# fperezgamonal/flownet2-tf

Measured on AMD Instinct MI355X. Metric: forward pairs/sec at 512x384 (FlowNet2), higher is better.
Workload: dtype f16x2 (split fp16 hi+lo operands, 3 fp16 MFMAs per product, fp32 accumulate); 1 GPU; FlowNet2 forward, batch=4 synthetic 512x384 pairs per GPU, seeded synthetic weights; pairs_per_gpu=4, parallelism=dp1 (no collective)

## Files before the change

flownet2-tf_amd/csrc/conv.hip:

```cpp
#include "conv_common.h"
#include <cstdlib>

namespace fn2 {

template <typename T, typename OutT, int TC, int WC, int WP>
__global__ void __launch_bounds__(256) conv_igemm_kernel(const ConvArgs p) {
  constexpr int CH = 16 / (int)sizeof(T);
  constexpr int BC = WC * TC * 16;
  constexpr int BP = WP * 64;
  constexpr int NT = 256;
  static_assert(WC * WP == 4, "4 waves per block");
  constexpr int NPR = BP / 64;
  constexpr int NWR = (BC * 4 + NT - 1) / NT;
  constexpr int WSWZ_BIT = (TC == 4) ? 5 : (TC == 2) ? 4 : 3;
  __shared__ uint4 lds[2][(BC + BP) * 4];

  const int tid = threadIdx.x, lane = tid & 63, wave = tid >> 6;
  const int wc = wave / WP, wp = wave % WP;
  const int cid = tid & 3;

  int pad_y = p.pad, pad_x = p.pad, oy_off = 0, ox_off = 0, osc = 1;
  const T* wgt = reinterpret_cast<const T*>(p.wgt);
  const int phase = blockIdx.z / p.splitk, split = blockIdx.z - phase * p.splitk;
  if (p.deconv) {
// ... 40 lines not shown
        const T* src = in + (pbase[q] + (size_t)iy * p.W + ix) * p.in_cs + p.in_c0 + cc * CH;
        v = *reinterpret_cast<const uint4*>(src);
      }
      rp[q] = v;
    }
#pragma unroll
    for (int q = 0; q < NWR; ++q) {
      const int e = tid + NT * q;
      uint4 v = make_uint4(0, 0, 0, 0);
      if (e < BC * 4) {
        const T* src = wgt + (size_t)(c0 + (e >> 2)) * wrow_elems + ((size_t)kt * 4 + cid) * CH;
        v = *reinterpret_cast<const uint4*>(src);
      }
      rw[q] = v;
    }
  };
  auto advance = [&]() {
    cc += 4;
    while (cc >= p.cin_chunks) {
      cc -= p.cin_chunks;
      if (++kx == p.KW) { kx = 0; ++ky; }
    }
  };
  auto store_step = [&](int buf) {
#pragma unroll
    for (int q = 0; q < NWR; ++q) {
      const int e = tid + NT * q;
      if (e < BC * 4) {
        const int row = e >> 2;
        lds[buf][row * 4 + (cid ^ (((row >> WSWZ_BIT) & 1) * 3))] = rw[q];
      }
    }
#pragma unroll
    for (int q = 0; q < NPR; ++q) {
      const int row = (tid >> 2) + 64 * q;
      lds[buf][(BC + row) * 4 + (cid ^ (((row >> 3) & 1) * 3))] = rp[q];
    }
  };

  const int fi = lane & 15, fchunk = (lane >> 4) ^ (((fi >> 3) & 1) * 3);
  int a_off[TC], b_off[4];
#pragma unroll
  for (int t = 0; t < TC; ++t)
    a_off[t] = (wc * TC * 16 + (fi >> 2) * (TC * 4) + t * 4 + (fi & 3)) * 4 + fchunk;
#pragma unroll
  for (int pt = 0; pt < 4; ++pt) b_off[pt] = (BC + wp * 64 + pt * 16 + fi) * 4 + fchunk;

  f32x4 acc[TC][4];
#pragma unroll
  for (int t = 0; t < TC; ++t)
#pragma unroll
    for (int pt = 0; pt < 4; ++pt) acc[t][pt] = f32x4{0.f, 0.f, 0.f, 0.f};

  load_step(kt0);
  store_step(0);
  __syncthreads();

  for (int kt = kt0; kt < kt1; ++kt) {
    const int buf = (kt - kt0) & 1;
    const bool more = kt + 1 < kt1;
    if (more) {
      advance();
      load_step(kt + 1);
    }
    uint4 fa[TC], fb[4];
#pragma unroll
    for (int t = 0; t < TC; ++t) fa[t] = lds[buf][a_off[t]];
#pragma unroll
    for (int pt = 0; pt < 4; ++pt) fb[pt] = lds[buf][b_off[pt]];
    if constexpr (sizeof(T) == 2) {
#pragma unroll
      for (int t = 0; t < TC; ++t)
#pragma unroll
        for (int pt = 0; pt < 4; ++pt)
          acc[t][pt] = mfma_16x16x32<T>(fa[t], fb[pt], acc[t][pt]);
    } else {
#pragma unroll
      for (int j = 0; j < 4; ++j)
#pragma unroll
        for (int t = 0; t < TC; ++t)
#pragma unroll
          for (int pt = 0; pt < 4; ++pt)
            acc[t][pt] = __builtin_amdgcn_mfma_f32_16x16x4f32(__builtin_bit_cast(f32x4, fa[t])[j],
                                                             __builtin_bit_cast(f32x4, fb[pt])[j], acc[t][pt], 0, 0, 0);
    }
    if (more) store_step(buf ^ 1);
    __syncthreads();
  }

  OutT* out = reinterpret_cast<OutT*>(p.out);
  const int cout_base = c0 + wc * TC * 16 + (lane >> 4) * (TC * 4);
  if (p.splitk > 1) {
    float* slab = p.ws + (size_t)split * p.N * p.out_H * p.out_W * p.ws_cs;
#pragma unroll
    for (int pt = 0; pt < 4; ++pt) {
      const int m = m0 + wp * 64 + pt * 16 + fi;
      if (m >= p.M) continue;
      const int n = m / (p.OH * p.OW);
      const int rem = m - n * (p.OH * p.OW);
      const int oy = rem / p.OW, ox = rem - oy * p.OW;
      float* po = slab + (((size_t)n * p.out_H + (oy * osc + oy_off)) * p.out_W + (ox * osc + ox_off)) * p.ws_cs;
#pragma unroll
      for (int t = 0; t < TC; ++t) {
        const int co = cout_base + t * 4;
        if (co < p.ws_cs)
          *reinterpret_cast<float4*>(po + co) =
              make_float4(acc[t][pt][0], acc[t][pt][1], acc[t][pt][2], acc[t][pt][3]);
      }
    }
    return;
  }
  float bias[TC][4];
#pragma unroll
  for (int t = 0; t < TC; ++t)
#pragma unroll
    for (int r = 0; r < 4; ++r) {
      const int co = cout_base + t * 4 + r;
      bias[t][r] = (p.bias != nullptr && co < p.Cout) ? p.bias[co] : 0.f;
    }
#pragma unroll
  for (int pt = 0; pt < 4; ++pt) {
    const int m = m0 + wp * 64 + pt * 16 + fi;
    if (m >= p.M) continue;
    const int n = m / (p.OH * p.OW);
    const int rem = m - n * (p.OH * p.OW);
    const int oy = rem / p.OW, ox = rem - oy * p.OW;
    OutT* po = out + (((size_t)n * p.out_H + (oy * osc + oy_off)) * p.out_W + (ox * osc + ox_off)) * p.out_cs +
               p.out_c0;
#pragma unroll
    for (int t = 0; t < TC; ++t) {
      float v[4];
      const int co = cout_base + t * 4;
#pragma unroll
      for (int r = 0; r < 4; ++r) {
        float x = acc[t][pt][r] * p.out_scale + bias[t][r];
        if constexpr (sizeof(OutT) == 4) {
          if (p.accum && co + r < p.Cout) x += load_elem<OutT>(po + co + r);
          if (co + r < p.Cout) x = act_grad<OutT>(p, out, po + co + r, co + r, x);
        }
        if (p.act == FN2_ACT_LEAKY) x = leaky(x);
        v[r] = x;
      }
      if (p.vec_ok && co + 3 < p.Cout) {
        store4<OutT>(po + co, v[0], v[1], v[2], v[3]);
      } else {
#pragma unroll
        for (int r = 0; r < 4; ++r)
          if (co + r < p.Cout) store_elem<OutT>(po + co + r, v[r]);
      }
    }
  }
}

template <typename OutT>
__global__ void __launch_bounds__(256) splitk_finalize_kernel(const float* __restrict__ ws, const float* __restrict__ bias,
                                                              OutT* __restrict__ out, long npix, int ws_cs, int splitk,
                                                              int Cout, int out_cs, int out_c0, int act, int vec_ok,
                                                              float out_scale, int accum, const OutT* __restrict__ mask_y,
                                                              int mask_c0, int mask_c1, const float* __restrict__ up_src,
                                                              const float* __restrict__ up_w, const float* __restrict__ up_bias,
                                                              int up_c0, int out_H, int out_W) {
  const int groups = ws_cs / 4;
  const int groups_all = groups + (up_src != nullptr ? 1 : 0);
  const long total = npix * groups_all;
  const size_t slab = (size_t)npix * ws_cs;
  for (long i = (long)blockIdx.x * blockDim.x + threadIdx.x; i < total; i += (long)gridDim.x * blockDim.x) {
    const long pix = i / groups_all;
    const int co = (int)(i - pix * groups_all) * 4;
    if (co == groups * 4) {
      const int ox = (int)(pix % out_W), oy = (int)((pix / out_W) % out_H), n = (int)(pix / out_W / out_H);
      const int H = out_H >> 1, W = out_W >> 1;
      const int a = oy & 1, b = ox & 1, y = oy >> 1, x = ox >> 1;
      float r0 = up_bias ? up_bias[0] : 0.f, r1 = up_bias ? up_bias[1] : 0.f;
#pragma unroll
      for (int ty = 0; ty < 2; ++ty) {
        const int iy = y - 1 + a + ty, ky = 3 - a - 2 * ty;
        if (iy < 0 || iy >= H) continue;
#pragma unroll
        for (int tx = 0; tx < 2; ++tx) {
          const int ix = x - 1 + b + tx, kx = 3 - b - 2 * tx;
          if (ix < 0 || ix >= W) continue;
          const float2 v = *reinterpret_cast<const float2*>(up_src + (((long)n * H + iy) * W + ix) * 2);
          const float* ww = up_w + (ky * 4 + kx) * 4;
          r0 += v.x * ww[0] + v.y * ww[1];
          r1 += v.x * ww[2] + v.y * ww[3];
        }
      }
      OutT* pu = out + (size_t)pix * out_cs + up_c0;
      store_elem<OutT>(pu, r0);
      store_elem<OutT>(pu + 1, r1);
      continue;
    }
    float4 v = *reinterpret_cast<const float4*>(ws + pix * ws_cs + co);
    int s = 1;
    for (; s + 3 < splitk; s += 4) {
      float4 t[4];
#pragma unroll
      for (int u = 0; u < 4; ++u) t[u] = *reinterpret_cast<const float4*>(ws + (s + u) * slab + pix * ws_cs + co);
#pragma unroll
      for (int u = 0; u < 4; ++u) { v.x += t[u].x; v.y += t[u].y; v.z += t[u].z; v.w += t[u].w; }
    }
    for (; s < splitk; ++s) {
      const float4 t = *reinterpret_cast<const float4*>(ws + s * slab + pix * ws_cs + co);
      v.x += t.x; v.y += t.y; v.z += t.z; v.w += t.w;
    }
    float r[4] = {v.x, v.y, v.z, v.w};
    OutT* po = out + (size_t)pix * out_cs + out_c0 + co;
    const bool full = vec_ok && co + 3 < Cout;
    float old[4] = {0.f, 0.f, 0.f, 0.f}, yv[4] = {1.f, 1.f, 1.f, 1.f};
    const bool mask = mask_y != nullptr && co < mask_c1 && co + 4 > mask_c0;
    if constexpr (sizeof(OutT) == 4) {
      if (full) {
        if (accum) load4<OutT>(po, old);
        if (mask) load4<OutT>(mask_y + (size_t)pix * out_cs + out_c0 + co, yv);
      } else {
#pragma unroll
        for (int j = 0; j < 4; ++j)
          if (co + j < Cout) {
            if (accum) old[j] = load_elem<OutT>(po + j);
            if (mask) yv[j] = load_elem<OutT>(mask_y + (size_t)pix * out_cs + out_c0 + co + j);
          }
      }
    }
#pragma unroll
    for (int j = 0; j < 4; ++j) {
      r[j] *= out_scale;
      if (bias != nullptr && co + j < Cout) r[j] += bias[co + j];
      if constexpr (sizeof(OutT) == 4) {
        if (accum) r[j] += old[j];
        if (mask && co + j >= mask_c0 && co + j < mask_c1) r[j] *= yv[j] > 0.f ? 1.f : (yv[j] < 0.f ? 0.1f : 0.55f);
      }
      if (act == FN2_ACT_LEAKY) r[j] = leaky(r[j]);
    }
    if (vec_ok && co + 3 < Cout) {
      store4<OutT>(po, r[0], r[1], r[2], r[3]);
    } else {
#pragma unroll
      for (int j = 0; j < 4; ++j)
        if (co + j < Cout) store_elem<OutT>(po + j, r[j]);
    }
  }
}

template <typename T>
__device__ __forceinline__ void dot_chunk(const uint4& x, const uint4& w0, const uint4& w1, float& a0, float& a1);
template <>
__device__ __forceinline__ void dot_chunk<float>(const uint4& x, const uint4& w0, const uint4& w1, float& a0,
                                                 float& a1) {
  const float4 xv = __builtin_bit_cast(float4, x), u = __builtin_bit_cast(float4, w0), v = __builtin_bit_cast(float4, w1);
  a0 += xv.x * u.x + xv.y * u.y + xv.z * u.z + xv.w * u.w;
  a1 += xv.x * v.x + xv.y * v.y + xv.z * v.z + xv.w * v.w;
}
template <>
__device__ __forceinline__ void dot_chunk<bf16_t>(const uint4& x, const uint4& w0, const uint4& w1, float& a0,
                                                  float& a1) {
  const unsigned xs[4] = {x.x, x.y, x.z, x.w}, us[4] = {w0.x, w0.y, w0.z, w0.w}, vs[4] = {w1.x, w1.y, w1.z, w1.w};
#pragma unroll
  for (int j = 0; j < 4; ++j) {
    const float xl = __uint_as_float(xs[j] << 16), xh = __uint_as_float(xs[j] & 0xffff0000u);
    a0 += xl * __uint_as_float(us[j] << 16) + xh * __uint_as_float(us[j] & 0xffff0000u);
    a1 += xl * __uint_as_float(vs[j] << 16) + xh * __uint_as_float(vs[j] & 0xffff0000u);
  }
}

template <>
__device__ __forceinline__ void dot_chunk<x2_t>(const uint4&, const uint4&, const uint4&, float&, float&) {}
template <>
__device__ __forceinline__ void dot_chunk<f16_t>(const uint4& x, const uint4& w0, const uint4& w1, float& a0,
                                                 float& a1) {
  typedef __attribute__((ext_vector_type(8))) _Float16 h8;
  const h8 xv = __builtin_bit_cast(h8, x), u = __builtin_bit_cast(h8, w0), v = __builtin_bit_cast(h8, w1);
#pragma unroll
  for (int j = 0; j < 8; ++j) {
    a0 += (float)xv[j] * (float)u[j];
    a1 += (float)xv[j] * (float)v[j];
  }
}

template <typename T>
__global__ void __launch_bounds__(256) flow_head_kernel(const ConvArgs p) {
  constexpr int CH = 16 / (int)sizeof(T);
  const int lane = threadIdx.x & 63;
  const long wave = ((long)blockIdx.x * blockDim.x + threadIdx.x) >> 6;
  const long nwaves = ((long)gridDim.x * blockDim.x) >> 6;
  const T* in = reinterpret_cast<const T*>(p.in);
  const T* w0 = reinterpret_cast<const T*>(p.wgt);
  const T* w1 = w0 + (size_t)p.ksteps * 4 * CH;
  float* out = reinterpret_cast<float*>(p.out);
  if constexpr (is_x2<T>::value) {
    const float* wf0 = reinterpret_cast<const float*>(p.wgt);
    const float* wf1 = wf0 + (size_t)p.ksteps * 4 * CH;
    const int groups = p.cin_chunks >> 1;
    const int nitems = 9 * groups;
    if (p.dbg & 16384) {
      __shared__ float part[8];
      for (long m = blockIdx.x; m < p.M; m += gridDim.x)
        fh_pixel(in, p.H, p.W, p.in_cs, p.in_c0, groups, wf0, wf1, p.bias, p.out_scale, out + (size_t)m * p.out_cs + p.out_c0, m, part);
      return;
    }
    for (long m = wave; m < p.M; m += nwaves) {
      const int x = (int)(m % p.W), y = (int)((m / p.W) % p.H);
      const size_t nb = (size_t)(m / p.W / p.H) * p.H * p.W;
      float a0 = 0.f, a1 = 0.f;
      for (int q = lane; q < nitems; q += 64) {
        const int tap = q / groups, gi = q - tap * groups;
        const int ky = tap / 3, kx = tap - ky * 3;
        const int iy = y + ky - 1, ix = x + kx - 1;
        if (iy < 0 || iy >= p.H || ix < 0 || ix >= p.W) continue;
        const uint4* src = reinterpret_cast<const uint4*>(in + (nb + (size_t)iy * p.W + ix) * p.in_cs + p.in_c0 + gi * 8);
        float xv[8];
        join8(src[0], src[1], xv);
        const float* u = wf0 + (size_t)q * 8;
        const float* v = wf1 + (size_t)q * 8;
#pragma unroll
        for (int j = 0; j < 8; ++j) {
          a0 += xv[j] * u[j];
          a1 += xv[j] * v[j];
        }
      }
// ... 626 lines not shown
  }
  a.kg = 1;
  if (d->wgt_layout == 1 && tile == 128 && !(a.dbg & 32)) {
    const char* e_kg = getenv("FN2_KG");
    if (!e_kg || atoi(e_kg) != 0) {
      const char* e3 = getenv("FN2_KG3_MAX");
      const char* e2 = getenv("FN2_KG2_MAX");
      const long blocks = (long)cdiv(a.M, 64) * (a.cout_pad / 128) * phases;
      if (blocks <= (e3 ? atoi(e3) : 0)) { a.bp64 = 1; a.kg = 3; }
      else if (blocks <= (e2 ? atoi(e2) : 95)) { a.bp64 = 1; a.kg = 2; }
    }
  }
  if (d->wgt_layout == 1 && tile == 128 && !(a.dbg & 32) && d->in.dtype == FN2_F16X2) {
    const char* e_lo = getenv("FN2_DEEP_MIN");
    const char* e_hi = getenv("FN2_DEEP_MAX");
    const long blocks = (long)cdiv(a.M, 64) * (a.cout_pad / 128) * phases;
    const int lo = e_lo ? atoi(e_lo) : 0, hi = e_hi ? atoi(e_hi) : -1;
    if (blocks >= lo && blocks <= hi) { a.bp64 = 3; a.kg = 1; }
  }
  if (d->wgt_layout == 1 && tile == 128 && a.bp64 == 1 && a.kg == 1) {
    const char* e_ring = getenv("FN2_RING_MAX");
    const int ring_max = e_ring ? atoi(e_ring) : 512;
    const long blocks = (long)cdiv(a.M, 64) * (a.cout_pad / 128) * phases;
    if ((a.dbg & 256) || (blocks >= 384 && blocks <= ring_max)) a.bp64 = 2;
    const char* e_rs = getenv("FN2_RING_SPLIT");
    if (e_rs && blocks >= atoi(e_rs) && blocks < 384) a.bp64 = 2;
  }
  *tile_out = tile;
  *phases_out = phases;
  return FN2_OK;
}

static int preferred_split(const ConvArgs& a, int tile, int phases) {
  if (a.merged) return 1;
  const int bp = tile == 128 ? (a.bp64 ? 64 : 128) : (a.bp64 ? 128 : 256);
  const long blocks = (long)cdiv(a.M, bp) * (a.cout_pad / tile) * phases;
  const char* e_min = getenv("FN2_SPLIT_MINBLOCKS");
  if (blocks >= (e_min ? atoi(e_min) : 384)) return 1;
  if (a.bp64 == 3) {
    const char* e_sl = getenv("FN2_DEEP_SLOTS");
    int s = (int)((e_sl ? atoi(e_sl) : 256) / blocks);
    const int maxs = a.ksteps / 16;
    if (s > maxs) s = maxs;
    if (s > 16) s = 16;
    if (s < 2) return 1;
    const int kper = cdiv(a.ksteps, s);
    return cdiv(a.ksteps, kper);
  }
  if (a.kg > 1) {
    const char* e_nos = getenv("FN2_KG_NOSPLIT");
    if (blocks >= (e_nos ? atoi(e_nos) : 96)) return 1;
    const char* e_sl = getenv("FN2_KG_SLOTS");
    int s = (int)((e_sl ? atoi(e_sl) : 256) / blocks);
    const int maxs = a.ksteps / (12 * a.kg);
    if (s > maxs) s = maxs;
    if (s > 16) s = 16;
    if (s < 2) return 1;
    const int kper = cdiv(a.ksteps, s);
    return cdiv(a.ksteps, kper);
  }
  const char* e = getenv("FN2_SPLIT_SLOTS");
  const char* e_rsl = getenv("FN2_RING_SPLIT_SLOTS");
  const int slots = (tile == 128 && a.bp64 == 2) ? (e_rsl ? atoi(e_rsl) : 512) : e ? atoi(e) : 640;
  int s = (int)(slots / blocks);
  const int maxs = a.ksteps / 8;
  if (s > maxs) s = maxs;
  if (s > 16) s = 16;
  if (s < 2) return 1;
  const int kper = cdiv(a.ksteps, s);
  return cdiv(a.ksteps, kper);
}

static int64_t split_bytes(const ConvArgs& a, int s) {
  return (int64_t)s * a.N * a.out_H * a.out_W * a.ws_cs * (int64_t)sizeof(float);
}

}

extern "C" {

int64_t fn2_conv2d_workspace_bytes(const fn2_conv_desc* d) {
  ConvArgs a;
  int tile, phases;
  if (build_args(d, &a, &tile, &phases) != FN2_OK) return 0;
  if (is_flow_head(d)) return 0;
  const int s = preferred_split(a, tile, phases);
  return s > 1 ? split_bytes(a, s) : 0;
}

int fn2_conv2d_splits(const fn2_conv_desc* d) {
  ConvArgs a;
  int tile, phases;
  if (build_args(d, &a, &tile, &phases) != FN2_OK || is_flow_head(d)) return 1;
  int sk = preferred_split(a, tile, phases);
  while (sk > 1 && (d->workspace == nullptr || split_bytes(a, sk) > d->workspace_bytes)) --sk;
  if ((long)a.N * a.out_H * a.out_W * a.ws_cs >= (1L << 31)) sk = 1;
  if (sk > 1) {
    const int kper = cdiv(a.ksteps, sk);
    sk = cdiv(a.ksteps, kper);
    if (d->wgt_layout >= 1) sk = cdiv(a.ksteps / 2, cdiv(kper, 2));
  }
  return sk < 1 ? 1 : sk;
}

int fn2_conv2d_kernel_name(const fn2_conv_desc* d, char* name, int cap) {
  FN2_REQUIRE(name && cap > 0, "conv2d_kernel_name: no buffer");
  name[0] = 0;
  if (!d || d->wgt_layout < 1 || is_flow_head(d)) return FN2_OK;
  conv_name_sink() = ConvNameSink{name, cap};
  const int rc = fn2_conv2d(d, nullptr);
  conv_name_sink() = ConvNameSink{nullptr, 0};
  return rc;
}

int fn2_conv2d(const fn2_conv_desc* d, void* stream) {
  ConvArgs a;
  int tile, phases;
  int rc = build_args(d, &a, &tile, &phases);
  if (rc) return rc;
  hipStream_t s = (hipStream_t)stream;
  if (is_flow_head(d)) {
    int blocks = grid_for((long)a.M * 64, 256);
    if (d->in.dtype == FN2_F16X2 && a.M <= 4096 && !(a.dbg & 32768)) {
      a.dbg |= 16384;
      blocks = a.M;
    } else {
      a.dbg &= ~16384;
    }
    if (d->in.dtype == FN2_F32)
      hipLaunchKernelGGL(flow_head_kernel<float>, dim3(blocks), dim3(256), 0, s, a);
    else if (d->in.dtype == FN2_BF16)
      hipLaunchKernelGGL(flow_head_kernel<bf16_t>, dim3(blocks), dim3(256), 0, s, a);
    else if (d->in.dtype == FN2_F16)
      hipLaunchKernelGGL(flow_head_kernel<f16_t>, dim3(blocks), dim3(256), 0, s, a);
    else
      hipLaunchKernelGGL(flow_head_kernel<x2_t>, dim3(blocks), dim3(256), 0, s, a);
    FN2_CHECK_LAUNCH("flow_head");
    return FN2_OK;
  }
  int sk = preferred_split(a, tile, phases);
  while (sk > 1 && (d->workspace == nullptr || split_bytes(a, sk) > d->workspace_bytes)) --sk;
  if ((long)a.N * a.out_H * a.out_W * a.ws_cs >= (1L << 31)) sk = 1;
  if (sk > 1) {
    a.kper = cdiv(a.ksteps, sk);
    sk = cdiv(a.ksteps, a.kper);
  }
  if (sk > 1) {
    a.splitk = sk;
    a.ws = reinterpret_cast<float*>(d->workspace);
  }
  if (d->up_src != nullptr && d->kind == 5 && 2 * d->out.c == 32) {
    a.up_src = d->up_src; a.up_w = d->up_w; a.up_bias = d->up_bias; a.up_c0 = d->up_c0;
  }
  if (d->head != nullptr && !conv_name_sink().buf) {
    const fn2_conv_desc* h = reinterpret_cast<const fn2_conv_desc*>(d->head);
    FN2_REQUIRE(d->kind == 1 && is_flow_head(h) && h->head == nullptr && h->up_src == nullptr,
                "conv2d: head rides on a kind-1 transposed conv and is a 3x3 two-output fp32 flow head");
    FN2_REQUIRE(h->in.data == d->in.data && h->in.n == d->in.n && h->in.h == d->in.h && h->in.w == d->in.w &&
                    h->in.cs == d->in.cs && h->in.c0 == d->in.c0 && h->in.dtype == d->in.dtype,
                "conv2d: head and transposed conv must read the same view");
    ConvArgs ha;
    int htile, hphases;
    rc = build_args(h, &ha, &htile, &hphases);
    if (rc) return rc;
    const char* e = getenv("FN2_HEAD_RIDE");
    const bool ride = d->in.dtype == FN2_F16X2 && d->wgt_layout == 2 && tile == 128 && sk > 1 && !(e && atoi(e) == 0);
    if (ride) {
      a.fh_M = ha.M;
      a.fh_w = reinterpret_cast<const float*>(ha.wgt);
      a.fh_w1 = ha.ksteps * 4 * 4;
      a.fh_groups = ha.cin_chunks >> 1;
      a.fh_bias = ha.bias;
      a.fh_out = reinterpret_cast<float*>(ha.out);
      a.fh_out_cs = ha.out_cs; a.fh_out_c0 = ha.out_c0;
      a.fh_scale = ha.out_scale;
    } else {
      rc = fn2_conv2d(h, stream);
      if (rc) return rc;
    }
  }
  if (d->wgt_layout >= 1) {
    a.ksteps = a.ksteps / 2;
    a.kper = cdiv(a.kper, 2);
    a.splitk = cdiv(a.ksteps, a.kper);
    if (a.splitk == 1) a.ws = nullptr;
    rc = launch_conv_fast(a, d->in.dtype, d->out.dtype, tile, phases, s);
  } else if (d->in.dtype == FN2_F32 && d->out.dtype == FN2_F16X2) rc = launch_conv<float, x2_t>(a, tile, phases, s);
  else if (d->in.dtype == FN2_F32) rc = launch_conv<float, float>(a, tile, phases, s);
  else if (d->in.dtype == FN2_BF16 && d->out.dtype == FN2_BF16) rc = launch_conv<bf16_t, bf16_t>(a, tile, phases, s);
  else if (d->in.dtype == FN2_BF16) rc = launch_conv<bf16_t, float>(a, tile, phases, s);
  else if (d->out.dtype == FN2_F16) rc = launch_conv<f16_t, f16_t>(a, tile, phases, s);
  else rc = launch_conv<f16_t, float>(a, tile, phases, s);
  if (rc || conv_name_sink().buf) return rc;
  if (a.splitk == 1) {
    if (d->up_src == nullptr || a.up_src != nullptr) return rc;
    fn2_tensor uv = d->out;
    uv.c = 2; uv.c0 = d->up_c0;
    return fn2_upsample_flow(d->up_src, d->up_w, d->up_bias, &uv, d->out.n, d->out.h / 2, d->out.w / 2, stream);
  }
  if ((a.dbg & 524288) || d->raw_partials) return rc;
  const long npix = (long)a.N * a.out_H * a.out_W;
  const int fgrid = grid_for(npix * (a.ws_cs / 4 + (d->up_src != nullptr ? 1 : 0)), 256);
  if (d->out.dtype == FN2_F32)
    hipLaunchKernelGGL(splitk_finalize_kernel<float>, dim3(fgrid), dim3(256), 0, s, a.ws, a.bias, (float*)a.out, npix,
                       a.ws_cs, a.splitk, a.Cout, a.out_cs, a.out_c0, a.act, a.vec_ok, a.out_scale, a.accum, (const float*)a.mask_y, a.mask_c0, a.mask_c1, d->up_src, d->up_w, d->up_bias, d->up_c0, a.out_H, a.out_W);
  else if (d->out.dtype == FN2_F16X2)
    hipLaunchKernelGGL(splitk_finalize_kernel<x2_t>, dim3(fgrid), dim3(256), 0, s, a.ws, a.bias, (x2_t*)a.out,
                       npix, a.ws_cs, a.splitk, a.Cout, a.out_cs, a.out_c0, a.act, a.vec_ok, a.out_scale, a.accum, (const x2_t*)a.mask_y, a.mask_c0, a.mask_c1, d->up_src, d->up_w, d->up_bias, d->up_c0, a.out_H, a.out_W);
  else if (d->out.dtype == FN2_BF16)
    hipLaunchKernelGGL(splitk_finalize_kernel<bf16_t>, dim3(fgrid), dim3(256), 0, s, a.ws, a.bias, (bf16_t*)a.out,
                       npix, a.ws_cs, a.splitk, a.Cout, a.out_cs, a.out_c0, a.act, a.vec_ok, a.out_scale, a.accum, (const bf16_t*)a.mask_y, a.mask_c0, a.mask_c1, d->up_src, d->up_w, d->up_bias, d->up_c0, a.out_H, a.out_W);
  else
    hipLaunchKernelGGL(splitk_finalize_kernel<f16_t>, dim3(fgrid), dim3(256), 0, s, a.ws, a.bias, (f16_t*)a.out,
                       npix, a.ws_cs, a.splitk, a.Cout, a.out_cs, a.out_c0, a.act, a.vec_ok, a.out_scale, a.accum, (const f16_t*)a.mask_y, a.mask_c0, a.mask_c1, d->up_src, d->up_w, d->up_bias, d->up_c0, a.out_H, a.out_W);
  FN2_CHECK_LAUNCH("splitk_finalize");
  return FN2_OK;
}

int fn2_flow_head_gather(const float* t, int t_cs, const float* bias, float* out, int n, int h, int w, void* stream) {
  FN2_REQUIRE(t && out, "flow_head_gather: null pointer");
  FN2_REQUIRE(t_cs >= 18 && t_cs % 2 == 0 && n >= 1 && h >= 1 && w >= 1, "flow_head_gather: t must hold 18 partials per pixel");
  const long tiles = (long)n * ((h + GT_Y - 1) / GT_Y) * ((w + GT_X - 1) / GT_X);
  if (tiles >= 1024)
    hipLaunchKernelGGL(flow_head_gather_kernel, dim3((unsigned)std::min<long>(tiles, 1 << 16)), dim3(256), 0,
                       (hipStream_t)stream, t, t_cs, bias, out, n, h, w);
  else
    hipLaunchKernelGGL(flow_head_gather_small_kernel, dim3(grid_for((long)n * h * w, 256)), dim3(256), 0,
                       (hipStream_t)stream, t, t_cs, bias, out, n, h, w);
  FN2_CHECK_LAUNCH("flow_head_gather");
  return FN2_OK;
}

int fn2_flow_head_tail(const float* t, int t_cs, int taps, const float* bias, float* pf, int n, int h, int w, int ring,
                       const float* up_w, const float* up_bias, const fn2_tensor* up_out, void* stream) {
  return fn2_flow_head_tail_slabs(t, t_cs, 1, 0, 1.f, taps, bias, pf, n, h, w, ring, up_w, up_bias, up_out, stream);
}

int fn2_flow_head_tail_slabs(const float* t, int t_cs, int nslab, int64_t slab_stride, float scale, int taps, const float* bias,
                             float* pf, int n, int h, int w, int ring, const float* up_w, const float* up_bias,
                             const fn2_tensor* up_out, void* stream) {
  FN2_REQUIRE(t && pf, "flow_head_tail: null pointer");
  FN2_REQUIRE(nslab >= 1 && (nslab == 1 || slab_stride >= (int64_t)n * h * w * t_cs), "flow_head_tail: bad slab geometry");
  const TailSrc ts{t, t_cs, nslab, (long)slab_stride, scale};
  FN2_REQUIRE(taps == 3 || taps == 5, "flow_head_tail: taps must be 3 or 5");
  FN2_REQUIRE(t_cs >= 2 * taps * taps && t_cs % 2 == 0 && n >= 1 && h >= 1 && w >= 1,
              "flow_head_tail: t must hold 2 * taps^2 partials per pixel");
  FN2_REQUIRE(!ring || (h >= 3 && w >= 3), "flow_head_tail: a border ring needs h, w >= 3");
  const bool up = up_w != nullptr;
  hipStream_t s = (hipStream_t)stream;
  if (!up) {
    launch_head_tail_t<float>(taps, false, ts, bias, pf, n, h, w, ring, nullptr, nullptr, nullptr, 0, 0, s);
  } else {
    int rc = check_view(up_out, "flow_head_tail upsample output");
    if (rc) return rc;
    FN2_REQUIRE(up_out->c == 2 && up_out->n == n && up_out->h == 2 * h && up_out->w == 2 * w,
                "flow_head_tail: the upsample view must be [n, 2h, 2w, 2]");
    if (up_out->dtype == FN2_F16X2) FN2_REQUIRE(up_out->c0 % 2 == 0, "flow_head_tail: split-fp16 slice must start at an even channel");
    void* d = up_out->data;
    if (up_out->dtype == FN2_F32) launch_head_tail_t<float>(taps, true, ts, bias, pf, n, h, w, ring, up_w, up_bias, d, up_out->cs, up_out->c0, s);
    else if (up_out->dtype == FN2_F16X2) launch_head_tail_t<x2_t>(taps, true, ts, bias, pf, n, h, w, ring, up_w, up_bias, d, up_out->cs, up_out->c0, s);
    else if (up_out->dtype == FN2_BF16) launch_head_tail_t<bf16_t>(taps, true, ts, bias, pf, n, h, w, ring, up_w, up_bias, d, up_out->cs, up_out->c0, s);
    else launch_head_tail_t<f16_t>(taps, true, ts, bias, pf, n, h, w, ring, up_w, up_bias, d, up_out->cs, up_out->c0, s);
  }
  FN2_CHECK_LAUNCH("flow_head_tail");
  return FN2_OK;
}

int fn2_flow_head5(const fn2_tensor* x, const void* wgt, int cin_pad, int kpad, float out_scale, const float* bias, float* pf,
                   int ring, const float* ring_w, const float* ring_b, void* stream) {
  int rc = check_view(x, "flow_head5 input");
  if (rc) return rc;
  FN2_REQUIRE(wgt && pf, "flow_head5: null pointer");
  FN2_REQUIRE(x->dtype == FN2_F16X2 && x->cs % 8 == 0 && x->c0 % 8 == 0, "flow_head5: split-fp16 input, 8-aligned view");
  FN2_REQUIRE(cin_pad % 32 == 0 && cin_pad >= x->c && x->c0 + cin_pad <= x->cs && kpad == cin_pad,
              "flow_head5: the channel run must be whole 128-byte lines inside the buffer (kpad = cin_pad)");
  FN2_REQUIRE(!ring || (x->h >= 3 && x->w >= 3), "flow_head5: a border ring needs h, w >= 3");
  const long in_bytes = (long)x->n * x->h * x->w * x->cs * 4;
  FN2_REQUIRE(in_bytes < (1L << 31), "flow_head5: input buffer >= 2 GiB is not addressable by the LDS-DMA kernel");
  ConvArgs a = {};
  a.in = x->data; a.wgt = wgt; a.bias = bias; a.out = pf;
  a.N = x->n; a.H = x->h; a.W = x->w; a.in_cs = x->cs; a.in_c0 = x->c0;
  a.cin_chunks = cin_pad / 4;
  a.KH = a.KW = 1; a.stride = 1; a.pad = 0;
  a.OH = x->h; a.OW = x->w;
  a.h5_tx = cdiv(x->w, 28); a.h5_ty = cdiv(x->h, 4); a.h5_ring = ring ? 1 : 0;
  const long blocks = (long)x->n * a.h5_ty * a.h5_tx;
  FN2_REQUIRE(blocks * 256 < (1L << 31), "flow_head5: too many tiles");
  a.M = (int)(blocks * 256);
  a.out_H = x->h; a.out_W = x->w; a.out_cs = 2; a.out_c0 = 0; a.Cout = 2;
  a.ksteps = cin_pad / 32;
  a.cout_pad = 64;
  a.act = FN2_ACT_NONE;
  a.kh_ph[0] = a.kh_ph[1] = a.kw_ph[0] = a.kw_ph[1] = 1;
  a.kg = 1; a.splitk = 1; a.kper = a.ksteps; a.ws = nullptr; a.ws_cs = 4;
  a.out_scale = out_scale == 0.f ? 1.f : out_scale;
  a.in_bytes = (int)in_bytes;
  { const char* e = getenv("FN2_H5_DBG"); a.dbg = e ? atoi(e) : 0; }
  a.h5_tiles = (int)blocks;
  long total = blocks;
  if (ring && ring_w != nullptr) {
    FN2_REQUIRE(ring_b != nullptr, "flow_head5: ring_w without ring_b");
    a.h5_wc = ring_w; a.h5_bc = ring_b; a.h5_groups = (x->c + 7) / 8;
    FN2_REQUIRE(x->c0 + a.h5_groups * 8 <= x->cs, "flow_head5: the last 8-channel group reaches past the buffer");
    total += cdiv((long)x->n * (2 * x->w + 2 * (x->h - 2)), 16);
  }
  {
    const char* e = getenv("FN2_H5_STRIP");
    if ((a.ksteps == 3 || a.ksteps == 6) && !(e && atoi(e) == 0) && !(a.dbg & 10)) {
      const int nstrip = cdiv(x->w, 60);
      const char* eb = getenv("FN2_H5_BLOCKS");
      const int target = eb ? atoi(eb) : 256;
      const int segs = std::max(1, std::min(x->h, target / std::max(1, x->n * nstrip)));
      const int rows = cdiv(x->h, segs);
      a.h5_tx = nstrip; a.h5_ty = cdiv(x->h, rows); a.h5_rows = rows;
      return launch_head5_strip(a, x->n * a.h5_ty * a.h5_tx, (hipStream_t)stream);
    }
  }
  return launch_head5(a, (int)total, (hipStream_t)stream);
}

int fn2_flow_head_ring(const fn2_tensor* x, const float* wc, const float* bc, float* pf, void* stream) {
  int rc = check_view(x, "flow_head_ring input");
  if (rc) return rc;
  FN2_REQUIRE(wc && bc && pf, "flow_head_ring: null pointer");
  FN2_REQUIRE(x->dtype == FN2_F16X2 && x->cs % 8 == 0 && x->c0 % 8 == 0, "flow_head_ring: split-fp16 input, 8-aligned view");
  FN2_REQUIRE(x->h >= 3 && x->w >= 3, "flow_head_ring: h, w >= 3");
  const int groups = (x->c + 7) / 8;
  FN2_REQUIRE(x->c0 + groups * 8 <= x->cs, "flow_head_ring: the last 8-channel group reaches past the buffer");
  const long ring = (long)x->n * (2 * x->w + 2 * (x->h - 2));
  hipLaunchKernelGGL(head_ring_kernel, dim3(grid_for(ring * 64, 256)), dim3(256), 0, (hipStream_t)stream, (const x2_t*)x->data,
                     x->cs, x->c0, groups, wc, bc, pf, x->n, x->h, x->w);
  FN2_CHECK_LAUNCH("flow_head_ring");
  return FN2_OK;
}

int fn2_upsample_flow(const float* in, const float* w, const float* bias, const fn2_tensor* out, int n, int h, int wd,
                      void* stream) {
  FN2_REQUIRE(in && w, "upsample_flow: null pointer");
  int rc = check_view(out, "upsample_flow output");
  if (rc) return rc;
  FN2_REQUIRE(out->c == 2 && out->n == n && out->h == 2 * h && out->w == 2 * wd,
              "upsample_flow: output view must be [n, 2h, 2w, 2]");
  const long total = (long)n * 4 * h * wd;
  if (out->dtype == FN2_F32)
    hipLaunchKernelGGL(upsample_flow_kernel<float>, dim3(grid_for(total, 256)), dim3(256), 0, (hipStream_t)stream,
                       in, w, bias, (float*)out->data, n, h, wd, out->cs, out->c0);
  else if (out->dtype == FN2_F16X2)
    hipLaunchKernelGGL(upsample_flow_kernel<x2_t>, dim3(grid_for(total, 256)), dim3(256), 0, (hipStream_t)stream,
                       in, w, bias, (x2_t*)out->data, n, h, wd, out->cs, out->c0);
  else if (out->dtype == FN2_BF16)
    hipLaunchKernelGGL(upsample_flow_kernel<bf16_t>, dim3(grid_for(total, 256)), dim3(256), 0, (hipStream_t)stream,
                       in, w, bias, (bf16_t*)out->data, n, h, wd, out->cs, out->c0);
  else
    hipLaunchKernelGGL(upsample_flow_kernel<f16_t>, dim3(grid_for(total, 256)), dim3(256), 0, (hipStream_t)stream,
                       in, w, bias, (f16_t*)out->data, n, h, wd, out->cs, out->c0);
  FN2_CHECK_LAUNCH("upsample_flow");
  return FN2_OK;
}

int fn2_pack_pair(const float* a, const float* b, const fn2_tensor* out, int pad, void* stream) {
  FN2_REQUIRE(a && b, "pack_pair: null pointer");
  int rc = check_view(out, "pack_pair output");
  if (rc) return rc;
  FN2_REQUIRE(out->c == 6, "pack_pair: output view must have 6 channels");
  return pack_imgs<2>(a, b, out, out->n, 0, pad, stream);
}

int fn2_pack_image_s2d(const float* img, int n_img, int h, int w, const fn2_tensor* out, int n0, int pad, void* stream) {
  FN2_REQUIRE(img, "pack_image_s2d: null pointer");
// ... 32 lines not shown
```

flownet2-tf_amd/csrc/conv2.hip:

```cpp
#include "conv_common.h"

#include <type_traits>
#include <algorithm>
#include <utility>

#ifndef FN2_X2_ORDER
#define FN2_X2_ORDER 0
#endif
#ifndef FN2_CONV_ABLATE
#define FN2_CONV_ABLATE 0
#endif
#ifndef FN2_SETPRIO
#define FN2_SETPRIO 1
#endif

namespace fn2 {

typedef __attribute__((address_space(3))) void* lptr_t;

constexpr unsigned kOobOffset = 0x80000000u;

typedef int v4i_t __attribute__((ext_vector_type(4)));
typedef unsigned u32x4_t __attribute__((ext_vector_type(4)));

__device__ __forceinline__ v4i_t make_rsrc(const void* base, int bytes) {
  const unsigned long long a = (unsigned long long)base;
  return v4i_t{(int)(a & 0xffffffffu), (int)((a >> 32) & 0xffffu), bytes, 0x00020000};
}

__device__ __forceinline__ void dma16(const v4i_t rsrc, const void* lds, unsigned voff, int soff) {
  const unsigned la = (unsigned)(unsigned long long)(lptr_t)lds;
  asm volatile("s_mov_b32 m0, %0\n\ts_nop 0\n\tbuffer_load_dwordx4 %1, %2, %3 offen lds"
               :: "s"(la), "v"(voff), "s"(rsrc), "s"(soff) : "memory");
}

__device__ __forceinline__ void h5_ring_pixel(const ConvArgs& p, long m) {
  const int lane = threadIdx.x & 63;
  const int H = p.OH, W = p.OW, ring = 2 * W + 2 * (H - 2);
  const int nitems = 25 * p.h5_groups;
  const size_t case_stride = (size_t)nitems * 16;
  const x2_t* in = reinterpret_cast<const x2_t*>(p.in);
  float* pf = reinterpret_cast<float*>(p.out);
  const int n = (int)(m / ring), r = (int)(m - (long)n * ring);
  int y, x;
  if (r < W) { y = 0; x = r; }
  else if (r < 2 * W) { y = H - 1; x = r - W; }
  else { const int q = r - 2 * W; y = 1 + (q >> 1); x = (q & 1) ? W - 1 : 0; }
  const int cy = y == 0 ? 0 : (y == H - 1 ? 2 : 1), cx = x == 0 ? 0 : (x == W - 1 ? 2 : 1);
  const int cs = 3 * cy + cx;
  const float* w = p.h5_wc + (size_t)cs * case_stride;
  float a0 = 0.f, a1 = 0.f;
  constexpr int U = 5;
  for (int q0 = lane; q0 < nitems; q0 += 64 * U) {
    uint4 xs[U][2];
    float4 ws[U][4];
    bool ok[U];
#pragma unroll
    for (int k = 0; k < U; ++k) {
      const int q = min(q0 + 64 * k, nitems - 1);
      const int tap = q / p.h5_groups, gi = q - tap * p.h5_groups;
      const int ky = tap / 5, kx = tap - ky * 5;
      const int iy = y + ky - 2, ix = x + kx - 2;
      ok[k] = q0 + 64 * k < nitems && iy >= 0 && iy < H && ix >= 0 && ix < W;
      const int cy2 = min(max(iy, 0), H - 1), cx2 = min(max(ix, 0), W - 1);
      const uint4* src = reinterpret_cast<const uint4*>(in + (((size_t)n * H + cy2) * W + cx2) * p.in_cs + p.in_c0 + gi * 8);
      xs[k][0] = src[0];
      xs[k][1] = src[1];
      const float4* u = reinterpret_cast<const float4*>(w + (size_t)q * 16);
#pragma unroll
      for (int j = 0; j < 4; ++j) ws[k][j] = u[j];
    }
#pragma unroll
    for (int k = 0; k < U; ++k) {
      float xv[8];
      join8(xs[k][0], xs[k][1], xv);
      if (ok[k]) {
#pragma unroll
        for (int j = 0; j < 4; ++j) {
          a0 += xv[2 * j] * ws[k][j].x;
          a1 += xv[2 * j] * ws[k][j].y;
          a0 += xv[2 * j + 1] * ws[k][j].z;
          a1 += xv[2 * j + 1] * ws[k][j].w;
        }
      }
    }
  }
#pragma unroll
  for (int off = 32; off > 0; off >>= 1) {
    a0 += __shfl_xor(a0, off, 64);
    a1 += __shfl_xor(a1, off, 64);
  }
  if (lane == 0)
    *reinterpret_cast<float2*>(pf + (((size_t)n * H + y) * W + x) * 2) = make_float2(a0 + p.h5_bc[2 * cs], a1 + p.h5_bc[2 * cs + 1]);
}

__device__ __forceinline__ void h5_ring_block(const ConvArgs& p, int rb) {
  const int wave = threadIdx.x >> 6;
  const long total = (long)p.N * (2 * p.OW + 2 * (p.OH - 2));
  for (int k = 0; k < 4; ++k) {
    const long m = (long)rb * 16 + wave * 4 + k;
    if (m >= total) return;
    h5_ring_pixel(p, m);
  }
}

__device__ __forceinline__ float* h5_t(uint4* a, uint4* b, int half, int w) {
  const int byte = w * 4;
  return byte < half ? reinterpret_cast<float*>(reinterpret_cast<char*>(a) + byte)
                     : reinterpret_cast<float*>(reinterpret_cast<char*>(b) + (byte - half));
}

template <typename T, typename OutT, int WC, int WP, int TCN = 2, int TPN = 2, int STAGES = 2, int KG = 1, bool M16 = false,
          bool WREG = false, bool SLAB = false, bool HEAD5 = false, bool FEED = false>
__global__ void __launch_bounds__(256 * KG + (FEED ? 256 : 0)) conv_igemm2_kernel(const ConvArgs p) {
#if defined(__HIP_DEVICE_COMPILE__)
  constexpr int CH = 16 / (int)sizeof(T);
  constexpr int ESZ = (int)sizeof(T);
  constexpr int BC = WC * TCN * 32, BP = WP * TPN * 32;
  static_assert(WC * WP == 4, "4 waves per block");
  constexpr int NWI = BC / 32;
  constexpr int NPI = BP / 32;
  static_assert(!WREG || (is_x2<T>::value && TCN == 1 && KG == 1 && (STAGES == 2 || STAGES == 3) && !M16),
                "WREG: split fp16, one cout tile per wave, two-stage loop or 3-slot ring");
  constexpr int BOFF = WREG ? 0 : BC;
  constexpr int kWTileBytes = (32 * TPN * (TCN * 32 + 4) + 32 * TPN) * 4;
  constexpr int kPoolHalfRows = (STAGES * BP * 128 / 2 > 2 * kWTileBytes ? STAGES * BP * 128 / 2 : 2 * kWTileBytes) / 128 + 1;
  constexpr int ROWS = WREG ? kPoolHalfRows : BC + BP;
  static_assert(KG == 1 || STAGES == 2, "K groups run the two-stage loop");
  constexpr bool kDeep = STAGES > 3;
  __shared__ uint4 lds0_all[(kDeep ? STAGES : WREG ? 2 : KG) * ROWS * 8];
  __shared__ uint4 lds1_all[(kDeep || WREG) ? 1 : KG * ROWS * 8];
  __shared__ uint4 lds2_own[(STAGES == 3 && !WREG) ? ROWS * 8 : 1];

  if constexpr (HEAD5) {
    if ((int)blockIdx.x >= p.h5_tiles) {
      h5_ring_block(p, (int)blockIdx.x - p.h5_tiles);
      return;
    }
  }
  if constexpr (WREG && SLAB && is_x2<T>::value) {
    if (p.fh_M > 0 && (int)blockIdx.z >= p.fh_z0) {
      if (FEED && threadIdx.x >= 256) return;
      float* part = reinterpret_cast<float*>(lds0_all);
      const long e = (((long)blockIdx.z - p.fh_z0) * gridDim.y + blockIdx.y) * gridDim.x + blockIdx.x;
      const long total = (long)(gridDim.z - p.fh_z0) * gridDim.y * gridDim.x;
      for (long m = e; m < p.fh_M; m += total)
        fh_pixel(reinterpret_cast<const x2_t*>(p.in), p.H, p.W, p.in_cs, p.in_c0, p.fh_groups, p.fh_w, p.fh_w + p.fh_w1,
                 p.fh_bias, p.fh_scale, p.fh_out + (size_t)m * p.fh_out_cs + p.fh_out_c0, m, part);
      return;
    }
  }
  const int tid = threadIdx.x, lane = tid & 63;
  const int wave_all = __builtin_amdgcn_readfirstlane(tid >> 6);
  const int grp = KG > 1 ? wave_all >> 2 : 0;
  static_assert(!FEED || (WREG && STAGES == 3 && KG == 1), "FEED: the WREG ring");
  const bool feeder = FEED && wave_all >= 4;
  const int wave = (KG > 1 || FEED) ? wave_all & 3 : wave_all;
  uint4* const lds0 = lds0_all + grp * (ROWS * 8);
  uint4* const lds1 = WREG ? lds0_all + BP * 8 : kDeep ? lds0_all + ROWS * 8 : lds1_all + grp * (ROWS * 8);
  uint4* const lds2 = WREG ? lds0_all + 2 * BP * 8 : lds2_own;
  uint4* const ep1 = (kDeep || WREG) ? lds0_all + ROWS * 8 : lds1_all;
  const int wc = wave / WP, wp = wave % WP;

  int pad_y = p.pad, pad_x = p.pad, oy_off = 0, ox_off = 0, osc = 1;
  const T* wgt = reinterpret_cast<const T*>(p.wgt);
  const int phase = blockIdx.z / p.splitk, split = blockIdx.z - phase * p.splitk;
  const unsigned wrow_bytes = (unsigned)p.ksteps * 128u;
  if (p.deconv) {
    const int a = phase >> 1, b = phase & 1;
    pad_y = a ? p.ph_pad1 : p.ph_pad0; pad_x = b ? p.ph_pad1 : p.ph_pad0; oy_off = a; ox_off = b; osc = 2;
    wgt += (size_t)phase * p.cout_pad * (wrow_bytes / ESZ);
  }
  const int khi = p.deconv ? p.kh_ph[phase >> 1] : p.KH, kwi = p.deconv ? p.kw_ph[phase & 1] : p.KW;
  const int nst_all = (p.cin_chunks >> 3) * khi * kwi;
  const int kt0 = split * p.kper + grp;
  const int kt1 = (FN2_CONV_ABLATE && (p.dbg & 1048576)) ? kt0 : min(nst_all, split * p.kper + p.kper);
  int bx = blockIdx.x, by = blockIdx.y;
  if (!(p.dbg & 4)) {
    const int NT = HEAD5 ? p.h5_tiles : gridDim.x * gridDim.y, L = blockIdx.x + gridDim.x * blockIdx.y;
    const int xcd = L & 7, chunk = NT >> 3, rem = NT & 7;
    const int Lp = xcd * chunk + min(xcd, rem) + (L >> 3);
    if (p.wmajor) {
      by = Lp / (int)gridDim.x;
      bx = Lp - by * (int)gridDim.x;
    } else {
      bx = Lp / (int)gridDim.y;
      by = Lp - bx * (int)gridDim.y;
    }
  }
  const int m0 = bx * BP;
  const int c0 = by * BC;

  const v4i_t rsrc_w = make_rsrc(wgt, (int)(p.cout_pad * wrow_bytes));
  const v4i_t rsrc_x = make_rsrc(p.in, p.in_bytes);

  const int lrow = lane >> 3, lphys = lane & 7;
  unsigned woff[NWI];
#pragma unroll
  for (int j = 0; j < NWI; ++j) {
    const int row = wave * (BC / 4) + j * 8 + lrow;
    woff[j] = (unsigned)(c0 + row) * wrow_bytes + (unsigned)((lphys ^ ((row >> 1) & 7)) * 16);
  }
  int roff[NPI];
  unsigned vmask[NPI];
#pragma unroll
  for (int j = 0; j < NPI; ++j) {
    const int row = wave * (BP / 4) + j * 8 + lrow;
    const int m = m0 + row;
    bool v = m < p.M;
    const int mm = v ? m : 0;
    int n = mm / (p.OH * p.OW);
    const int rem = mm - n * (p.OH * p.OW);
    int oy = rem / p.OW, ox = rem - oy * p.OW;
    if constexpr (HEAD5) {
      static_assert(BP == 256, "HEAD5: 8 x 32 positions per block");
      const int tx = bx % p.h5_tx, tyn = bx / p.h5_tx;
      n = tyn / p.h5_ty;
      oy = (tyn - n * p.h5_ty) * 4 - 2 + (row >> 5);
      ox = tx * 28 - 2 + (row & 31);
      v = true;
    }
    const int iy0 = oy * p.stride - pad_y, ix0 = ox * p.stride - pad_x;
    roff[j] = (((n * p.H + iy0) * p.W + ix0) * p.in_cs + p.in_c0) * ESZ + (lphys ^ ((row >> 1) & 7)) * 16;
    unsigned mk = 0;
    if (v) {
      for (int k = 0; k < p.KH; ++k) mk |= (unsigned)(iy0 + k >= 0 && iy0 + k < p.H) << k;
      for (int k = 0; k < p.KW; ++k) mk |= (unsigned)(ix0 + k >= 0 && ix0 + k < p.W) << (8 + k);
    }
    vmask[j] = mk;
  }
  const int spt = p.cin_chunks >> 3;
  const int ntap = khi * kwi;
  const bool tap_outer = FN2_CONV_ABLATE && (p.dbg & 16);
  int sc = tap_outer ? kt0 % spt : kt0 / ntap;
  int tap = tap_outer ? kt0 / spt : kt0 - sc * ntap;
  int ky = tap / kwi, kx = tap - ky * kwi;
  int wstage = kt0;

  auto issue_piece = [&](auto piece_c, uint4* lds) {
    constexpr int i = decltype(piece_c)::value;
    if constexpr (i < NWI) {
      if constexpr (!WREG) {
        if (!(FN2_CONV_ABLATE && (p.dbg & 2)))
          dma16(rsrc_w, &lds[(wave * (BC / 4) + i * 8) * 8], woff[i], ((ky * p.KW + kx) * spt + sc) * 128);
      }
    } else {
      constexpr int j = i - NWI;
      const unsigned tbit = (1u << ky) | (1u << (8 + kx));
      const int toff = ((ky * p.W + kx) * p.in_cs + sc * 8 * CH) * ESZ;
      const unsigned voff = ((vmask[j] & tbit) == tbit && wstage < kt1) ? (unsigned)(roff[j] + toff) : kOobOffset;
      if (!(FN2_CONV_ABLATE && (p.dbg & 1)))
        dma16(rsrc_x, &lds[(BOFF + wave * (BP / 4) + j * 8) * 8], voff, 0);
    }
  };
  u32x4_t wfa[WREG ? 4 : 1], wfb[WREG ? 4 : 1], wfc[(WREG && STAGES == 3) ? 4 : 1];
  const unsigned wlane = (unsigned)lane * 16u;
  const int wtile_off = WREG ? ((c0 >> 5) + wc) * (p.ksteps * 4096) : 0;
  auto load_w = [&](u32x4_t (&wf)[WREG ? 4 : 1]) {
    if constexpr (WREG) {
      const int soff = wtile_off + ((ky * p.KW + kx) * spt + sc) * 4096;
      asm volatile("buffer_load_dwordx4 %0, %4, %5, %6 offen\n\t"
                   "buffer_load_dwordx4 %1, %4, %5, %6 offen offset:1024\n\t"
                   "buffer_load_dwordx4 %2, %4, %5, %6 offen offset:2048\n\t"
                   "buffer_load_dwordx4 %3, %4, %5, %6 offen offset:3072"
                   : "=&v"(wf[0]), "=&v"(wf[1]), "=&v"(wf[2]), "=&v"(wf[3])
                   : "v"(wlane), "s"(rsrc_w), "s"(soff) : "memory");
    }
  };
  auto advance1 = [&]() {
    ++wstage;
    if (tap_outer) {
      if (++sc == spt) {
        sc = 0;
        if (++kx == kwi) { kx = 0; ++ky; }
      }
      if (ky == khi) { ky = 0; sc = spt; }
    } else if (++kx == kwi) {
      kx = 0;
      if (++ky == khi) { ky = 0; ++sc; }
    }
  };
  auto advance = [&]() {
#pragma unroll
    for (int g = 0; g < KG; ++g) advance1();
  };
  auto issue_stage = [&](uint4* lds) {
    [&]<int... I>(std::integer_sequence<int, I...>) {
      (issue_piece(std::integral_constant<int, I>{}, lds), ...);
    }(std::make_integer_sequence<int, NWI + NPI>{});
    advance();
  };
  auto issue_stage_w = [&](uint4* lds, u32x4_t (&wf)[WREG ? 4 : 1]) {
    [&]<int... I>(std::integer_sequence<int, I...>) {
      (issue_piece(std::integral_constant<int, I>{}, lds), ...);
    }(std::make_integer_sequence<int, NWI + NPI>{});
    load_w(wf);
    advance();
  };
  auto wait_w = [&](u32x4_t (&wf)[WREG ? 4 : 1]) {
    if constexpr (WREG)
      asm volatile("s_waitcnt vmcnt(0)" : "+v"(wf[0]), "+v"(wf[1]), "+v"(wf[2]), "+v"(wf[3]) :: "memory");
  };

  const int fr = lane & 31, fh = lane >> 5, fsw = (fr >> 1) & 7;
  f32x16 acc[TCN][TPN];
#pragma unroll
  for (int tc = 0; tc < TCN; ++tc)
#pragma unroll
    for (int tp = 0; tp < TPN; ++tp)
#pragma unroll
      for (int q = 0; q < 16; ++q) acc[tc][tp][q] = 0.f;
  f32x4 acc16[M16 ? TCN * 2 : 1][M16 ? TPN * 2 : 1];
  if constexpr (M16) {
#pragma unroll
    for (int a = 0; a < TCN * 2; ++a)
#pragma unroll
      for (int b = 0; b < TPN * 2; ++b) acc16[a][b] = f32x4{0.f, 0.f, 0.f, 0.f};
  }

  auto compute = [&](const uint4* lds) {
    if (FN2_CONV_ABLATE && (p.dbg & 131072)) return;
#if FN2_SETPRIO
    __builtin_amdgcn_s_setprio(1);
#endif
    const uint4* A = &lds[(wc * TCN * 32 + fr) * 8];
    const uint4* B = &lds[(BC + wp * TPN * 32 + fr) * 8];
    if constexpr (is_x2<T>::value && M16) {
      const int r16 = lane & 15, g16 = lane >> 4;
      uint4 ah[TCN * 2], al[TCN * 2], bh[TPN * 2], bl[TPN * 2];
#pragma unroll
      for (int t = 0; t < TCN * 2; ++t) {
        const int row = wc * TCN * 32 + t * 16 + r16, sw = (row >> 1) & 7;
        ah[t] = lds[row * 8 + ((2 * g16) ^ sw)];
        al[t] = lds[row * 8 + ((2 * g16 + 1) ^ sw)];
      }
#pragma unroll
      for (int t = 0; t < TPN * 2; ++t) {
        const int row = BC + wp * TPN * 32 + t * 16 + r16, sw = (row >> 1) & 7;
        bh[t] = lds[row * 8 + ((2 * g16) ^ sw)];
        bl[t] = lds[row * 8 + ((2 * g16 + 1) ^ sw)];
      }
#pragma unroll
      for (int a = 0; a < TCN * 2; ++a)
#pragma unroll
        for (int b = 0; b < TPN * 2; ++b) {
          acc16[a][b] = mfma_16x16x32<f16_t>(al[a], bh[b], acc16[a][b]);
          acc16[a][b] = mfma_16x16x32<f16_t>(ah[a], bl[b], acc16[a][b]);
// ... 176 lines not shown
      asm volatile("s_waitcnt vmcnt(%0)\n\ts_barrier" :: "n"(ND * (D - 1)) : "memory");
      issue_stage(slot_ptr(wr));
      compute(slot_ptr(rd));
      rd = rd + 1 == STAGES ? 0 : rd + 1;
      wr = wr + 1 == STAGES ? 0 : wr + 1;
    }
    asm volatile("s_waitcnt vmcnt(0)" ::: "memory");
  } else {
    constexpr int ND = NWI + NPI;
    static_assert(ND == 5 || ND == 6 || ND == 8, "vmcnt literal below");
    auto ring_sync = [] {
      if constexpr (ND == 5) asm volatile("s_waitcnt vmcnt(5)\n\ts_barrier" ::: "memory");
      else if constexpr (ND == 6) asm volatile("s_waitcnt vmcnt(6)\n\ts_barrier" ::: "memory");
      else asm volatile("s_waitcnt vmcnt(8)\n\ts_barrier" ::: "memory");
    };
    issue_stage(lds0);
    issue_stage(lds1);
    const int nst3 = (kt1 - kt0 + 2) / 3 * 3;
    for (int s = 0; s < nst3; s += 3) {
      ring_sync(); issue_stage(lds2); compute(lds0);
      ring_sync(); issue_stage(lds0); compute(lds1);
      ring_sync(); issue_stage(lds1); compute(lds2);
    }
    asm volatile("s_waitcnt vmcnt(0)" ::: "memory");
  }

  if constexpr (KG > 1) {
    constexpr int NA4 = TCN * TPN * 4;
    static_assert((KG - 1) * 4 * NA4 * 64 <= KG * ROWS * 8, "reduction scratch must fit the stage buffers");
    float4* red = reinterpret_cast<float4*>(lds0_all);
    auto acc4 = [&](int idx) -> float4 {
      if constexpr (M16) {
        const f32x4 v = acc16[idx / (TPN * 2)][idx % (TPN * 2)];
        return make_float4(v[0], v[1], v[2], v[3]);
      } else {
        const int t = idx >> 2, q = idx & 3;
        return make_float4(acc[t / TPN][t % TPN][4 * q], acc[t / TPN][t % TPN][4 * q + 1], acc[t / TPN][t % TPN][4 * q + 2],
                           acc[t / TPN][t % TPN][4 * q + 3]);
      }
    };
    if (grp > 0) {
#pragma unroll
      for (int idx = 0; idx < NA4; ++idx) red[(((grp - 1) * 4 + wave) * NA4 + idx) * 64 + lane] = acc4(idx);
    }
    __syncthreads();
    if (grp > 0) return;
#pragma unroll
    for (int g = 0; g < KG - 1; ++g)
#pragma unroll
      for (int idx = 0; idx < NA4; ++idx) {
        const float4 v = red[((g * 4 + wave) * NA4 + idx) * 64 + lane];
        if constexpr (M16) {
          f32x4& d = acc16[idx / (TPN * 2)][idx % (TPN * 2)];
          d[0] += v.x; d[1] += v.y; d[2] += v.z; d[3] += v.w;
        } else {
          const int t = idx >> 2, q = idx & 3;
          acc[t / TPN][t % TPN][4 * q] += v.x; acc[t / TPN][t % TPN][4 * q + 1] += v.y;
          acc[t / TPN][t % TPN][4 * q + 2] += v.z; acc[t / TPN][t % TPN][4 * q + 3] += v.w;
        }
      }
  }

  if constexpr (HEAD5) {
    if (p.dbg & 2) return;
    constexpr int TS = 52;
    static_assert(256 * TS * 4 <= 2 * ROWS * 128, "T fits the stage buffers");
#pragma unroll
    for (int tc = 0; tc < TCN; ++tc)
#pragma unroll
      for (int tp = 0; tp < TPN; ++tp) {
        const int pos = wp * TPN * 32 + tp * 32 + fr;
        const int cb = tc * 32 + fh * 16;
#pragma unroll
        for (int q = 0; q < 4; ++q)
          if (cb + 4 * q < TS)
            *reinterpret_cast<float4*>(h5_t(lds0_all, lds1_all, ROWS * 128, pos * TS + cb + 4 * q)) =
                make_float4(acc[tc][tp][4 * q] * p.out_scale, acc[tc][tp][4 * q + 1] * p.out_scale,
                            acc[tc][tp][4 * q + 2] * p.out_scale, acc[tc][tp][4 * q + 3] * p.out_scale);
      }
    __syncthreads();
    if (p.dbg & 8) return;
    const int tx = bx % p.h5_tx, tyn = bx / p.h5_tx;
    const int n = tyn / p.h5_ty, ty = tyn - n * p.h5_ty;
    float* pf = reinterpret_cast<float*>(p.out);
    if (tid < 224) {
      const int o = tid & 1, px = tid >> 1;
      const int py = px / 28, pxx = px - py * 28;
      const int oy = ty * 4 + py, ox = tx * 28 + pxx;
      if (oy < p.OH && ox < p.OW && !(p.h5_ring && (oy == 0 || oy == p.OH - 1 || ox == 0 || ox == p.OW - 1))) {
        float a = p.bias ? p.bias[o] : 0.f;
#pragma unroll
        for (int uy = 0; uy < 5; ++uy)
#pragma unroll
          for (int ux = 0; ux < 5; ++ux)
            a += *h5_t(lds0_all, lds1_all, ROWS * 128, ((py + uy) * 32 + pxx + ux) * TS + (uy * 5 + ux) * 2 + o);
        pf[(((size_t)n * p.OH + oy) * p.OW + ox) * 2 + o] = a;
      }
    }
    return;
  }
  if (FN2_CONV_ABLATE && (p.dbg & 262144)) return;
  if constexpr (M16) {
    OutT* out16 = reinterpret_cast<OutT*>(p.out);
    const int r16 = lane & 15, g16 = lane >> 4;
    float* slab = p.splitk > 1 ? p.ws + (size_t)split * p.N * p.out_H * p.out_W * p.ws_cs : nullptr;
#pragma unroll
    for (int b = 0; b < TPN * 2; ++b) {
      const int m = m0 + wp * TPN * 32 + b * 16 + r16;
      if (m >= p.M) continue;
      const int n = m / (p.OH * p.OW);
      const int rem = m - n * (p.OH * p.OW);
      const int oy = rem / p.OW, ox = rem - oy * p.OW;
      const size_t opix = ((size_t)n * p.out_H + (oy * osc + oy_off)) * p.out_W + (ox * osc + ox_off);
      OutT* po = out16 + opix * p.out_cs + p.out_c0;
#pragma unroll
      for (int a = 0; a < TCN * 2; ++a) {
        const int co = c0 + wc * TCN * 32 + (a >> 1) * 32 + 16 * (g16 & 1) + 8 * (a & 1) + 4 * (g16 >> 1);
        if (slab != nullptr) {
          if (co < p.ws_cs)
            *reinterpret_cast<float4*>(slab + opix * p.ws_cs + co) =
                make_float4(acc16[a][b][0], acc16[a][b][1], acc16[a][b][2], acc16[a][b][3]);
          continue;
        }
        float v[4];
#pragma unroll
        for (int j = 0; j < 4; ++j) {
          float x = acc16[a][b][j] * p.out_scale + ((p.bias != nullptr && co + j < p.Cout) ? p.bias[co + j] : 0.f);
          if constexpr (sizeof(OutT) == 4) {
            if (p.accum && co + j < p.Cout) x += load_elem<OutT>(po + co + j);
            if (co + j < p.Cout) x = act_grad<OutT>(p, out16, po + co + j, co + j, x);
          }
          if (p.act == FN2_ACT_LEAKY) x = leaky(x);
          v[j] = x;
        }
        if (p.vec_ok && co + 3 < p.Cout) store_vec<OutT, 4>(po + co, v);
        else
#pragma unroll
          for (int j = 0; j < 4; ++j)
            if (co + j < p.Cout) store_elem<OutT>(po + co + j, v[j]);
      }
    }
    return;
  }

  OutT* out = reinterpret_cast<OutT*>(p.out);
  constexpr int WCOLS = TCN * 32, RS = WCOLS + 4, WROWS = 32 * TPN;
  constexpr int WTW = WROWS * RS + WROWS;
  constexpr bool kLdsT = (KG > 1 ? 4 : 2) * WTW * 4 <= KG * ROWS * 128;
  if constexpr (FEED && !kLdsT) { if (feeder) return; }
  float* const tl = reinterpret_cast<float*>(KG > 1 ? ep1 : (wave < 2 ? lds0_all : ep1)) + (KG > 1 ? wave : (wave & 1)) * WTW;
  constexpr int CPR = WCOLS / 4, RPI = 64 / CPR;
  static_assert(!SLAB || WREG, "SLAB is a specialisation of the WREG instantiations");
  if ((SLAB || !WREG) && p.splitk > 1) {
    float* slab = p.ws + (size_t)split * p.N * p.out_H * p.out_W * p.ws_cs;
    if constexpr (kLdsT) {
      if constexpr (STAGES >= 3) __syncthreads();
      if constexpr (FEED) { if (feeder) return; }
      int* rowoff = reinterpret_cast<int*>(tl + WROWS * RS);
#pragma unroll
      for (int tp = 0; tp < TPN; ++tp) {
        const int m = m0 + wp * TPN * 32 + tp * 32 + fr;
        const int mm = m < p.M ? m : 0;
        const int n = mm / (p.OH * p.OW);
        const int rem = mm - n * (p.OH * p.OW);
        const int oy = rem / p.OW, ox = rem - oy * p.OW;
        if (fh == 0) rowoff[tp * 32 + fr] = m < p.M ? (int)((((size_t)n * p.out_H + (oy * osc + oy_off)) * p.out_W + (ox * osc + ox_off)) * p.ws_cs) : -1;
#pragma unroll
        for (int tc = 0; tc < TCN; ++tc)
#pragma unroll
          for (int q = 0; q < 4; ++q)
            *reinterpret_cast<float4*>(tl + (tp * 32 + fr) * RS + tc * 32 + fh * 16 + q * 4) =
                make_float4(acc[tc][tp][4 * q], acc[tc][tp][4 * q + 1], acc[tc][tp][4 * q + 2], acc[tc][tp][4 * q + 3]);
      }
      const int rr = lane / CPR, ch = lane - rr * CPR;
      const int co = c0 + wc * WCOLS + ch * 4;
#pragma unroll
      for (int i = 0; i < WROWS / RPI; ++i) {
        const int row = i * RPI + rr;
        const float4 v = *reinterpret_cast<const float4*>(tl + row * RS + ch * 4);
        const int off = rowoff[row];
        if (off >= 0 && co < p.ws_cs) *reinterpret_cast<float4*>(slab + (size_t)off + co) = v;
      }
      return;
    }
#pragma unroll
    for (int tp = 0; tp < TPN; ++tp) {
      const int m = m0 + wp * TPN * 32 + tp * 32 + fr;
      if (m >= p.M) continue;
      const int n = m / (p.OH * p.OW);
      const int rem = m - n * (p.OH * p.OW);
      const int oy = rem / p.OW, ox = rem - oy * p.OW;
      float* po = slab + (((size_t)n * p.out_H + (oy * osc + oy_off)) * p.out_W + (ox * osc + ox_off)) * p.ws_cs;
#pragma unroll
      for (int tc = 0; tc < TCN; ++tc)
#pragma unroll
        for (int q = 0; q < 4; ++q) {
          const int co = c0 + wc * TCN * 32 + tc * 32 + fh * 16 + q * 4;
          if (co < p.ws_cs)
            *reinterpret_cast<float4*>(po + co) = make_float4(acc[tc][tp][4 * q], acc[tc][tp][4 * q + 1],
                                                              acc[tc][tp][4 * q + 2], acc[tc][tp][4 * q + 3]);
        }
    }
    return;
  }
  if constexpr (SLAB) return;
  const bool vec16 = (p.out_cs % 8 == 0) && (p.out_c0 % 8 == 0);
  const bool wide = kLdsT && sizeof(OutT) == 4 && vec16 && c0 + wc * WCOLS + WCOLS <= p.Cout && !(p.dbg & 4194304);
  int* const rowoff = reinterpret_cast<int*>(tl + WROWS * RS);
  if constexpr (STAGES >= 3 && kLdsT) __syncthreads();
  if constexpr (FEED) { if (feeder) return; }
#pragma unroll
  for (int tc = 0; tc < TCN; ++tc) {
    const int cout_base = c0 + wc * TCN * 32 + tc * 32 + fh * 16;
    float bias[16];
#pragma unroll
    for (int q = 0; q < 16; ++q) bias[q] = (p.bias != nullptr && cout_base + q < p.Cout) ? p.bias[cout_base + q] : 0.f;
#pragma unroll
    for (int tp = 0; tp < TPN; ++tp) {
      const int m = m0 + wp * TPN * 32 + tp * 32 + fr;
      if (wide && tc == 0 && fh == 0) rowoff[tp * 32 + fr] = m < p.M ? 0 : -1;
      if (m >= p.M) continue;
      const int n = m / (p.OH * p.OW);
      const int rem = m - n * (p.OH * p.OW);
      const int oy = rem / p.OW, ox = rem - oy * p.OW;
      const size_t opix = (((size_t)n * p.out_H + (oy * osc + oy_off)) * p.out_W + (ox * osc + ox_off));
      OutT* po = out + opix * p.out_cs + p.out_c0 + cout_base;
      float v[16];
#pragma unroll
      for (int q = 0; q < 16; ++q) v[q] = acc[tc][tp][q] * p.out_scale + bias[q];
      accum_act_grad16<OutT>(p, out, po, cout_base, vec16 && cout_base + 15 < p.Cout, v);
      if (p.act == FN2_ACT_LEAKY) {
#pragma unroll
        for (int q = 0; q < 16; ++q) v[q] = leaky(v[q]);
      }
      if (wide) {
        if (tc == 0 && fh == 0) rowoff[tp * 32 + fr] = (int)opix;
        store16<OutT>(reinterpret_cast<OutT*>(tl + (tp * 32 + fr) * RS + tc * 32 + fh * 16), v);
      } else if (vec16 && cout_base + 15 < p.Cout) {
        store16<OutT>(po, v);
      } else {
#pragma unroll
        for (int q = 0; q < 16; ++q)
          if (cout_base + q < p.Cout) store_elem<OutT>(po + q, v[q]);
      }
    }
  }
  if (wide) {
    const int rr = lane / CPR, ch = lane - rr * CPR;
    OutT* ob = out + p.out_c0 + c0 + wc * WCOLS + ch * 4;
#pragma unroll
    for (int i = 0; i < WROWS / RPI; ++i) {
      const int row = i * RPI + rr;
      const uint4 v = *reinterpret_cast<const uint4*>(tl + row * RS + ch * 4);
      const int opix = rowoff[row];
      if (opix >= 0) *reinterpret_cast<uint4*>(ob + (size_t)opix * p.out_cs) = v;
    }
  }
#endif
}

template <typename OutT, int WC, int WP, int TCN, int TPN, int KW>
__global__ void __launch_bounds__(256) conv_halo_kernel(const ConvArgs p) {
#if defined(__HIP_DEVICE_COMPILE__)
  using T = x2_t;
  constexpr int ESZ = 4;
  constexpr int BC = WC * TCN * 32, BP = WP * TPN * 32;
  static_assert(WC * WP == 4, "4 waves per block");
  constexpr int NWI = BC / 32;
  constexpr int BROWS = BP + 8;
  constexpr int NBP = BROWS / 8;
  constexpr int NBW = (NBP + 3) / 4;
  __shared__ uint4 ldsA[2][BC * 8];
  __shared__ uint4 ldsB[2][BROWS * 8];

  const int tid = threadIdx.x, lane = tid & 63;
  const int wave = __builtin_amdgcn_readfirstlane(tid >> 6);
  const int wc = wave / WP, wp = wave % WP;

  int pad_y = p.pad, pad_x = p.pad, oy_off = 0, ox_off = 0, osc = 1;
  const T* wgt = reinterpret_cast<const T*>(p.wgt);
  const int phase = blockIdx.z;
  const unsigned wrow_bytes = (unsigned)p.ksteps * 128u;
  if (p.merged) {
    pad_y = phase ? p.ph_pad1 : p.ph_pad0; pad_x = 1; oy_off = phase; ox_off = 0; osc = 2;
    wgt += (size_t)phase * p.cout_pad * (wrow_bytes / ESZ);
  } else if (p.deconv) {
    const int a = phase >> 1, b = phase & 1;
    pad_y = a ? p.ph_pad1 : p.ph_pad0; pad_x = b ? p.ph_pad1 : p.ph_pad0; oy_off = a; ox_off = b; osc = 2;
    wgt += (size_t)phase * p.cout_pad * (wrow_bytes / ESZ);
  }
  int bx = blockIdx.x, by = blockIdx.y;
  {
    const int NT = gridDim.x * gridDim.y, L = blockIdx.x + gridDim.x * blockIdx.y;
    const int xcd = L & 7, chunk = NT >> 3, rem = NT & 7;
    const int Lp = xcd * chunk + min(xcd, rem) + (L >> 3);
    bx = Lp / (int)gridDim.y;
    by = Lp - bx * (int)gridDim.y;
  }
  const int m0 = bx * BP, c0 = by * BC;
  const int tn = m0 / (p.OH * p.OW);
  const int trem = m0 - tn * (p.OH * p.OW);
  const int toy = trem / p.OW, tox = trem - toy * p.OW;
  const int iy_base = toy - pad_y, ix_base = tox - pad_x;

  const v4i_t rsrc_w = make_rsrc(wgt, (int)(p.cout_pad * wrow_bytes));
  const v4i_t rsrc_x = make_rsrc(p.in, p.in_bytes);
  const int lrow = lane >> 3, lphys = lane & 7;
// ... 788 lines not shown
```

flownet2-tf_amd/csrc/conv_common.h:

```cpp
#pragma once
#include "fn2_common.h"

namespace fn2 {

struct ConvArgs {
  const void* in;
  const void* wgt;
  const float* bias;
  void* out;
  int N, H, W, in_cs, in_c0;
  int cin_chunks;
  int KH, KW, stride, pad;
  int OH, OW;
  int M;
  int out_H, out_W, out_cs, out_c0, Cout;
  int ksteps;
  int cout_pad;
  int act;
  int deconv;
  int ph_pad0, ph_pad1;
  int kh_ph[2], kw_ph[2];
  int merged;
  int wmajor;
  int bp64;
  int KH_KW_hint;
  int kg;
  int h5_tx, h5_ty, h5_ring;
  int h5_tiles, h5_groups;
  const float* h5_wc;
  const float* h5_bc;
  int h5_rows;
  int fh_M, fh_z0;
  const float* fh_w;
  int fh_w1, fh_groups;
  const float* fh_bias;
  float* fh_out;
  int fh_out_cs, fh_out_c0;
  float fh_scale;
  const float* up_src; const float* up_w; const float* up_bias; int up_c0;
  int wfrag;
  int accum;
  int vec_ok;
  int splitk;
  int kper;
  float* ws;
  int ws_cs;
  float out_scale;
  int in_bytes;
  const void* mask_y;
  int mask_c0, mask_c1;
  int dbg;
};

__device__ __forceinline__ void fh_pixel(const x2_t* __restrict__ in, int H, int W, int in_cs, int in_c0, int groups,
                                         const float* __restrict__ wf0, const float* __restrict__ wf1,
                                         const float* __restrict__ bias, float out_scale, float* __restrict__ po, long m,
                                         float* part) {
  const int lane = threadIdx.x & 63, wv = threadIdx.x >> 6;
  const int nitems = 9 * groups;
  const int x = (int)(m % W), y = (int)((m / W) % H);
  const size_t nb = (size_t)(m / W / H) * H * W;
  float a0 = 0.f, a1 = 0.f;
  for (int q = threadIdx.x; q < nitems; q += 256) {
    const int tap = q / groups, gi = q - tap * groups;
    const int ky = tap / 3, kx = tap - ky * 3;
    const int iy = y + ky - 1, ix = x + kx - 1;
    if (iy < 0 || iy >= H || ix < 0 || ix >= W) continue;
    const uint4* src = reinterpret_cast<const uint4*>(in + (nb + (size_t)iy * W + ix) * in_cs + in_c0 + gi * 8);
    float xv[8];
    join8(src[0], src[1], xv);
    const float* u = wf0 + (size_t)q * 8;
    const float* v = wf1 + (size_t)q * 8;
#pragma unroll
    for (int j = 0; j < 8; ++j) {
      a0 += xv[j] * u[j];
      a1 += xv[j] * v[j];
    }
  }
#pragma unroll
  for (int off = 32; off > 0; off >>= 1) {
    a0 += __shfl_xor(a0, off, 64);
    a1 += __shfl_xor(a1, off, 64);
  }
  if (lane == 0) { part[wv * 2] = a0; part[wv * 2 + 1] = a1; }
  __syncthreads();
  if (threadIdx.x == 0) {
    po[0] = (part[0] + part[2] + part[4] + part[6]) * out_scale + (bias ? bias[0] : 0.f);
    po[1] = (part[1] + part[3] + part[5] + part[7]) * out_scale + (bias ? bias[1] : 0.f);
  }
  __syncthreads();
}

template <typename OutT>
__device__ __forceinline__ float act_grad(const ConvArgs& p, const OutT* out_base, const OutT* elem, int co, float x) {
  if (p.mask_y != nullptr && co >= p.mask_c0 && co < p.mask_c1) {
    const float y = load_elem<OutT>(reinterpret_cast<const OutT*>(p.mask_y) + (elem - out_base));
    x *= y > 0.f ? 1.f : (y < 0.f ? 0.1f : 0.55f);
  }
  return x;
}

template <typename OutT>
__device__ __forceinline__ void accum_act_grad16(const ConvArgs& p, const OutT* out_base, const OutT* po, int cout_base,
                                                 bool full, float (&v)[16]) {
  if constexpr (sizeof(OutT) == 4) {
    const bool mask = p.mask_y != nullptr && cout_base < p.mask_c1 && cout_base + 16 > p.mask_c0;
    if (!p.accum && !mask) return;
    if (full) {
      if (p.accum) {
        float o[16];
        load16<OutT>(po, o);
#pragma unroll
        for (int q = 0; q < 16; ++q) v[q] += o[q];
      }
      if (mask) {
        float y[16];
        load16<OutT>(reinterpret_cast<const OutT*>(p.mask_y) + (po - out_base), y);
#pragma unroll
        for (int q = 0; q < 16; ++q)
          if (cout_base + q >= p.mask_c0 && cout_base + q < p.mask_c1) v[q] *= y[q] > 0.f ? 1.f : (y[q] < 0.f ? 0.1f : 0.55f);
      }
    } else {
#pragma unroll
      for (int q = 0; q < 16; ++q)
        if (cout_base + q < p.Cout) {
          if (p.accum) v[q] += load_elem<OutT>(po + q);
          v[q] = act_grad<OutT>(p, out_base, po + q, cout_base + q, v[q]);
        }
    }
  }
}

template <typename OutT>
__device__ __forceinline__ void store4(OutT* p, float a, float b, float c, float d) {
  const float v[4] = {a, b, c, d};
  store_vec<OutT, 4>(p, v);
}

struct ConvNameSink { char* buf; int cap; };
ConvNameSink& conv_name_sink();

int launch_conv_fast(const ConvArgs& a, int in_dtype, int out_dtype, int tile, int phases, hipStream_t s);
int launch_head5(const ConvArgs& a, int blocks, hipStream_t s);
int launch_head5_strip(const ConvArgs& a, int blocks, hipStream_t s);
bool conv_fast_ok(int in_dtype, int cin_pad, int cout);

}
```

flownet2-tf_amd/src/_hip.py:

```python
import ctypes as C
import os

import numpy as np
import torch

_HERE = os.path.dirname(os.path.abspath(__file__))
LIB_PATH = os.path.join(os.path.dirname(_HERE), "lib", "libflownet2_hip.so")

FN2_F32, FN2_BF16, FN2_F16, FN2_F16X2 = 0, 1, 2, 3
ACT_NONE, ACT_LEAKY = 0, 1
OK = 0
ERR_INVALID_ARGUMENT, ERR_UNSUPPORTED, ERR_HIP = -1, -2, -3


class Fn2Tensor(C.Structure):
    _fields_ = [("data", C.c_void_p), ("dtype", C.c_int32), ("n", C.c_int32), ("h", C.c_int32),
                ("w", C.c_int32), ("c", C.c_int32), ("cs", C.c_int32), ("c0", C.c_int32)]


class Fn2ConvPlan(C.Structure):
    _fields_ = [("layout", C.c_int32), ("cout_tile", C.c_int32), ("kstep_elems", C.c_int32),
                ("wgt_dtype", C.c_int32)]


class Fn2ConvDesc(C.Structure):
    _fields_ = [("inp", Fn2Tensor), ("out", Fn2Tensor), ("wgt", C.c_void_p), ("bias", C.c_void_p),
                ("kind", C.c_int32), ("kh", C.c_int32), ("kw", C.c_int32), ("stride", C.c_int32),
                ("pad", C.c_int32), ("act", C.c_int32), ("cin_pad", C.c_int32), ("cout_pad", C.c_int32),
                ("kpad", C.c_int32), ("wgt_layout", C.c_int32), ("accumulate", C.c_int32), ("out_scale", C.c_float), ("workspace", C.c_void_p), ("workspace_bytes", C.c_int64),
                ("act_grad_y", C.c_void_p), ("act_grad_c0", C.c_int32), ("act_grad_c1", C.c_int32),
                ("up_src", C.c_void_p), ("up_w", C.c_void_p), ("up_bias", C.c_void_p), ("up_c0", C.c_int32),
                ("head", C.c_void_p), ("raw_partials", C.c_int32)]


class Fn2BwdwDesc(C.Structure):
    _fields_ = [("x", Fn2Tensor), ("dy", Fn2Tensor), ("dw", C.c_void_p), ("kind", C.c_int32), ("kh", C.c_int32),
                ("kw", C.c_int32), ("stride", C.c_int32), ("pad", C.c_int32), ("cin_pad", C.c_int32),
                ("cout_pad", C.c_int32), ("kpad", C.c_int32), ("wgt_layout", C.c_int32), ("db", C.c_void_p)]


_i, _p, _f = C.c_int, C.c_void_p, C.c_float
_ip = C.POINTER(C.c_int)
_tp = C.POINTER(Fn2Tensor)

PROTOTYPES = {
    "fn2_last_error": (C.c_char_p, []),
    "fn2_version": (_i, []),
    "fn2_crc32c": (C.c_uint32, [_p, C.c_int64, C.c_uint32]),
    "fn2_device_info": (_i, [C.c_char_p, _i, _ip]),
    "fn2_correlation_out_shape": (_i, [_i] * 7 + [_ip] * 3),
    "fn2_correlation_f32": (_i, [_p, _p, _p] + [_i] * 9 + [_p]),
    "fn2_correlation_workspace_bytes": (C.c_int64, [_i] * 9),
    "fn2_correlation_f32_ws": (_i, [_p, _p, _p] + [_i] * 9 + [_p, C.c_int64, _p]),
    "fn2_correlation_grad_f32": (_i, [_p] * 5 + [_i] * 9 + [_p]),
    "fn2_flow_warp_f32": (_i, [_p, _p, _p, _i, _i, _i, _i, _p]),
    "fn2_flow_warp_grad_f32": (_i, [_p] * 5 + [_i] * 4 + [_p]),
    "fn2_downsample_f32": (_i, [_p, _p] + [_i] * 6 + [_p]),
    "fn2_downsample_scaled_f32": (_i, [_p, _f, _p] + [_i] * 6 + [_p]),
    "fn2_fill_zero": (_i, [_p, C.c_int64, _p]),
    "fn2_add_f32": (_i, [_p, _p, C.c_int64, _p]),
    "fn2_slice_copy_f32": (_i, [_tp, _p, _p]),
    "fn2_resize_bilinear_f32": (_i, [_p, _p] + [_i] * 6 + [_f, _p]),
    "fn2_conv2d_plan": (_i, [_i, _i, _i, C.POINTER(Fn2ConvPlan)]),
    "fn2_conv2d_workspace_bytes": (C.c_int64, [C.POINTER(Fn2ConvDesc)]),
    "fn2_conv2d": (_i, [C.POINTER(Fn2ConvDesc), _p]),
    "fn2_conv2d_kernel_name": (_i, [C.POINTER(Fn2ConvDesc), C.c_char_p, _i]),
    "fn2_conv2d_splits": (_i, [C.POINTER(Fn2ConvDesc)]),
    "fn2_augment_f32": (_i, [_p, _p, _p, _p, _i, _i, _i, _i, _i, _i, _p]),
    "fn2_flow_augmentation_f32": (_i, [_p, _p, _p, _p, _i, _i, _i, _i, _i, _p]),
    "fn2_flow_head_gather": (_i, [_p, _i, _p, _p, _i, _i, _i, _p]),
    "fn2_upsample_flow": (_i, [_p, _p, _p, _tp, _i, _i, _i, _p]),
    "fn2_flow_head_tail": (_i, [_p, _i, _i, _p, _p, _i, _i, _i, _i, _p, _p, _tp, _p]),
    "fn2_flow_head_tail_slabs": (_i, [_p, _i, _i, C.c_int64, _f, _i, _p, _p, _i, _i, _i, _i, _p, _p, _tp, _p]),
    "fn2_flow_head_ring": (_i, [_tp, _p, _p, _p, _p]),
    "fn2_flow_head5": (_i, [_tp, _p, _i, _i, _f, _p, _p, _i, _p, _p, _p]),
    "fn2_u8_to_f32_lut": (_i, [_p, _p, _p, C.c_int64, _p]),
    "fn2_pack_pair": (_i, [_p, _p, _tp, _i, _p]),
    "fn2_pack_interp_u8": (_i, [_p, _p, _p, _p, _p, _tp, _i, _p]),
    "fn2_pack_image": (_i, [_p, _i, _tp, _i, _i, _p]),
    "fn2_pack_image_s2d": (_i, [_p, _i, _i, _i, _tp, _i, _i, _p]),
    "fn2_correlation_fused": (_i, [_tp, _tp, _tp, _i, _i, _i, _p]),
    "fn2_stack_input": (_i, [_p, _p, _p, _tp, _i, _p]),
    "fn2_fusion_input": (_i, [_p, _p, _p, _p, _tp, _i, _p]),
    "fn2_stack_input_pf": (_i, [_p, _p, _p, _i, _i, _f, _p, _tp, _i, _p]),
    "fn2_fusion_input_pf": (_i, [_p, _p, _p, _f, _p, _p, _f, _p, _i, _i, _tp, _i, _p]),
    "fn2_epe_loss_grad": (_i, [_p, _p, _p, _p, _i, _i, _i, _f, _f, _p]),
    "fn2_epe_loss_grad_weighted": (_i, [_p, _p, _p, _p, _p, _i, _i, _i, _f, _f, _p]),
    "fn2_leaky_bwd": (_i, [_tp, _tp, _p, _p]),
    "fn2_bias_grad": (_i, [_tp, _p, _p]),
    "fn2_gather_f32": (_i, [_p, _p, _p, C.c_int64, _p]),
    "fn2_to_f16x2": (_i, [_p, _p, _p, C.c_int64, _f, _p]),
    "fn2_to_f16x2_frag": (_i, [_p, _p, _p, C.c_int64, _f, _i, _p]),
    "fn2_adam_step": (_i, [_p, _p, _p, _p, C.c_int64, _f, _f, _f, _f, _i, _f, _f, _p]),
    "fn2_adam_step_multi": (_i, [_p, _p, _p, _i, _f, _f, _f, _f, _i, _f, _p]),
    "fn2_adam_step_multi_dev": (_i, [_p, _p, _p, _i, _p, _p]),
    "fn2_upsample_flow_bwd": (_i, [_tp, _p, _p, _p, _p, _i, _p]),
    "fn2_head_bwd_filter": (_i, [_tp, _p, _p, _i, _i, _p]),
    "fn2_head_g18": (_i, [_p, _tp, _p]),
    "fn2_head_bwd_data": (_i, [_p, _p, _tp, _i, _i, _p]),
    "fn2_conv2d_bwd_filter": (_i, [C.POINTER(Fn2BwdwDesc), _p]),
    "fn2_variational_workspace_bytes": (C.c_int64, [_i, _i, _i]),
    "fn2_variational_refine": (_i, [_p, _p, C.c_int64, C.c_int64, _p, C.c_int64, C.c_int64, _i, _i, _i, _f, _f, _f, _f,
                                    _i, _i, _i, _f, _p, C.c_int64, _p]),
    "fn2_capture_begin": (_i, [_p]),
    "fn2_capture_end": (_i, [_p, C.POINTER(C.c_void_p)]),
    "fn2_graph_launch": (_i, [_p, _p]),
    "fn2_graph_destroy": (_i, [_p]),
}

_lib = None


class HipLibraryMissing(RuntimeError):
    pass


def lib():
    global _lib
    if _lib is None:
        if not os.path.exists(LIB_PATH):
            raise HipLibraryMissing(
                "libflownet2_hip.so not found at %s -- build it with `make -C flownet2-tf_amd/csrc` "
                "(or __graft_entry__.build()); this package has no CPU fallback" % LIB_PATH)
        l = C.CDLL(LIB_PATH)
        for name, (res, args) in PROTOTYPES.items():
            fn = getattr(l, name)
            fn.restype = res
            fn.argtypes = args
        _lib = l
    return _lib


def check(rc):
    if rc == OK:
        return
    msg = lib().fn2_last_error().decode("utf-8", "replace")
    if rc == ERR_INVALID_ARGUMENT:
        raise ValueError(msg)
    if rc == ERR_UNSUPPORTED:
        raise NotImplementedError(msg)
    raise RuntimeError("HIP error: " + msg)


def require_device():
    if not torch.cuda.is_available():
        raise RuntimeError("no ROCm device visible: the FlowNet2 ops run on MI355X only (no CPU fallback)")
    return torch.device("cuda", torch.cuda.current_device())


def stream_ptr():
    return C.c_void_p(torch.cuda.current_stream().cuda_stream)


def ptr(t):
    return C.c_void_p(t.data_ptr())


def dtype_code(t):
    if t.dtype == torch.float32:
        return FN2_F32
    if t.dtype == torch.bfloat16:
        return FN2_BF16
    if t.dtype == torch.float16:
        return FN2_F16
    raise ValueError("unsupported dtype %s" % t.dtype)


def view(buf, c=None, c0=0, code=None):
    n, h, w, cs = buf.shape
    assert buf.is_contiguous()
    return Fn2Tensor(buf.data_ptr(), dtype_code(buf) if code is None else code, n, h, w,
                     cs - c0 if c is None else c, cs, c0)


def conv_plan(in_code, cin_pad, cout):
    p = Fn2ConvPlan()
    check(lib().fn2_conv2d_plan(in_code, cin_pad, cout, C.byref(p)))
    return p


def to_device_f32(x):
    dev = require_device()
    if isinstance(x, np.ndarray):
        return torch.from_numpy(np.ascontiguousarray(x, dtype=np.float32)).to(dev), "numpy"
    if isinstance(x, torch.Tensor):
        kind = "cuda" if x.is_cuda else "cpu"
        return x.detach().to(device=dev, dtype=torch.float32).contiguous(), kind
    raise TypeError("expected torch.Tensor or numpy.ndarray, got %r" % type(x))


def from_device(t, kind):
    if kind == "numpy":
        return t.cpu().numpy()
    if kind == "cpu":
        return t.cpu()
    return t
```

flownet2-tf_amd/src/engine.py:

```python
import ctypes as C
import math
import os

import numpy as np
import torch

from . import _hip, netdefs, weights as W

_DT = {"f32": torch.float32, "bf16": torch.bfloat16, "f16": torch.float16, "f16x2": torch.float32}
_CODE = {"f32": _hip.FN2_F32, "bf16": _hip.FN2_BF16, "f16": _hip.FN2_F16, "f16x2": _hip.FN2_F16X2}
_TILE_ARGS = {128: "2, 2, 2, 2", 64: "1, 4, 2, 2", 32: "1, 4, 1, 2"}


def conv2_kernel_args(tile, m, cout_pad, phases, x2=True):
    dbg = int(os.environ.get("FN2_CONV_DBG", "0"))
    blocks64 = -(-m // 64) * (cout_pad // 128) * phases if tile == 128 else 0
    big = "FN2_M16_MIN" in os.environ and blocks64 >= max(int(os.environ["FN2_M16_MIN"]), 513)
    m16 = "true" if (x2 and not dbg & 512 and (dbg & 1024 or big)) else "false"
    full = dbg & 32
    if tile < 128:
        base = {64: "1, 4, 2, 2, 2, 1", 32: "1, 4, 1, 2, 2, 1"}[tile] if full else {64: "1, 4, 2, 1, 2, 1", 32: "1, 4, 1, 1, 2, 1"}[tile]
        return f"{base}, {m16}"
    blocks = -(-m // 64) * (cout_pad // 128) * phases
    if not full and int(os.environ.get("FN2_KG", "1")):
        if blocks <= int(os.environ.get("FN2_KG3_MAX", "0")):
            return f"2, 2, 2, 1, 2, 3, {m16}"
        if blocks <= int(os.environ.get("FN2_KG2_MAX", "95")):
            return f"2, 2, 2, 1, 2, 2, {m16}"
    if not full and blocks >= int(os.environ.get("FN2_BP64_MIN", "96")):
        ring = 384 <= blocks <= int(os.environ.get("FN2_RING_MAX", "512"))
        return f"2, 2, 2, 1, 3, 1, {m16}" if ring else f"2, 2, 2, 1, 2, 1, {m16}"
    return f"2, 2, 2, 2, 2, 1, {m16}"


_TNAME = {"f32": "float", "bf16": "__bf16", "f16": "_Float16", "f16x2": "fn2::x2_t"}


def _round_up(x, m):
    return (x + m - 1) // m * m


class BatchTooLarge(ValueError):

    def __init__(self, name, batch, nbytes, limit):
        self.fit = max(1, int(batch * (limit - 1) // nbytes))
        super().__init__("activation tensor %s of a batch of %d pairs is %d bytes (limit %d): at most %d pairs per engine"
                         % (name, batch, nbytes, limit, self.fit))


class Engine:
    MAX_TENSOR_BYTES = 1 << 31

    def __init__(self, model, weights, batch, height, width, dtype="f32", device=None, heads_as_gemm=True,
                 no_deconv_biases=None, strict=True, uint8_inputs=False, plain_stems=False, fragment_weights=None,
                 interp_u8_inputs=False):
        if model not in netdefs.MODELS:
            raise ValueError("unknown model %r" % model)
        if dtype not in _DT:
            raise ValueError("dtype must be 'f32', 'bf16', 'f16' or 'f16x2'")
        if height % 64 or width % 64:
            raise ValueError("height and width must be multiples of 64 (pad with Net.adapt_x, net.py:373-388)")
        self.lib = _hip.lib()
        self.device = device if device is not None else _hip.require_device()
        self.model, self.N, self.H, self.W = model, int(batch), int(height), int(width)
        self.dtype_name, self.tdtype = dtype, _DT[dtype]
        self.act_code = _CODE[dtype]
        self.code_of = {}
        self.weights = weights
        if no_deconv_biases is None:
            no_deconv_biases = "FlowNetS/predict_flow6/biases" not in weights
        self.no_deconv_biases = bool(no_deconv_biases)
        self.consumed = set()
        self.ignored_variables = []
        self.ops = []
        self.kernel_of = []
        self.branch_of = []
        self._branch = 0
        self.desc_branch = []
        self.syncs = []
        self._lanes_on = bool(int(os.environ.get("FN2_BRANCHES", "1")))
        default_mask = 0b10011 if model == "FlowNet2" else (0b10101 if model == "FlowNetSD" else 0b10001)
        self._lane_mask = int(os.environ.get("FN2_LANE_MASK", str(default_mask)))
        self.keep = []
        self.bufs = {}
        self.layer_flops = []
        self.layer_bytes = []
        self.layer_io_bytes = []
        self.in_a = torch.zeros((self.N, self.H, self.W, 3), dtype=torch.float32, device=self.device)
        self.in_b = torch.zeros_like(self.in_a)
        self.uint8_inputs = bool(uint8_inputs)
        if self.uint8_inputs:
            self.in_a_u8 = torch.zeros((self.N, self.H, self.W, 3), dtype=torch.uint8, device=self.device)
            self.in_b_u8 = torch.zeros_like(self.in_a_u8)
            self._lut_div = torch.from_numpy((np.arange(256, dtype=np.float64) / 255.0).astype(np.float32)).to(self.device)
            self._lut_raw = torch.arange(256, dtype=torch.float32, device=self.device)
            self._lut = [self._lut_div.clone(), self._lut_div.clone()]
            self._lut_mode = [True, True]
            cnt = self.in_a_u8.numel()
            for src, lut, dst, nm in ((self.in_a_u8, self._lut[0], self.in_a, "a"), (self.in_b_u8, self._lut[1], self.in_b, "b")):
                self.kernel_of.append("u8_to_f32_lut_kernel")
                self.ops.append((f"input_{nm}/u8_to_f32", self.lib.fn2_u8_to_f32_lut,
                                 (_hip.ptr(src), _hip.ptr(lut), _hip.ptr(dst), cnt)))
                self.branch_of.append(0)
        self.interp_u8_inputs = bool(interp_u8_inputs)
        if self.interp_u8_inputs:
            if model != "FlowNetS_interp":
                raise ValueError("interp_u8_inputs belongs to FlowNetS_interp, not %s" % model)
            self.in_img_u8 = torch.zeros((self.N, self.H, self.W, 3), dtype=torch.uint8, device=self.device)
            self.in_mask_u8 = torch.zeros((self.N, self.H, self.W), dtype=torch.uint8, device=self.device)
            self.in_sparse = torch.zeros((self.N, self.H, self.W, 2), dtype=torch.float32, device=self.device)
            self.in_flags = torch.ones((self.N, 2), dtype=torch.uint8, device=self.device)
            self._lut_255 = torch.from_numpy((np.arange(256, dtype=np.float64) / 255.0).astype(np.float32)).to(self.device)
        self.graph = None
        self.conv_descs = []
        self.layers = []
        self.heads_as_gemm = heads_as_gemm
        self.plain_stems = bool(plain_stems)
        self.fragment_weights = bool(int(os.environ.get("FN2_WREG", "1"))) if fragment_weights is None else bool(fragment_weights)
        self.compose_heads = bool(heads_as_gemm) and dtype == "f16x2" and bool(int(os.environ.get("FN2_COMPOSE", "1")))
        self._head_t = None
        self._defer_flow = False
        self._own_ws = set()
        self._pending_head = None
        self.outputs = self._build()
        assert self._pending_head is None
        self._check_variables(strict)
        self._alloc_workspace()
        self._resolve_kernel_names()

    def _buf(self, name, n, h, w, c, dtype=None, stem=False):
        line = 64 if self.act_code in (_hip.FN2_BF16, _hip.FN2_F16) else 32
        cs = (_round_up(c, line) if c > 32 else _round_up(c, 8)) if dtype is None else c
        if dtype is None and not stem and line == 32 and 8 < c <= 32:
            cs = 32

        td = self.tdtype if dtype is None else dtype
        nbytes = n * h * w * cs * torch.empty((), dtype=td).element_size()
        if nbytes >= self.MAX_TENSOR_BYTES:
            if self.N <= 1:
                raise ValueError("one %d x %d pair needs a %d-byte tensor (%s): above the %d-byte limit of the kernels"
                                 % (self.H, self.W, nbytes, name, self.MAX_TENSOR_BYTES))
            raise BatchTooLarge(name, self.N, nbytes, self.MAX_TENSOR_BYTES)
        t = torch.zeros((n, h, w, cs), dtype=td, device=self.device)
        assert name not in self.bufs, name
        self.bufs[name] = t
        self.code_of[t.data_ptr()] = self.act_code if dtype is None else _hip.FN2_F32
        return t

    def _code(self, buf):
        base = buf.untyped_storage().data_ptr()
        return self.code_of.get(buf.data_ptr(), self.code_of.get(base, _hip.dtype_code(buf)))

    def _v(self, buf, c=None, c0=0):
        return _hip.view(buf, c, c0, self._code(buf))

    def _w(self, key):
        if key not in self.weights:
            raise KeyError("the weights lack %r, a variable of the reference's %s graph" % (key, self.model))
        self.consumed.add(key)
        return self.weights[key]

    def _bias(self, scope, name, kind, cout):
        key = f"{scope}/{name}/biases"
        if not netdefs.has_bias(self.model, name, kind, self.no_deconv_biases):
            if key in self.weights:
                self.ignored_variables.append(key)
            return None
        b = np.asarray(self._w(key), np.float32).reshape(-1)
        if b.shape[0] != cout:
            raise ValueError("%s has %d entries, the layer has %d outputs" % (key, b.shape[0], cout))
        return W.to_device(b, torch.float32, self.device)

    _SLOT_SUFFIXES = ("/Adam", "/Adam_1", "/Momentum", "/ExponentialMovingAverage")

    def _check_variables(self, strict):
        roots = tuple(sorted({scope.split("/")[0] + "/" for scope, _ in netdefs.model_scopes(self.model)}))
        stray = [k for k in self.weights
                 if k.startswith(roots) and k not in self.consumed and k not in self.ignored_variables
                 and not k.endswith(self._SLOT_SUFFIXES)]
        if self.ignored_variables:
            import warnings
            warnings.warn("%s: %d bias tensors of the checkpoint belong to layers the reference graph builds without "
                          "biases and are ignored, as the reference ignores them (first: %s)"
                          % (self.model, len(self.ignored_variables), self.ignored_variables[0]))
        if stray and strict:
            raise ValueError("%s: %d checkpoint variables are read by no layer (first: %s); pass strict=False to "
                             "ignore them" % (self.model, len(stray), ", ".join(sorted(stray)[:4])))
        self.stray_variables = stray

    def _sync(self, waiter, waited):
        if waiter != waited:
            self.syncs.append((len(self.ops), waiter, waited))

    def _lane(self, lane):
        eng = self

        class _L:
            def __enter__(self_):
                self_.prev = eng._branch
                eng._branch = lane if (eng._lanes_on and (eng._lane_mask >> lane) & 1) else self_.prev

            def __exit__(self_, *exc):
                eng._branch = self_.prev
        return _L()

    def _head_lane(self):
        hd = self._branch + 2
        return hd if (self._lanes_on and self._branch in (0, 1) and (self._lane_mask >> hd) & 1) else self._branch

    def _op(self, name, fn, *args, kernel=None):
        self.kernel_of.append(kernel if kernel is not None else fn.__name__.replace("fn2_", ""))
        self.ops.append((name, fn, args))
        self.branch_of.append(self._branch)

    def _conv(self, scope, spec, src, dst, up=None, up_after=None, defer_head=False):
        name, kind, k, stride, pad, cin, cout, act = spec
        sbuf, sc0, sc = src
        dbuf, dc0, dc = dst
        assert sc == cin and dc == cout, (scope, name, sc, cin, dc, cout)
        head_px = dbuf.shape[0] * dbuf.shape[1] * dbuf.shape[2]
        if (self.heads_as_gemm and kind == "conv" and cout == 2 and k == 3 and stride == 1 and pad == 1 and not act
                and dbuf.dtype == torch.float32 and head_px >= int(os.environ.get("FN2_HEAD_GEMM_MIN", "8192"))
                and self._head_gemm(scope, spec, src, dst, up)):
            return up is not None and bool(int(os.environ.get("FN2_FUSE_UPFLOW", "1")))
        wname = f"{scope}/{name}/weights"
        in_code = self._code(sbuf)
        esz = 2 if in_code in (_hip.FN2_BF16, _hip.FN2_F16) else 4
        cin_pad = _round_up(cin, 8)
        cin_line = _round_up(cin, 128 // esz)
        if sc0 + cin_line <= sbuf.shape[3] and _hip.conv_plan(in_code, cin_line, cout).layout == 1:
            cin_pad = cin_line
        plan = _hip.conv_plan(in_code, cin_pad, cout)
        tile, layout = plan.cout_tile, plan.layout
        merged = (kind != "conv" and self.compose_heads and cout == 16 and in_code == _hip.FN2_F16X2 and layout == 1
                  and tile == 32 and sbuf.shape[2] % 128 == 0 and bool(int(os.environ.get("FN2_DECONV_MERGED", "1"))))
        if kind == "conv":
            packed, cin_pad, cout_pad, kpad = W.pack_conv(self._w(wname), tile, plan.kstep_elems, cin_pad, layout)
        elif merged:
            packed, cin_pad, cout_pad, kpad = W.pack_deconv_merged(self._w(wname), tile, plan.kstep_elems, cin_pad, layout)
        else:
            packed, cin_pad, cout_pad, kpad = W.pack_deconv(self._w(wname), tile, plan.kstep_elems, cin_pad, layout)
        bias = self._bias(scope, name, kind, cout)
        out_scale = 1.0
        if plan.wgt_dtype == _hip.FN2_F16X2:
            wmax = float(abs(packed).max())
            if wmax > 0:
                k2 = int(math.floor(math.log2(1024.0 / wmax)))
                packed = packed * (2.0 ** k2)
                out_scale = 2.0 ** (-k2)
        wdev = W.packed_to_device(packed, plan.wgt_dtype, self.device)
        d = _hip.Fn2ConvDesc()
        d.inp = self._v(sbuf, sc, sc0)
        d.out = self._v(dbuf, dc, dc0)
        d.wgt = wdev.data_ptr()
        d.bias = bias.data_ptr() if bias is not None else None
        d.kind = 0 if kind == "conv" else (5 if merged else 1)
        d.kh = d.kw = k
        d.stride, d.pad = stride, pad
        d.act = _hip.ACT_LEAKY if act else _hip.ACT_NONE
        d.cin_pad, d.cout_pad, d.kpad = cin_pad, cout_pad, kpad
        d.wgt_layout = layout
        d.out_scale = out_scale
        frag = False
        if (self.fragment_weights and layout == 1 and tile >= int(os.environ.get("FN2_WREG_TILE_MIN", "128"))
                and plan.wgt_dtype == _hip.FN2_F16X2 and self._wants_fragments(d)):
            wdev = W.to_fragment_order(wdev)
            d.wgt, d.wgt_layout, frag = wdev.data_ptr(), 2, True
        self.keep += [d, wdev, bias]
        self.conv_descs.append(d)
        self.desc_branch.append(self._branch)
        up_rec = None
        if self._pending_head is not None and kind != "conv":
            hd = self._pending_head
            assert up_after is not None and hd.inp.data == d.inp.data and hd.inp.c0 == d.inp.c0, (scope, name)
            d.head = C.addressof(hd)
            self._pending_head = None
        if up_after is not None:
            assert kind != "conv" and (not merged or cout == 16)
            up_name, up_src, (ubuf, uc0, uc) = up_after
            assert ubuf is dbuf and uc == 2
            uw = W.to_device(self._w(f"{scope}/{up_name}/weights"), torch.float32, self.device)
            ub = self._bias(scope, up_name, "deconv", 2)
            d.up_src, d.up_w, d.up_bias, d.up_c0 = up_src.data_ptr(), uw.data_ptr(), (ub.data_ptr() if ub is not None else None), uc0
            uv = self._v(ubuf, uc, uc0)
            self.keep += [uw, ub, uv]
            up_rec = dict(scope=scope, name=up_name, kind="upflow", src=up_src, dst=up_after[2], w=uw, b=ub, view=uv)
        self.layers.append(dict(scope=scope, name=name, kind=d.kind, k=k, stride=stride, pad=pad, cin=cin, cout=cout,
                                act=bool(act), src=src, dst=dst, desc=d, w=wdev, b=bias, cin_pad=cin_pad,
                                cout_pad=cout_pad, kpad=kpad, layout=layout, tile=tile, kstep=plan.kstep_elems, frag=frag))
        if up_rec is not None:
            self.layers.append(up_rec)
        tn = _TNAME[self.dtype_name] if in_code == self.act_code else "float"
        if kind == "conv" and cout == 2 and k == 3 and stride == 1 and pad == 1:
            kern = f"flow_head_kernel<{tn}>"
        elif layout == 1:
            on = _TNAME[self.dtype_name] if self._code(dbuf) == self.act_code else "float"
            m_px = dbuf.shape[0] * dbuf.shape[1] * dbuf.shape[2] // (4 if kind != "conv" else 1)
            kern = f"conv_igemm2_kernel<{tn}, {on}, {conv2_kernel_args(tile, m_px, cout_pad, 4 if kind != 'conv' else 1, tn == 'fn2::x2_t')}>"
        else:
            shape = {128: "4, 2, 2", 64: "4, 1, 4", 32: "2, 1, 4", 16: "1, 1, 4"}[tile]
            on = _TNAME[self.dtype_name] if self._code(dbuf) == self.act_code else "float"
            kern = f"conv_igemm_kernel<{tn}, {on}, {shape}>"
        if defer_head and kern.startswith("flow_head_kernel"):
            assert self._pending_head is None
            self._pending_head = d
        else:
            self._op(f"{scope}/{name}", self.lib.fn2_conv2d, C.byref(d), kernel=kern)
        n, oh, ow = dbuf.shape[0], dbuf.shape[1], dbuf.shape[2]
        taps = k * k if kind == "conv" else 4
        self.layer_flops.append((f"{scope}/{name}", 2.0 * n * oh * ow * taps * cin * cout))
        osz = 4 if dbuf.dtype == torch.float32 else 2
        self.layer_io_bytes.append((f"{scope}/{name}", float(sbuf.shape[0] * sbuf.shape[1] * sbuf.shape[2] * cin * esz
                                                            + n * oh * ow * cout * osz + k * k * cin * cout * esz)))

    def _head_slabs(self, d, head_t, t_cs):
        need = int(self.lib.fn2_conv2d_workspace_bytes(C.byref(d)))
        if need <= 0 or not int(os.environ.get("FN2_HEAD_SLABS", "1")):
            return _hip.ptr(head_t), t_cs, 1, 0, 1.0
        ws = torch.empty((need + 3) // 4, dtype=torch.float32, device=self.device)
        d.workspace, d.workspace_bytes, d.raw_partials = ws.data_ptr(), need, 1
        self.keep.append(ws)
        self._own_ws.add(C.addressof(d))
        splits = int(self.lib.fn2_conv2d_splits(C.byref(d)))
        if splits <= 1:
            d.raw_partials = 0
            return _hip.ptr(head_t), t_cs, 1, 0, 1.0
        ws_cs = (d.out.c + 3) // 4 * 4
        return ws.data_ptr(), ws_cs, splits, d.out.n * d.out.h * d.out.w * ws_cs, float(d.out_scale) or 1.0

    def _wants_fragments(self, d):
        need = int(self.lib.fn2_conv2d_workspace_bytes(C.byref(d)))
        d.workspace, d.workspace_bytes = (1, need) if need else (None, 0)
        buf = C.create_string_buffer(256)
        rc = self.lib.fn2_conv2d_kernel_name(C.byref(d), buf, 256)
        d.workspace, d.workspace_bytes = None, 0
        which = os.environ.get("FN2_WREG_KERNELS", "false>")
        return rc == 0 and buf.value.decode().startswith("conv_igemm2_kernel") and buf.value.decode().endswith(which)

    def _head_gemm(self, scope, spec, src, dst, up=None):
        name, kind, k, stride, pad, cin, cout, act = spec
        sbuf, sc0, sc = src
        pf = dst[0]
        in_code = self._code(sbuf)
        esz = 2 if in_code in (_hip.FN2_BF16, _hip.FN2_F16) else 4
        cin_line = _round_up(cin, 128 // esz)
        if sc0 + cin_line > sbuf.shape[3]:
            return False
        plan = _hip.conv_plan(in_code, cin_line, 18)
        if plan.layout != 1:
            return False
        w = np.asarray(self._w(f"{scope}/{name}/weights"), np.float32)
        w1 = np.ascontiguousarray(w.transpose(2, 0, 1, 3)).reshape(1, 1, cin, 18)
        packed, cin_pad, cout_pad, kpad = W.pack_conv(w1, plan.cout_tile, plan.kstep_elems, cin_line, plan.layout)
        out_scale = 1.0
        if plan.wgt_dtype == _hip.FN2_F16X2:
            wmax = float(abs(packed).max())
            if wmax > 0:
                k2 = int(math.floor(math.log2(1024.0 / wmax)))
                packed, out_scale = packed * (2.0 ** k2), 2.0 ** (-k2)
        wdev = W.packed_to_device(packed, plan.wgt_dtype, self.device)
        bias = self._bias(scope, name, kind, cout)
        if self._head_t is None:
            self._head_t = {}
        if self._branch not in self._head_t:
            self._head_t[self._branch] = torch.zeros((self.N * self.H * self.W, 32), dtype=torch.float32, device=self.device)
        head_t = self._head_t[self._branch]
        n, h, wd = pf.shape[0], pf.shape[1], pf.shape[2]
        d = _hip.Fn2ConvDesc()
        d.inp = self._v(sbuf, sc, sc0)
        d.out = _hip.Fn2Tensor(head_t.data_ptr(), _hip.FN2_F32, n, h, wd, 18, 32, 0)
        d.wgt, d.bias = wdev.data_ptr(), None
        d.kind, d.kh, d.kw, d.stride, d.pad = 0, 1, 1, 1, 0
        d.act = _hip.ACT_NONE
        d.cin_pad, d.cout_pad, d.kpad, d.wgt_layout = cin_pad, cout_pad, kpad, plan.layout
        d.out_scale = out_scale
        self.keep += [d, wdev, bias]
        self.conv_descs.append(d)
        self.desc_branch.append(self._branch)
        tn = _TNAME[self.dtype_name] if in_code == self.act_code else "float"
        self._op(f"{scope}/{name}", self.lib.fn2_conv2d, C.byref(d),
                 kernel=f"conv_igemm2_kernel<{tn}, float, {conv2_kernel_args(plan.cout_tile, 0, cout_pad, 1, tn == 'fn2::x2_t')}>")
        t_ptr, t_cs, nslab, slab, tscale = self._head_slabs(d, head_t, 32)
        if up is not None and int(os.environ.get("FN2_FUSE_UPFLOW", "1")):
            up_name, (ubuf, uc0, uc) = up
            uw = W.to_device(self._w(f"{scope}/{up_name}/weights"), torch.float32, self.device)
            ub = self._bias(scope, up_name, "deconv", 2)
            uv = self._v(ubuf, uc, uc0)
            self.keep += [uw, ub, uv]
            self.layers.append(dict(scope=scope, name=up_name, kind="upflow", src=pf, dst=up[1], w=uw, b=ub, view=uv))
            self._op(f"{scope}/{name}/tail+{up_name}", self.lib.fn2_flow_head_tail_slabs, t_ptr, t_cs, nslab, slab,
                     C.c_float(tscale), 3, _hip.ptr(bias) if bias is not None else None, _hip.ptr(pf), n, h, wd, 0, _hip.ptr(uw),
                     _hip.ptr(ub) if ub is not None else None, C.byref(uv), kernel="flow_head_tail")
        else:
            self._op(f"{scope}/{name}/tail", self.lib.fn2_flow_head_tail_slabs, t_ptr, t_cs, nslab, slab, C.c_float(tscale), 3,
                     _hip.ptr(bias) if bias is not None else None, _hip.ptr(pf), n, h, wd, 0, None, None, None,
                     kernel="flow_head_tail")
        self.layer_flops.append((f"{scope}/{name}", 2.0 * n * h * wd * 9 * cin * 2))
        self.layer_io_bytes.append((f"{scope}/{name}", float(n * h * wd * (cin * esz + 2 * 4) + 18 * cin * esz)))
        return True

    def _composed_head(self, scope, ic_spec, pf_spec, src, pf, up=None):
        sbuf, sc0, sc = src
        in_code = self._code(sbuf)
        if in_code != _hip.FN2_F16X2 or sc0 % 8 or sbuf.shape[1] < 3 or sbuf.shape[2] < 3:
            return False
        cin_line = _round_up(sc, 32)
        if sc0 + cin_line > sbuf.shape[3]:
            return False
        plan = _hip.conv_plan(in_code, cin_line, 50)
        if plan.layout != 1:
            return False
        ic_name, pf_name = ic_spec[0], pf_spec[0]
        w1, w2 = self._w(f"{scope}/{ic_name}/weights"), self._w(f"{scope}/{pf_name}/weights")
        b1 = self._w(f"{scope}/{ic_name}/biases") if netdefs.has_bias(self.model, ic_name, "conv", self.no_deconv_biases) else None
        b2 = self._w(f"{scope}/{pf_name}/biases") if netdefs.has_bias(self.model, pf_name, "conv", self.no_deconv_biases) else None
        w5, bias5 = W.compose_interconv_head(w1, b1, w2, b2)
        n, h, wd = pf.shape[0], pf.shape[1], pf.shape[2]
        groups = (sc + 7) // 8
        wc = np.zeros((9, 25, groups * 8, 2), np.float32)
        wc[:, :, :sc, :] = w5.reshape(9, 25, sc, 2)
        wcd = W.to_device(wc, torch.float32, self.device)
        bcd = W.to_device(bias5.astype(np.float32), torch.float32, self.device)
        vin = self._v(sbuf, sc, sc0)
        self.keep += [wcd, bcd, vin]
        w1x1 = np.ascontiguousarray(w5[4].transpose(2, 0, 1, 3)).reshape(1, 1, sc, 50).astype(np.float32)
        packed, cin_pad, cout_pad, kpad = W.pack_conv(w1x1, plan.cout_tile, plan.kstep_elems, cin_line, plan.layout)
        out_scale = 1.0
        wmax = float(abs(packed).max())
        if wmax > 0:
            k2 = int(math.floor(math.log2(1024.0 / wmax)))
            packed, out_scale = packed * (2.0 ** k2), 2.0 ** (-k2)
        wdev = W.packed_to_device(packed, plan.wgt_dtype, self.device)
        cm = ic_spec[6]
        if n * h * wd >= int(os.environ.get("FN2_HEAD5_MIN", "65536")) and plan.cout_tile == 64 and kpad == cin_pad:
            b5 = W.to_device(bias5[4].astype(np.float32), torch.float32, self.device)
            vx = self._v(sbuf, sc, sc0)
            self.keep += [wdev, b5, vx]
            strip = cin_pad in (96, 192) and int(os.environ.get("FN2_H5_STRIP", "1"))
            self._op(f"{scope}/{ic_name}+{pf_name}", self.lib.fn2_flow_head5, C.byref(vx), _hip.ptr(wdev), cin_pad, kpad,
                     C.c_float(out_scale), _hip.ptr(b5), _hip.ptr(pf), 1, _hip.ptr(wcd), _hip.ptr(bcd),
                     kernel=("head5_strip_kernel<%d>" % (cin_pad // 96)) if strip else
                     "conv_igemm2_kernel<fn2::x2_t, float, 1, 4, 2, 2, 2, 1, false, false, false, true>")
            self.layer_flops.append((f"{scope}/{ic_name}+{pf_name}", 2.0 * n * h * wd * 9 * (sc * cm + cm * 2)))
            self.layer_io_bytes.append((f"{scope}/{ic_name}+{pf_name}", float(n * h * wd * (sc * 4 + 2 * 4) + 9 * (sc * cm + 2 * cm) * 4)))
            return 1
        self._op(f"{scope}/{pf_name}/ring", self.lib.fn2_flow_head_ring, C.byref(vin), _hip.ptr(wcd), _hip.ptr(bcd), _hip.ptr(pf),
                 kernel="flow_head_ring")
        if self._head_t is None:
            self._head_t = {}
        key = (self._branch, 64)
        if key not in self._head_t:
            self._head_t[key] = torch.zeros((self.N * self.H * self.W, 64), dtype=torch.float32, device=self.device)
        head_t = self._head_t[key]
        d = _hip.Fn2ConvDesc()
        d.inp = self._v(sbuf, sc, sc0)
        d.out = _hip.Fn2Tensor(head_t.data_ptr(), _hip.FN2_F32, n, h, wd, 50, 64, 0)
        d.wgt, d.bias = wdev.data_ptr(), None
        d.kind, d.kh, d.kw, d.stride, d.pad = 0, 1, 1, 1, 0
        d.act = _hip.ACT_NONE
        d.cin_pad, d.cout_pad, d.kpad, d.wgt_layout = cin_pad, cout_pad, kpad, plan.layout
        d.out_scale = out_scale
        b5 = W.to_device(bias5[4].astype(np.float32), torch.float32, self.device)
        self.keep += [d, wdev, b5]
        self.conv_descs.append(d)
        self.desc_branch.append(self._branch)
        self._op(f"{scope}/{ic_name}+{pf_name}", self.lib.fn2_conv2d, C.byref(d), kernel="conv_igemm2_kernel (composed head)")
        t_ptr, t_cs, nslab, slab, tscale = self._head_slabs(d, head_t, 64)
        if up is not None:
            up_name, (ubuf, uc0, uc) = up
            uw = W.to_device(self._w(f"{scope}/{up_name}/weights"), torch.float32, self.device)
            ub = self._bias(scope, up_name, "deconv", 2)
            uv = self._v(ubuf, uc, uc0)
            self.keep += [uw, ub, uv]
            self.layers.append(dict(scope=scope, name=up_name, kind="upflow", src=pf, dst=up[1], w=uw, b=ub, view=uv))
            self._op(f"{scope}/{pf_name}/tail+{up_name}", self.lib.fn2_flow_head_tail_slabs, t_ptr, t_cs, nslab, slab,
                     C.c_float(tscale), 5, _hip.ptr(b5), _hip.ptr(pf), n, h, wd, 1, _hip.ptr(uw),
                     _hip.ptr(ub) if ub is not None else None, C.byref(uv), kernel="flow_head_tail")
        else:
            self._op(f"{scope}/{pf_name}/tail", self.lib.fn2_flow_head_tail_slabs, t_ptr, t_cs, nslab, slab, C.c_float(tscale), 5,
                     _hip.ptr(b5), _hip.ptr(pf), n, h, wd, 1, None, None, None, kernel="flow_head_tail")
        self.layer_flops.append((f"{scope}/{ic_name}+{pf_name}", 2.0 * n * h * wd * 9 * (sc * cm + cm * 2)))
        self.layer_io_bytes.append((f"{scope}/{ic_name}+{pf_name}", float(n * h * wd * (sc * 4 + 2 * 4) + 9 * (sc * cm + 2 * cm) * 4)))
        return 2 if up is not None else 1

    def _conv_stem(self, scope, spec, sbuf, dst, s2d=False):
        name, kind, k, stride, pad, cin, cout, act = spec
        dbuf, dc0, dc = dst
        assert kind == "conv" and dc == cout
        k_alg, cin_alg = k, cin
        w_hwio = self._w(f"{scope}/{name}/weights")
        if s2d:
            assert stride == 2 and cin == 3 and sbuf.shape[3] == 16
            k2 = (k + 1) // 2
            w = np.zeros((k2, k2, 16, cout), np.float32)
            for ky in range(k):
                for kx in range(k):
                    w[ky // 2, kx // 2, ((ky & 1) * 2 + (kx & 1)) * 4:((ky & 1) * 2 + (kx & 1)) * 4 + 3] = w_hwio[ky, kx]
            w_hwio, k, stride, cin = w, k2, 1, 16
        cs = sbuf.shape[3]
        in_code = self._code(sbuf)
        esz = 2 if in_code in (_hip.FN2_BF16, _hip.FN2_F16) else 4
        run = _round_up(k * cs, 128 // esz)
        plan = _hip.conv_plan(in_code, run, cout)
        assert plan.layout == 1, (scope, name)
        packed, cin_pad, cout_pad, kpad = W.pack_stem(w_hwio, cs, run, plan.cout_tile, plan.layout)
        bias = self._bias(scope, name, kind, cout)
        out_scale = 1.0
        if plan.wgt_dtype == _hip.FN2_F16X2:
            k2 = int(math.floor(math.log2(1024.0 / float(abs(packed).max()))))
            packed, out_scale = packed * (2.0 ** k2), 2.0 ** (-k2)
        wdev = W.packed_to_device(packed, plan.wgt_dtype, self.device)
        d = _hip.Fn2ConvDesc()
        d.inp = self._v(sbuf, cs, 0)
        d.out = self._v(dbuf, dc, dc0)
        d.wgt = wdev.data_ptr()
        d.bias = bias.data_ptr() if bias is not None else None
        d.kind = 2
        d.kh = d.kw = k
        d.stride, d.pad = stride, 0
        d.act = _hip.ACT_LEAKY if act else _hip.ACT_NONE
        d.cin_pad, d.cout_pad, d.kpad = cin_pad, cout_pad, kpad
        d.wgt_layout = plan.layout
        d.out_scale = out_scale
        self.keep += [d, wdev, bias]
        self.conv_descs.append(d)
        self.desc_branch.append(self._branch)
        self.layers.append(dict(scope=scope, name=name, kind=2, k=k, stride=stride, pad=pad, cin=cin, cout=cout,
                                act=bool(act), src=(sbuf, 0, cs), dst=dst, desc=d, w=wdev, b=bias, cin_pad=cin_pad,
                                cout_pad=cout_pad, kpad=kpad, layout=plan.layout, tile=plan.cout_tile,
                                kstep=plan.kstep_elems, cs=cs))
        tn = _TNAME[self.dtype_name]
        self._op(f"{scope}/{name}", self.lib.fn2_conv2d, C.byref(d),
                 kernel=f"conv_igemm2_kernel<{tn}, {tn}, {conv2_kernel_args(plan.cout_tile, 0, cout_pad, 1, tn == 'fn2::x2_t')}>")
        n, oh, ow = dbuf.shape[0], dbuf.shape[1], dbuf.shape[2]
        self.layer_flops.append((f"{scope}/{name}", 2.0 * n * oh * ow * k_alg * k_alg * cin_alg * cout))
        self.layer_io_bytes.append((f"{scope}/{name}", float(sbuf.numel() * esz + n * oh * ow * cout * esz
                                                            + k_alg * k_alg * cin_alg * cout * esz)))

    def _upflow(self, scope, name, src_f32, dst):
        dbuf, dc0, dc = dst
        w = W.to_device(self._w(f"{scope}/{name}/weights"), torch.float32, self.device)
        b = self._bias(scope, name, "deconv", 2)
        v = self._v(dbuf, dc, dc0)
        self.keep += [w, v, b]
        n, h, wd, _ = src_f32.shape
        self.layers.append(dict(scope=scope, name=name, kind="upflow", src=src_f32, dst=dst, w=w, b=b, view=v))
        self._op(f"{scope}/{name}", self.lib.fn2_upsample_flow, _hip.ptr(src_f32), _hip.ptr(w),
                 _hip.ptr(b) if b is not None else None, C.byref(v), n, h, wd)

    def _resize(self, name, src_f32, scale):
        n, h, w, c = src_f32.shape
        dst = self._buf(name, n, self.H, self.W, 2, torch.float32)
        self._op(name, self.lib.fn2_resize_bilinear_f32, _hip.ptr(src_f32), _hip.ptr(dst), n, h, w, c, self.H,
                 self.W, C.c_float(scale))
        return dst

    def _resolve_kernel_names(self):
        buf = C.create_string_buffer(256)
        for i, (name, fn, args) in enumerate(self.ops):
            if fn is self.lib.fn2_conv2d:
                if self.lib.fn2_conv2d_kernel_name(args[0], buf, 256) == 0 and buf.value:
                    self.kernel_of[i] = buf.value.decode()

    def _alloc_workspace(self):
        branches = self.desc_branch + [0] * (len(self.conv_descs) - len(self.desc_branch))
        self.workspace = {}
        for br in sorted(set(branches)):
            descs = [d for d, b in zip(self.conv_descs, branches) if b == br and C.addressof(d) not in self._own_ws]
            need = max([int(self.lib.fn2_conv2d_workspace_bytes(C.byref(d))) for d in descs] + [0])
            if need > 0:
                self.workspace[br] = torch.empty((need + 3) // 4, dtype=torch.float32, device=self.device)
                for d in descs:
                    d.workspace = self.workspace[br].data_ptr()
                    d.workspace_bytes = need

    def _refine(self, scope, tag, L, c6_1, cats, interconv):
        N = c6_1.shape[0]
        preds = {}
        M, Hd = self._branch, self._head_lane()
        h, w = c6_1.shape[1], c6_1.shape[2]
        pf = self._buf(f"{tag}/predict_flow6", N, h, w, 2, torch.float32)
        self._sync(Hd, M)
        skips, decs = (512, 512, 256, 128), (512, 256, 128, 64)
        ride_heads = (Hd == M and self.heads_as_gemm and self.dtype_name == "f16x2"
                      and bool(int(os.environ.get("FN2_UP_IN_DECONV", "1"))) and bool(int(os.environ.get("FN2_HEAD_IN_DECONV", "1"))))
        with self._lane(Hd):
            fused = self._conv(scope, L["predict_flow6"], (c6_1, 0, 1024), (pf, 0, 2),
                               up=("upsample_flow6to5", (cats[5], skips[0] + decs[0], 2)), defer_head=ride_heads)
        preds["predict_flow6"] = pf
        cur, cur_c = c6_1, 1024
        for i, (lvl, skip_c, dec_c) in enumerate(zip((5, 4, 3, 2), skips, decs)):
            cat = cats[lvl]
            h, w = cat.shape[1], cat.shape[2]
            ride = (not fused and Hd == M and self._code(cat) == self.act_code
                    and bool(int(os.environ.get("FN2_UP_IN_DECONV", "1"))))
            self._conv(scope, L[f"deconv{lvl}"], (cur, 0, cur_c), (cat, skip_c, dec_c),
                       up_after=(f"upsample_flow{lvl + 1}to{lvl}", pf, (cat, skip_c + dec_c, 2)) if ride else None)
            if not fused and not ride:
                with self._lane(Hd):
                    self._upflow(scope, f"upsample_flow{lvl + 1}to{lvl}", pf, (cat, skip_c + dec_c, 2))
            self._sync(M, Hd)
            if not interconv:
                self._sync(Hd, M)
            cur, cur_c = cat, skip_c + dec_c + 2
            head_src = (cat, 0, cur_c)
            pf = self._buf(f"{tag}/predict_flow{lvl}", N, h, w, 2, torch.float32)
            up = None
            if lvl > 2:
                up = (f"upsample_flow{lvl}to{lvl - 1}", (cats[lvl - 1], skips[i + 1] + decs[i + 1], 2))
            if interconv and self.compose_heads:
                self._sync(Hd, M)
                with self._lane(Hd):
                    composed = self._composed_head(scope, L[f"interconv{lvl}"], L[f"predict_flow{lvl}"], head_src, pf, up=up)
                if composed:
                    fused = composed == 2
                    preds[f"predict_flow{lvl}"] = pf
                    continue
            if interconv:
                ic = self._buf(f"{tag}/interconv{lvl}", N, h, w, dec_c)
                self._conv(scope, L[f"interconv{lvl}"], (cat, 0, cur_c), (ic, 0, dec_c))
                self._sync(Hd, M)
                head_src = (ic, 0, dec_c)
            with self._lane(Hd):
                fused = self._conv(scope, L[f"predict_flow{lvl}"], head_src, (pf, 0, 2), up=up,
                                   defer_head=ride_heads and lvl > 2 and not interconv)
            preds[f"predict_flow{lvl}"] = pf
        return preds

    def _final_flow(self, tag, preds, scale):
        M, Hd = self._branch, self._head_lane()
        if self._defer_flow:
            preds["flow"] = self._buf(f"{tag}/flow", self.N, self.H, self.W, 2, torch.float32)
            preds["_flow_src"] = (preds["predict_flow2"], scale)
            self._sync(M, Hd)
            return preds
        with self._lane(Hd):
            preds["flow"] = self._resize(f"{tag}/flow", preds["predict_flow2"], scale)
        self._sync(M, Hd)
        return preds

    def _alloc_cats(self, tag, N):
        H, W_ = self.H, self.W
        return {5: self._buf(f"{tag}/concat5", N, H // 32, W_ // 32, 1026),
                4: self._buf(f"{tag}/concat4", N, H // 16, W_ // 16, 770),
                3: self._buf(f"{tag}/concat3", N, H // 8, W_ // 8, 386),
                2: self._buf(f"{tag}/concat2", N, H // 4, W_ // 4, 194)}

    def _encoder_tail(self, scope, tag, L, cats):
        N, H, W_ = self.N, self.H, self.W
        c4 = self._buf(f"{tag}/conv4", N, H // 16, W_ // 16, 512)
        self._conv(scope, L["conv4"], (cats[3], 0, 256), (c4, 0, 512))
        self._conv(scope, L["conv4_1"], (c4, 0, 512), (cats[4], 0, 512))
        c5 = self._buf(f"{tag}/conv5", N, H // 32, W_ // 32, 512)
        self._conv(scope, L["conv5"], (cats[4], 0, 512), (c5, 0, 512))
        self._conv(scope, L["conv5_1"], (c5, 0, 512), (cats[5], 0, 512))
        c6 = self._buf(f"{tag}/conv6", N, H // 64, W_ // 64, 1024)
        self._conv(scope, L["conv6"], (cats[5], 0, 512), (c6, 0, 1024))
        c6_1 = self._buf(f"{tag}/conv6_1", N, H // 64, W_ // 64, 1024)
        self._conv(scope, L["conv6_1"], (c6, 0, 1024), (c6_1, 0, 1024))
        return c6_1

    def _net_s(self, scope, tag, x, cin):
        N, H, W_ = self.N, self.H, self.W
        L = {s[0]: s for s in netdefs.flownet_s_layers(cin)}
        cats = self._alloc_cats(tag, N)
        c1 = self._buf(f"{tag}/conv1", N, H // 2, W_ // 2, 64)
        self._conv_stem(scope, L["conv1"], x, (c1, 0, 64))
        self._conv(scope, L["conv2"], (c1, 0, 64), (cats[2], 0, 128))
        c3 = self._buf(f"{tag}/conv3", N, H // 8, W_ // 8, 256)
        self._conv(scope, L["conv3"], (cats[2], 0, 128), (c3, 0, 256))
        self._conv(scope, L["conv3_1"], (c3, 0, 256), (cats[3], 0, 256))
        c6_1 = self._encoder_tail(scope, tag, L, cats)
        preds = self._refine(scope, tag, L, c6_1, cats, False)
        return self._final_flow(tag, preds, 20.0)

    def _net_c(self, scope, tag):
        N, H, W_ = self.N, self.H, self.W
        L = {s[0]: s for s in netdefs.flownet_c_layers()}
        cats = self._alloc_cats(tag, N)
        batch_towers = os.environ.get("FN2_C_TOWERS", "lane") == "batch"
        if batch_towers:
            del self.bufs[f"{tag}/concat2"]
            cat2_all = self._buf(f"{tag}/concat2", 2 * N, H // 4, W_ // 4, 194)
            cats[2] = cat2_all[:N]
        c1 = self._buf(f"{tag}/conv1", 2 * N, H // 2, W_ // 2, 64)
        if self.plain_stems:
            x2 = self._buf(f"{tag}/images", 2 * N, H + 6, W_ + 6, 3, stem=True)
            v = self._v(x2, 3, 0)
            self.keep.append(v)
            self._op(f"{tag}/pack_a", self.lib.fn2_pack_image, _hip.ptr(self.in_a), N, C.byref(v), 0, 3)
            self._op(f"{tag}/pack_b", self.lib.fn2_pack_image, _hip.ptr(self.in_b), N, C.byref(v), N, 3)
            self._conv_stem(scope, L["conv1"], x2, (c1, 0, 64))
        else:
            x2 = self._buf(f"{tag}/images", 2 * N, (H + 6) // 2, (W_ + 6) // 2, 16, stem=True)
            v = self._v(x2, 16, 0)
            self.keep.append(v)
            self._op(f"{tag}/pack_a", self.lib.fn2_pack_image_s2d, _hip.ptr(self.in_a), N, H, W_, C.byref(v), 0, 3)
            self._op(f"{tag}/pack_b", self.lib.fn2_pack_image_s2d, _hip.ptr(self.in_b), N, H, W_, C.byref(v), N, 3)
            self._conv_stem(scope, L["conv1"], x2, (c1, 0, 64), s2d=True)
        M, T = self._branch, (4 if (self._lanes_on and self._lane_mask & 16 and not batch_towers) else self._branch)
        if batch_towers:
            self._conv(scope, L["conv2"], (c1, 0, 64), (cat2_all, 0, 128))
            c3 = self._buf(f"{tag}/conv_ab_3", 2 * N, H // 8, W_ // 8, 256)
            self._conv(scope, L["conv3"], (cat2_all, 0, 128), (c3, 0, 256))
            c3a, c3b = c3[:N], c3[N:]
        else:
            c2b = self._buf(f"{tag}/conv_b_2", N, H // 4, W_ // 4, 128)
            self._sync(T, M)
            self._conv(scope, L["conv2"], (c1[:N], 0, 64), (cats[2], 0, 128))
            with self._lane(T):
                self._conv(scope, L["conv2"], (c1[N:], 0, 64), (c2b, 0, 128))
            c3a = self._buf(f"{tag}/conv_a_3", N, H // 8, W_ // 8, 256)
            c3b = self._buf(f"{tag}/conv_b_3", N, H // 8, W_ // 8, 256)
            self._conv(scope, L["conv3"], (cats[2], 0, 128), (c3a, 0, 256))
            with self._lane(T):
                self._conv(scope, L["conv3"], (c2b, 0, 128), (c3b, 0, 256))
            self._sync(M, T)
            self._sync(T, M)
        net = self._buf(f"{tag}/corr_concat", N, H // 8, W_ // 8, 473)
        va, vb, vo = self._v(c3a, 256, 0), self._v(c3b, 256, 0), self._v(net, 441, 32)
        self.keep += [va, vb, vo]
        tn = _TNAME[self.dtype_name]
        self._op(f"{tag}/correlation", self.lib.fn2_correlation_fused, C.byref(va), C.byref(vb), C.byref(vo), 20, 2,
                 _hip.ACT_LEAKY, kernel=self._corr_kernel_name(tn, H // 8))
        self.layers.append(dict(scope=scope, name="correlation", kind="corr", fa=c3a, fb=c3b, dst=(net, 32, 441)))
        self.layer_flops.append((f"{scope}/correlation", 2.0 * N * (H // 8) * (W_ // 8) * 441 * 256))
        self.layer_bytes.append((f"{tag}/correlation", 4.0 * N * (H // 8) * (W_ // 8) * (2 * 256 + 441)))
        with self._lane(T):
            self._conv(scope, L["conv_redir"], (c3a, 0, 256), (net, 0, 32))
        self._sync(M, T)
        self._conv(scope, L["conv3_1"], (net, 0, 473), (cats[3], 0, 256))
        c6_1 = self._encoder_tail(scope, tag, L, cats)
        preds = self._refine(scope, tag, L, c6_1, cats, False)
        return self._final_flow(tag, preds, 20.0)

    def _net_sd(self, scope, tag, x):
        N, H, W_ = self.N, self.H, self.W
        L = {s[0]: s for s in netdefs.flownet_sd_layers()}
        cats = self._alloc_cats(tag, N)
        c0 = self._buf(f"{tag}/conv0", N, H, W_, 64)
        self._conv_stem(scope, L["conv0"], x, (c0, 0, 64))
        c1 = self._buf(f"{tag}/conv1", N, H // 2, W_ // 2, 64)
        self._conv(scope, L["conv1"], (c0, 0, 64), (c1, 0, 64))
        c1_1 = self._buf(f"{tag}/conv1_1", N, H // 2, W_ // 2, 128)
        self._conv(scope, L["conv1_1"], (c1, 0, 64), (c1_1, 0, 128))
        self._conv(scope, L["conv2"], (c1_1, 0, 128), (cats[2], 0, 128))
        c2_1 = self._buf(f"{tag}/conv2_1", N, H // 4, W_ // 4, 128)
        self._conv(scope, L["conv2_1"], (cats[2], 0, 128), (c2_1, 0, 128))
        c3 = self._buf(f"{tag}/conv3", N, H // 8, W_ // 8, 256)
        self._conv(scope, L["conv3"], (c2_1, 0, 128), (c3, 0, 256))
        self._conv(scope, L["conv3_1"], (c3, 0, 256), (cats[3], 0, 256))
        c6_1 = self._encoder_tail(scope, tag, L, cats)
        preds = self._refine(scope, tag, L, c6_1, cats, True)
        return self._final_flow(tag, preds, 0.05)

    def _corr_kernel_name(self, tn, h):
        nl = 4 if self.dtype_name in ("bf16", "f16") else 8
        if self.dtype_name != "f32" and h % 4 == 0 and int(os.environ.get("FN2_CORR3", "1")):
            return f"corr3_kernel<{tn}, {tn}, {nl}>"
        return f"corr2_kernel<{tn}, {tn}, {nl}>"

    def _pair_input(self, tag, pad):
        x = self._buf(f"{tag}/pair", self.N, self.H + 2 * pad, self.W + 2 * pad, 6, stem=True)
        v = self._v(x, 6, 0)
        self.keep.append(v)
        if self.interp_u8_inputs:
            self._op(f"{tag}/pack_interp_u8", self.lib.fn2_pack_interp_u8, _hip.ptr(self.in_img_u8), _hip.ptr(self.in_mask_u8),
                     _hip.ptr(self.in_sparse), _hip.ptr(self._lut_255), _hip.ptr(self.in_flags), C.byref(v), pad)
            return x
        self._op(f"{tag}/pack_pair", self.lib.fn2_pack_pair, _hip.ptr(self.in_a), _hip.ptr(self.in_b), C.byref(v), pad)
        return x

    def _stacked_input(self, tag, preds):
        x = self._buf(f"{tag}/stack", self.N, self.H + 6, self.W + 6, 16, stem=True)
        v = self._v(x, 12, 0)
        self.keep.append(v)
        if "_flow_src" in preds:
            pf2, scale = preds["_flow_src"]
            self._op(f"{tag}/stack_input", self.lib.fn2_stack_input_pf, _hip.ptr(self.in_a), _hip.ptr(self.in_b), _hip.ptr(pf2),
                     pf2.shape[1], pf2.shape[2], C.c_float(scale), _hip.ptr(preds["flow"]), C.byref(v), 3, kernel="stack_input")
        else:
            self._op(f"{tag}/stack_input", self.lib.fn2_stack_input, _hip.ptr(self.in_a), _hip.ptr(self.in_b),
                     _hip.ptr(preds["flow"]), C.byref(v), 3)
        return x

    def _sub(self, build, *args):
        prev, self._defer_flow = self._defer_flow, bool(int(os.environ.get("FN2_FLOW_IN_CONSUMER", "1")))
        try:
            return build(*args)
        finally:
            self._defer_flow = prev

    def _net_cs(self, scope, tag):
        pc = self._sub(self._net_c, scope + "/FlowNetC", tag + "/C")
        return self._net_s(scope + "/FlowNetS", tag + "/S", self._stacked_input(tag + "/S", pc), 12)

    def _net_css(self, scope, tag):
        pcs = self._sub(self._net_cs, scope + "/FlowNetCS", tag + "/CS")
        return self._net_s(scope + "/FlowNetS", tag + "/S", self._stacked_input(tag + "/S", pcs), 12)

    def _net_2(self, scope, tag):
        N, H, W_ = self.N, self.H, self.W
        fork = len(self.ops)
        css = self._sub(self._net_css, scope + "/FlowNetCSS", tag + "/CSS")
        if self._lanes_on and self._lane_mask & 2:
            fork += min(int(os.environ.get("FN2_SD_FORK_OPS", "0")), len(self.ops) - fork)
            self.syncs.append((fork, 1, 0))
            if self._lane_mask & 8 and int(os.environ.get("FN2_FORK3", "1")):
                self.syncs.append((fork, 3, 0))
        with self._lane(1):
            sd = self._sub(self._net_sd, scope + "/FlowNetSD", tag + "/SD", self._pair_input(tag + "/SD", 1))
        if self._lanes_on and self._lane_mask & 2:
            self._sync(0, 1)
        L = {s[0]: s for s in netdefs.fusion_layers()}
        xf = self._buf(f"{tag}/fusion_in", N, H + 2, W_ + 2, 16, stem=True)
        v = self._v(xf, 11, 0)
        self.keep.append(v)
        if "_flow_src" in sd and "_flow_src" in css:
            (pf_sd, s_sd), (pf_css, s_css) = sd["_flow_src"], css["_flow_src"]
            self._op(f"{tag}/fusion_input", self.lib.fn2_fusion_input_pf, _hip.ptr(self.in_a), _hip.ptr(self.in_b),
                     _hip.ptr(pf_sd), C.c_float(s_sd), _hip.ptr(sd["flow"]), _hip.ptr(pf_css), C.c_float(s_css),
                     _hip.ptr(css["flow"]), pf_sd.shape[1], pf_sd.shape[2], C.byref(v), 1, kernel="fusion_input")
        else:
            self._op(f"{tag}/fusion_input", self.lib.fn2_fusion_input, _hip.ptr(self.in_a), _hip.ptr(self.in_b),
                     _hip.ptr(sd["flow"]), _hip.ptr(css["flow"]), C.byref(v), 1)
        cat0 = self._buf(f"{tag}/concat0", N, H, W_, 82)
        cat1 = self._buf(f"{tag}/concat1", N, H // 2, W_ // 2, 162)
        self._conv_stem(scope, L["fuse_conv0"], xf, (cat0, 0, 64))
        f1 = self._buf(f"{tag}/fuse_conv1", N, H // 2, W_ // 2, 64)
        self._conv(scope, L["fuse_conv1"], (cat0, 0, 64), (f1, 0, 64))
        self._conv(scope, L["fuse_conv1_1"], (f1, 0, 64), (cat1, 0, 128))
        f2 = self._buf(f"{tag}/fuse_conv2", N, H // 4, W_ // 4, 128)
        self._conv(scope, L["fuse_conv2"], (cat1, 0, 128), (f2, 0, 128))
        f2_1 = self._buf(f"{tag}/fuse_conv2_1", N, H // 4, W_ // 4, 128)
        self._conv(scope, L["fuse_conv2_1"], (f2, 0, 128), (f2_1, 0, 128))
        pf2 = self._buf(f"{tag}/predict_flow2", N, H // 4, W_ // 4, 2, torch.float32)
        M, Hd = self._branch, self._head_lane()
        self._sync(Hd, M)
        with self._lane(Hd):
            fused = self._conv(scope, L["predict_flow2"], (f2_1, 0, 128), (pf2, 0, 2),
                               up=("fuse_upsample_flow2to1", (cat1, 160, 2)))
        self._conv(scope, L["fuse_deconv1"], (f2_1, 0, 128), (cat1, 128, 32))
        if not fused:
            with self._lane(Hd):
                self._upflow(scope, "fuse_upsample_flow2to1", pf2, (cat1, 160, 2))
        self._sync(M, Hd)
        pf1 = self._buf(f"{tag}/predict_flow1", N, H // 2, W_ // 2, 2, torch.float32)
        fused, composed = None, 0
        if self.compose_heads:
            self._sync(Hd, M)
            with self._lane(Hd):
                composed = self._composed_head(scope, L["fuse_interconv1"], L["predict_flow1"], (cat1, 0, 162), pf1,
                                               up=("fuse_upsample_flow1to0", (cat0, 80, 2)))
            fused = composed == 2
        if not composed:
            ic1 = self._buf(f"{tag}/fuse_interconv1", N, H // 2, W_ // 2, 32)
            self._conv(scope, L["fuse_interconv1"], (cat1, 0, 162), (ic1, 0, 32))
            self._sync(Hd, M)
            with self._lane(Hd):
                fused = self._conv(scope, L["predict_flow1"], (ic1, 0, 32), (pf1, 0, 2),
                                   up=("fuse_upsample_flow1to0", (cat0, 80, 2)))
        ride0 = (not fused and Hd == M and self.dtype_name == "f16x2" and self.heads_as_gemm
                 and bool(int(os.environ.get("FN2_UP_IN_DECONV", "1"))))
        self._conv(scope, L["fuse_deconv0"], (cat1, 0, 162), (cat0, 64, 16),
                   up_after=("fuse_upsample_flow1to0", pf1, (cat0, 80, 2)) if ride0 else None)
        if not fused and not ride0:
            with self._lane(Hd):
                self._upflow(scope, "fuse_upsample_flow1to0", pf1, (cat0, 80, 2))
        self._sync(M, Hd)
        pf0 = self._buf(f"{tag}/predict_flow0", N, H, W_, 2, torch.float32)
        if not (self.compose_heads and self._composed_head(scope, L["fuse_interconv0"], L["predict_flow0"], (cat0, 0, 82), pf0)):
            ic0 = self._buf(f"{tag}/fuse_interconv0", N, H, W_, 16)
            self._conv(scope, L["fuse_interconv0"], (cat0, 0, 82), (ic0, 0, 16))
            self._conv(scope, L["predict_flow0"], (ic0, 0, 16), (pf0, 0, 2))
        return {"predict_flow0": pf0, "flow": pf0}

    def _build(self):
        m = self.model
        if m in ("FlowNetS", "FlowNetS_interp"):
            return self._net_s("FlowNetS", "S", self._pair_input("S", 3), 6)
        if m == "FlowNetC":
            return self._net_c("FlowNetC", "C")
        if m == "FlowNetSD":
            return self._net_sd("FlowNetSD", "SD", self._pair_input("SD", 1))
        if m == "FlowNetCS":
            return self._net_cs("FlowNetCS", "CS")
        if m == "FlowNetCSS":
            return self._net_css("FlowNetCSS", "CSS")
        return self._net_2("FlowNet2", "F2")

    def set_inputs(self, input_a, input_b):
        for dst, src in ((self.in_a, input_a), (self.in_b, input_b)):
            t = src if isinstance(src, torch.Tensor) else torch.as_tensor(src)
            if tuple(t.shape) != tuple(dst.shape):
                raise ValueError("input shape %s != engine shape %s" % (tuple(t.shape), tuple(dst.shape)))
            dst.copy_(t.to(dtype=torch.float32), non_blocking=True)

    def set_inputs_u8(self, input_a, input_b, scale=(True, True)):
        if not self.uint8_inputs:
            raise ValueError("engine was built without uint8_inputs=True")
        for i, (dst, src) in enumerate(((self.in_a_u8, input_a), (self.in_b_u8, input_b))):
            t = src if isinstance(src, torch.Tensor) else torch.as_tensor(src)
            if t.dtype != torch.uint8:
                raise ValueError("set_inputs_u8 takes uint8 images, got %s" % t.dtype)
            if tuple(t.shape) != tuple(dst.shape):
                raise ValueError("input shape %s != engine shape %s" % (tuple(t.shape), tuple(dst.shape)))
            dst.copy_(t, non_blocking=True)
            if bool(scale[i]) != self._lut_mode[i]:
                self._lut[i].copy_(self._lut_div if scale[i] else self._lut_raw)
                self._lut_mode[i] = bool(scale[i])

    def set_inputs_interp(self, input_a, matches_a, sparse_flow):
        dev = lambda x: (x if isinstance(x, torch.Tensor) else torch.as_tensor(np.asarray(x))).to(
            device=self.device, dtype=torch.float32)
        sf, m = dev(sparse_flow), dev(matches_a)
        if m.ndim == 3:
            m = m[..., None]
        self.set_inputs(dev(input_a), torch.cat([sf * 0.05, m], dim=3))

    def set_inputs_interp_u8(self, input_a, matches_a, sparse_flow, scale_flags):
        if not self.interp_u8_inputs:
            raise ValueError("engine was built without interp_u8_inputs=True")
        as_t = lambda x: x if isinstance(x, torch.Tensor) else torch.as_tensor(np.asarray(x))
        img, m, sf = as_t(input_a), as_t(matches_a), as_t(sparse_flow)
        if img.dtype != torch.uint8 or m.dtype != torch.uint8:
            raise ValueError("set_inputs_interp_u8 takes a uint8 image and mask, got %s and %s" % (img.dtype, m.dtype))
        if sf.dtype != torch.float32:
            raise ValueError("set_inputs_interp_u8 takes a float32 sparse flow, got %s" % sf.dtype)
        if m.ndim == 4 and m.shape[3] == 1:
            m = m[..., 0]
        fl = torch.as_tensor(np.asarray(scale_flags, dtype=bool).astype(np.uint8))
        if fl.ndim == 1:
            fl = fl.expand(self.N, 2)
        for dst, src in ((self.in_img_u8, img), (self.in_mask_u8, m), (self.in_sparse, sf), (self.in_flags, fl)):
            if tuple(src.shape) != tuple(dst.shape):
                raise ValueError("input shape %s != engine shape %s" % (tuple(src.shape), tuple(dst.shape)))
            dst.copy_(src, non_blocking=True)

    def launch(self):
        if self.graph is not None:
            _hip.check(self.lib.fn2_graph_launch(self.graph, _hip.stream_ptr()))
            return
        s = _hip.stream_ptr()
        for name, fn, args in self.ops:
            rc = fn(*args, s)
            if rc:
                try:
                    _hip.check(rc)
                except Exception as e:
                    raise type(e)("%s: %s" % (name, e)) from None

    def capture(self):
        if self.graph is not None:
            return
        side = torch.cuda.Stream(device=self.device)
        side.wait_stream(torch.cuda.current_stream())
        extra = {b: torch.cuda.Stream(device=self.device) for b in sorted(set(self.branch_of) - {0})}
        with torch.cuda.stream(side):
            self.launch()
            side.synchronize()
            _hip.check(self.lib.fn2_capture_begin(_hip.stream_ptr()))
            try:
                if not extra:
                    self.launch()
# ... 88 lines not shown
```

include/flownet2_hip.h:

```cpp
#ifndef FLOWNET2_HIP_H_
#define FLOWNET2_HIP_H_

#include <stddef.h>
#include <stdint.h>

#ifdef __cplusplus
extern "C" {
#endif

typedef enum {
  FN2_OK = 0,
  FN2_ERR_INVALID_ARGUMENT = -1,
  FN2_ERR_UNSUPPORTED = -2,
  FN2_ERR_HIP = -3
} fn2_status;

typedef enum { FN2_F32 = 0, FN2_BF16 = 1, FN2_F16 = 2, FN2_F16X2 = 3 } fn2_dtype;

typedef enum { FN2_ACT_NONE = 0, FN2_ACT_LEAKY = 1  } fn2_act;

typedef struct {
  void* data;
  int32_t dtype;
  int32_t n, h, w;
  int32_t c;
  int32_t cs;
  int32_t c0;
} fn2_tensor;

const char* fn2_last_error(void);
int fn2_version(void);
uint32_t fn2_crc32c(const void* data, int64_t n, uint32_t crc);
int fn2_device_info(char* name, int cap, int* cus);


int fn2_correlation_out_shape(int h, int w, int kernel_size, int max_displacement, int stride_1,
                              int stride_2, int pad, int* out_h, int* out_w, int* out_c);

int fn2_correlation_f32(const float* a, const float* b, float* out, int n, int h, int w, int c,
                        int kernel_size, int max_displacement, int stride_1, int stride_2, int pad,
                        void* stream);
int64_t fn2_correlation_workspace_bytes(int n, int h, int w, int c, int kernel_size, int max_displacement, int stride_1,
                                        int stride_2, int pad);
int fn2_correlation_f32_ws(const float* a, const float* b, float* out, int n, int h, int w, int c, int kernel_size,
                           int max_displacement, int stride_1, int stride_2, int pad, void* workspace,
                           int64_t workspace_bytes, void* stream);

int fn2_correlation_grad_f32(const float* grad_out, const float* a, const float* b, float* grad_a,
                             float* grad_b, int n, int h, int w, int c, int kernel_size,
                             int max_displacement, int stride_1, int stride_2, int pad, void* stream);

int fn2_flow_warp_f32(const float* image, const float* flow, float* out, int n, int h, int w, int c,
                      void* stream);

int fn2_flow_warp_grad_f32(const float* image, const float* flow, const float* grad_out,
                           float* image_grad, float* flow_grad, int n, int h, int w, int c,
                           void* stream);

int fn2_downsample_f32(const float* in, float* out, int n, int in_h, int in_w, int c, int out_h,
                       int out_w, void* stream);

int fn2_downsample_scaled_f32(const float* in, float in_scale, float* out, int n, int in_h, int in_w, int c, int out_h,
                              int out_w, void* stream);

int fn2_resize_bilinear_f32(const float* in, float* out, int n, int in_h, int in_w, int c, int out_h,
                            int out_w, float scale, void* stream);


typedef struct {
  fn2_tensor in;
  fn2_tensor out;
  const void* wgt;
  const float* bias;
  int32_t kind;
  int32_t kh, kw, stride, pad;
  int32_t act;
  int32_t cin_pad;
  int32_t cout_pad;
  int32_t kpad;
  int32_t wgt_layout;
  int32_t accumulate;
  float out_scale;
  void* workspace;
  int64_t workspace_bytes;
  const void* act_grad_y;
  int32_t act_grad_c0, act_grad_c1;
  const float* up_src;
  const float* up_w;
  const float* up_bias;
  int32_t up_c0;
  const void* head;
  int32_t raw_partials;
} fn2_conv_desc;

typedef struct {
  int32_t layout, cout_tile, kstep_elems, wgt_dtype;
} fn2_conv_plan;
int fn2_conv2d_plan(int in_dtype, int cin_pad, int cout, fn2_conv_plan* plan);
int64_t fn2_conv2d_workspace_bytes(const fn2_conv_desc* d);
int fn2_conv2d(const fn2_conv_desc* d, void* stream);
int fn2_conv2d_kernel_name(const fn2_conv_desc* desc, char* name, int cap);
int fn2_conv2d_splits(const fn2_conv_desc* desc);

int fn2_flow_head_gather(const float* t, int t_cs, const float* bias, float* out, int n, int h, int w, void* stream);
int fn2_flow_head_tail(const float* t, int t_cs, int taps, const float* bias, float* pf, int n, int h, int w, int ring,
                       const float* up_w, const float* up_bias, const fn2_tensor* up_out, void* stream);
int fn2_flow_head_tail_slabs(const float* t, int t_cs, int nslab, int64_t slab_stride, float scale, int taps, const float* bias,
                             float* pf, int n, int h, int w, int ring, const float* up_w, const float* up_bias,
                             const fn2_tensor* up_out, void* stream);
int fn2_flow_head5(const fn2_tensor* x, const void* wgt, int cin_pad, int kpad, float out_scale, const float* bias, float* pf,
                   int ring, const float* ring_w, const float* ring_b, void* stream);
int fn2_flow_head_ring(const fn2_tensor* x, const float* wc, const float* bc, float* pf, void* stream);
int fn2_upsample_flow(const float* in, const float* w, const float* bias, const fn2_tensor* out, int n, int h, int wd,
                      void* stream);

int fn2_u8_to_f32_lut(const unsigned char* src, const float* lut256, float* dst, long count, void* stream);

int fn2_pack_pair(const float* a, const float* b, const fn2_tensor* out, int pad, void* stream);
int fn2_pack_interp_u8(const unsigned char* img, const unsigned char* mask, const float* sparse, const float* lut256,
                       const unsigned char* flags, const fn2_tensor* out, int pad, void* stream);
int fn2_pack_image(const float* img, int n_img, const fn2_tensor* out, int n0, int pad, void* stream);
int fn2_pack_image_s2d(const float* img, int n_img, int h, int w, const fn2_tensor* out, int n0, int pad, void* stream);

int fn2_correlation_fused(const fn2_tensor* a, const fn2_tensor* b, const fn2_tensor* out,
                          int max_displacement, int stride_2, int act, void* stream);

int fn2_stack_input(const float* a, const float* b, const float* flow, const fn2_tensor* out, int pad,
                    void* stream);

int fn2_fusion_input(const float* a, const float* b, const float* flow_sd, const float* flow_css,
                     const fn2_tensor* out, int pad, void* stream);
int fn2_stack_input_pf(const float* a, const float* b, const float* pf, int pf_h, int pf_w, float scale, float* flow_out,
                       const fn2_tensor* out, int pad, void* stream);
int fn2_fusion_input_pf(const float* a, const float* b, const float* pf_sd, float scale_sd, float* flow_sd_out,
                        const float* pf_css, float scale_css, float* flow_css_out, int pf_h, int pf_w,
                        const fn2_tensor* out, int pad, void* stream);


int fn2_epe_loss_grad(const float* pred, const float* label, float* dpred, float* loss_accum, int n, int h, int w,
                      float weight, float grad_mult, void* stream);
int fn2_epe_loss_grad_weighted(const float* pred, const float* label, const float* pixel_weight, float* dpred,
                               float* loss_accum, int n, int h, int w, float weight, float grad_mult, void* stream);
int fn2_leaky_bwd(const fn2_tensor* y, const fn2_tensor* g, float* db, void* stream);
int fn2_bias_grad(const fn2_tensor* g, float* db, void* stream);
int fn2_to_f16x2(void* dst, const float* src, const int32_t* map, int64_t n, float scale, void* stream);
int fn2_to_f16x2_frag(void* dst, const float* src, const int32_t* map, int64_t n, float scale, int k, void* stream);
int fn2_fill_zero(void* dst, int64_t bytes, void* stream);
int fn2_add_f32(float* dst, const float* src, int64_t n, void* stream);
int fn2_slice_copy_f32(const fn2_tensor* src, float* dst, void* stream);
int fn2_gather_f32(float* dst, const float* src, const int32_t* map, int64_t n, void* stream);
int fn2_adam_step(float* w, float* m, float* v, const float* g, int64_t n, float lr, float beta1, float beta2,
                  float eps, int step, float l2, float grad_scale, void* stream);
int fn2_adam_step_multi(const void* table, const int64_t* counts, const float* l2, int n_tensors, float lr, float beta1,
                        float beta2, float eps, int step, float grad_scale, void* stream);
int fn2_adam_step_multi_dev(const void* table, const int64_t* counts, const float* l2, int n_tensors, const float* hyper,
                            void* stream);
int fn2_upsample_flow_bwd(const fn2_tensor* g, const float* pf, const float* w, float* dpf, float* dw,
                          int accumulate, void* stream);
int fn2_head_bwd_filter(const fn2_tensor* x, const float* g, float* dw, int cin_pad, int kpad, void* stream);
int fn2_head_bwd_data(const float* g, const float* w, const fn2_tensor* dx, int cin_pad, int kpad, void* stream);

typedef struct {
  fn2_tensor x;
  fn2_tensor dy;
  float* dw;
  int32_t kind, kh, kw, stride, pad;
  int32_t cin_pad, cout_pad, kpad, wgt_layout;
  float* db;
} fn2_bwdw_desc;
int fn2_conv2d_bwd_filter(const fn2_bwdw_desc* d, void* stream);
int fn2_head_g18(const float* g, const fn2_tensor* out, void* stream);

int fn2_augment_f32(const float* src, const float* transforms, const float* chromatic, float* out, int n, int src_h,
                    int src_w, int c, int out_h, int out_w, void* stream);
int fn2_flow_augmentation_f32(const float* flows, const float* transforms_from_a, const float* inv_transforms_from_b,
                              float* out, int n, int src_h, int src_w, int out_h, int out_w, void* stream);

int64_t fn2_variational_workspace_bytes(int n, int h, int w);
int fn2_variational_refine(const uint8_t* img_a, const uint8_t* img_b, int64_t img_pitch, int64_t img_bstride,
                           float* flow, int64_t flow_pitch, int64_t flow_bstride, int n, int h, int w, float alpha,
                           float gamma, float delta, float sigma, int niter_outer, int niter_inner, int niter_solver,
                           float sor_omega, void* workspace, int64_t ws_bytes, void* stream);

int fn2_capture_begin(void* stream);
int fn2_capture_end(void* stream, void** graph_exec);
int fn2_graph_launch(void* graph_exec, void* stream);
int fn2_graph_destroy(void* graph_exec);

#ifdef __cplusplus
}
#endif
#endif
```

Baseline: 1112 pairs/s.

## Pair CSS and SD encoder-tail convolutions into one grouped split-K launch

Adds a paired-conv path that runs the matching conv4..conv6_1 layers of FlowNetCSS and FlowNetSD in a single launch. blockIdx.z phase selects which problem's input, weights and workspace slab a block uses, and one finalize kernel reduces both problems. The aim is to fill the GPU on these small, low-occupancy late encoder layers and halve their launch and finalize count, instead of relying on two streams overlapping. In exchange the SD branch must synchronise with the CSS lane at each paired step, the workspace must hold twice the slabs, and the split-K planning moves earlier so the head-ride check uses the adjusted split.

```diff
diff --git a/flownet2-tf_amd/csrc/conv.hip b/flownet2-tf_amd/csrc/conv.hip
--- a/flownet2-tf_amd/csrc/conv.hip
+++ b/flownet2-tf_amd/csrc/conv.hip
@@ -216,19 +216,30 @@
   }
 }
 
+struct FinalizePair {
+  const float* ws; const float* bias; void* out; int out_cs, out_c0; float out_scale;
+};
 template <typename OutT>
-__global__ void __launch_bounds__(256) splitk_finalize_kernel(const float* __restrict__ ws, const float* __restrict__ bias,
-                                                              OutT* __restrict__ out, long npix, int ws_cs, int splitk,
-                                                              int Cout, int out_cs, int out_c0, int act, int vec_ok,
-                                                              float out_scale, int accum, const OutT* __restrict__ mask_y,
+__global__ void __launch_bounds__(256) splitk_finalize_kernel(const float* __restrict__ ws_a, const float* __restrict__ bias_a,
+                                                              OutT* __restrict__ out_a, long npix, int ws_cs, int splitk,
+                                                              int Cout, int out_cs_a, int out_c0_a, int act, int vec_ok,
+                                                              float out_scale_a, int accum, const OutT* __restrict__ mask_y,
                                                               int mask_c0, int mask_c1, const float* __restrict__ up_src,
                                                               const float* __restrict__ up_w, const float* __restrict__ up_bias,
-                                                              int up_c0, int out_H, int out_W) {
+                                                              int up_c0, int out_H, int out_W, const FinalizePair p2) {
   const int groups = ws_cs / 4;
   const int groups_all = groups + (up_src != nullptr ? 1 : 0);
-  const long total = npix * groups_all;
+  const long total1 = npix * groups_all;
+  const long total = p2.ws != nullptr ? 2 * total1 : total1;
   const size_t slab = (size_t)npix * ws_cs;
-  for (long i = (long)blockIdx.x * blockDim.x + threadIdx.x; i < total; i += (long)gridDim.x * blockDim.x) {
+  for (long i0 = (long)blockIdx.x * blockDim.x + threadIdx.x; i0 < total; i0 += (long)gridDim.x * blockDim.x) {
+    const bool second = i0 >= total1;
+    const long i = second ? i0 - total1 : i0;
+    const float* ws = second ? p2.ws : ws_a;
+    const float* bias = second ? p2.bias : bias_a;
+    OutT* out = second ? reinterpret_cast<OutT*>(p2.out) : out_a;
+    const int out_cs = second ? p2.out_cs : out_cs_a, out_c0 = second ? p2.out_c0 : out_c0_a;
+    const float out_scale = second ? p2.out_scale : out_scale_a;
     const long pix = i / groups_all;
     const int co = (int)(i - pix * groups_all) * 4;
     if (co == groups * 4) {
@@ -1161,6 +1172,12 @@
   if (d->up_src != nullptr && d->kind == 5 && 2 * d->out.c == 32) {
     a.up_src = d->up_src; a.up_w = d->up_w; a.up_bias = d->up_bias; a.up_c0 = d->up_c0;
   }
+  if (d->wgt_layout >= 1) {
+    a.ksteps = a.ksteps / 2;
+    a.kper = cdiv(a.kper, 2);
+    a.splitk = cdiv(a.ksteps, a.kper);
+    if (a.splitk == 1) a.ws = nullptr;
+  }
   if (d->head != nullptr && !conv_name_sink().buf) {
     const fn2_conv_desc* h = reinterpret_cast<const fn2_conv_desc*>(d->head);
     FN2_REQUIRE(d->kind == 1 && is_flow_head(h) && h->head == nullptr && h->up_src == nullptr,
@@ -1173,7 +1190,7 @@
     rc = build_args(h, &ha, &htile, &hphases);
     if (rc) return rc;
     const char* e = getenv("FN2_HEAD_RIDE");
-    const bool ride = d->in.dtype == FN2_F16X2 && d->wgt_layout == 2 && tile == 128 && sk > 1 && !(e && atoi(e) == 0);
+    const bool ride = d->in.dtype == FN2_F16X2 && d->wgt_layout == 2 && tile == 128 && a.splitk > 1 && !(e && atoi(e) == 0);
     if (ride) {
       a.fh_M = ha.M;
       a.fh_w = reinterpret_cast<const float*>(ha.wgt);
@@ -1189,10 +1206,6 @@
     }
   }
   if (d->wgt_layout >= 1) {
-    a.ksteps = a.ksteps / 2;
-    a.kper = cdiv(a.kper, 2);
-    a.splitk = cdiv(a.ksteps, a.kper);
-    if (a.splitk == 1) a.ws = nullptr;
     rc = launch_conv_fast(a, d->in.dtype, d->out.dtype, tile, phases, s);
   } else if (d->in.dtype == FN2_F32 && d->out.dtype == FN2_F16X2) rc = launch_conv<float, x2_t>(a, tile, phases, s);
   else if (d->in.dtype == FN2_F32) rc = launch_conv<float, float>(a, tile, phases, s);
@@ -1212,18 +1225,129 @@
   const int fgrid = grid_for(npix * (a.ws_cs / 4 + (d->up_src != nullptr ? 1 : 0)), 256);
   if (d->out.dtype == FN2_F32)
     hipLaunchKernelGGL(splitk_finalize_kernel<float>, dim3(fgrid), dim3(256), 0, s, a.ws, a.bias, (float*)a.out, npix,
-                       a.ws_cs, a.splitk, a.Cout, a.out_cs, a.out_c0, a.act, a.vec_ok, a.out_scale, a.accum, (const float*)a.mask_y, a.mask_c0, a.mask_c1, d->up_src, d->up_w, d->up_bias, d->up_c0, a.out_H, a.out_W);
+                       a.ws_cs, a.splitk, a.Cout, a.out_cs, a.out_c0, a.act, a.vec_ok, a.out_scale, a.accum, (const float*)a.mask_y, a.mask_c0, a.mask_c1, d->up_src, d->up_w, d->up_bias, d->up_c0, a.out_H, a.out_W, FinalizePair{});
   else if (d->out.dtype == FN2_F16X2)
     hipLaunchKernelGGL(splitk_finalize_kernel<x2_t>, dim3(fgrid), dim3(256), 0, s, a.ws, a.bias, (x2_t*)a.out,
-                       npix, a.ws_cs, a.splitk, a.Cout, a.out_cs, a.out_c0, a.act, a.vec_ok, a.out_scale, a.accum, (const x2_t*)a.mask_y, a.mask_c0, a.mask_c1, d->up_src, d->up_w, d->up_bias, d->up_c0, a.out_H, a.out_W);
+                       npix, a.ws_cs, a.splitk, a.Cout, a.out_cs, a.out_c0, a.act, a.vec_ok, a.out_scale, a.accum, (const x2_t*)a.mask_y, a.mask_c0, a.mask_c1, d->up_src, d->up_w, d->up_bias, d->up_c0, a.out_H, a.out_W, FinalizePair{});
   else if (d->out.dtype == FN2_BF16)
     hipLaunchKernelGGL(splitk_finalize_kernel<bf16_t>, dim3(fgrid), dim3(256), 0, s, a.ws, a.bias, (bf16_t*)a.out,
-                       npix, a.ws_cs, a.splitk, a.Cout, a.out_cs, a.out_c0, a.act, a.vec_ok, a.out_scale, a.accum, (const bf16_t*)a.mask_y, a.mask_c0, a.mask_c1, d->up_src, d->up_w, d->up_bias, d->up_c0, a.out_H, a.out_W);
+                       npix, a.ws_cs, a.splitk, a.Cout, a.out_cs, a.out_c0, a.act, a.vec_ok, a.out_scale, a.accum, (const bf16_t*)a.mask_y, a.mask_c0, a.mask_c1, d->up_src, d->up_w, d->up_bias, d->up_c0, a.out_H, a.out_W, FinalizePair{});
   else
     hipLaunchKernelGGL(splitk_finalize_kernel<f16_t>, dim3(fgrid), dim3(256), 0, s, a.ws, a.bias, (f16_t*)a.out,
-                       npix, a.ws_cs, a.splitk, a.Cout, a.out_cs, a.out_c0, a.act, a.vec_ok, a.out_scale, a.accum, (const f16_t*)a.mask_y, a.mask_c0, a.mask_c1, d->up_src, d->up_w, d->up_bias, d->up_c0, a.out_H, a.out_W);
+                       npix, a.ws_cs, a.splitk, a.Cout, a.out_cs, a.out_c0, a.act, a.vec_ok, a.out_scale, a.accum, (const f16_t*)a.mask_y, a.mask_c0, a.mask_c1, d->up_src, d->up_w, d->up_bias, d->up_c0, a.out_H, a.out_W, FinalizePair{});
   FN2_CHECK_LAUNCH("splitk_finalize");
   return FN2_OK;
+}
+
+}
+
+namespace fn2 {
+
+static int pair_plan(const fn2_conv_desc* da, const fn2_conv_desc* db, ConvArgs* a, ConvArgs* b, int* tile_out,
+                     bool preferred, const char** why) {
+  *why = "null descriptor";
+  if (!da || !db) return 0;
+  *why = "both must be kind-0 split-fp16 convolutions on fragment-order weights (wgt_layout 2)";
+  for (const fn2_conv_desc* d : {da, db})
+    if (d->kind != 0 || d->in.dtype != FN2_F16X2 || d->out.dtype != FN2_F16X2 || d->wgt_layout != 2) return 0;
+  *why = "head, up_src, raw_partials, accumulate and act_grad_y do not go with a pair";
+  for (const fn2_conv_desc* d : {da, db})
+    if (d->head || d->up_src || d->raw_partials || d->accumulate || d->act_grad_y) return 0;
+  *why = "the two problems differ in geometry";
+  if (da->in.n != db->in.n || da->in.h != db->in.h || da->in.w != db->in.w || da->in.c != db->in.c ||
+      da->in.cs != db->in.cs || da->in.c0 != db->in.c0 || da->kh != db->kh || da->kw != db->kw ||
+      da->stride != db->stride || da->pad != db->pad || da->out.c != db->out.c || da->out.h != db->out.h ||
+      da->out.w != db->out.w || da->out.n != db->out.n || da->act != db->act || da->cin_pad != db->cin_pad ||
+      da->cout_pad != db->cout_pad || da->kpad != db->kpad)
+    return 0;
+  int tile, phases, tile_b, phases_b;
+  *why = "a descriptor of the pair is not a valid fn2_conv2d descriptor";
+  if (build_args(da, a, &tile, &phases) != FN2_OK || build_args(db, b, &tile_b, &phases_b) != FN2_OK) return 0;
+  *why = "a pair runs on the 128-cout tile";
+  if (tile != 128 || tile_b != 128 || phases != 1 || is_flow_head(da) || is_flow_head(db)) return 0;
+  if (a->vec_ok != b->vec_ok || a->wfrag != b->wfrag || a->wmajor != b->wmajor || a->dbg != b->dbg) return 0;
+  int sk = preferred_split(*a, tile, 2);
+  *why = "the pair's grid takes no K split (or the workspace holds no two slabs per problem)";
+  if (!preferred)
+    while (sk > 1 && (da->workspace == nullptr || 2 * split_bytes(*a, sk) > da->workspace_bytes)) --sk;
+  if ((long)a->N * a->out_H * a->out_W * a->ws_cs >= (1L << 31)) sk = 1;
+  if (sk < 2) return 0;
+  const int K = a->ksteps;
+  int kper = 0;
+  for (;;) {
+    kper = cdiv(K, sk);
+    const int s2 = cdiv(K / 2, cdiv(kper, 2));
+    if (s2 == sk) break;
+    sk = s2;
+  }
+  if (sk < 2) return 0;
+  for (ConvArgs* p : {a, b}) {
+    p->ksteps = K / 2;
+    p->kper = cdiv(kper, 2);
+    p->splitk = sk;
+  }
+  *tile_out = tile;
+  *why = "";
+  return sk;
+}
+
+static int pair_launch(const fn2_conv_desc* da, const fn2_conv_desc* db, hipStream_t s) {
+  ConvArgs a, b;
+  int tile;
+  const char* why;
+  const bool naming = conv_name_sink().buf != nullptr;
+  const int sk = pair_plan(da, db, &a, &b, &tile, false, &why);
+  FN2_REQUIRE(sk >= 2, "conv2d_pair: not an eligible pair: %s", why);
+  a.ws = reinterpret_cast<float*>(da->workspace);
+  a.in2 = b.in; a.wgt2 = b.wgt; a.in_bytes2 = b.in_bytes;
+  a.ws2 = a.ws + (size_t)sk * a.N * a.out_H * a.out_W * a.ws_cs;
+  int rc = launch_conv_fast(a, da->in.dtype, da->out.dtype, tile, 2, s);
+  if (rc || naming) return rc;
+  const long npix = (long)a.N * a.out_H * a.out_W;
+  const int fgrid = grid_for(2 * npix * (a.ws_cs / 4), 256);
+  const FinalizePair p2{a.ws2, b.bias, b.out, b.out_cs, b.out_c0, b.out_scale};
+  hipLaunchKernelGGL(splitk_finalize_kernel<x2_t>, dim3(fgrid), dim3(256), 0, s, a.ws, a.bias, (x2_t*)a.out, npix, a.ws_cs,
+                     sk, a.Cout, a.out_cs, a.out_c0, a.act, a.vec_ok, a.out_scale, 0, (const x2_t*)nullptr, 0, 0,
+                     (const float*)nullptr, (const float*)nullptr, (const float*)nullptr, 0, a.out_H, a.out_W, p2);
+  FN2_CHECK_LAUNCH("splitk_finalize (pair)");
+  return FN2_OK;
+}
+
+}
+
+extern "C" {
+
+int fn2_conv2d_pair_ok(const fn2_conv_desc* a, const fn2_conv_desc* b) {
+  return fn2_conv2d_pair_splits(a, b) >= 2 ? 1 : 0;
+}
+
+int fn2_conv2d_pair_splits(const fn2_conv_desc* da, const fn2_conv_desc* db) {
+  ConvArgs a, b;
+  int tile;
+  const char* why;
+  const int sk = pair_plan(da, db, &a, &b, &tile, false, &why);
+  return sk >= 2 ? sk : 1;
+}
+
+int64_t fn2_conv2d_pair_workspace_bytes(const fn2_conv_desc* da, const fn2_conv_desc* db) {
+  ConvArgs a, b;
+  int tile;
+  const char* why;
+  const int sk = pair_plan(da, db, &a, &b, &tile, true, &why);
+  return sk >= 2 ? 2 * split_bytes(a, sk) : 0;
+}
+
+int fn2_conv2d_pair(const fn2_conv_desc* da, const fn2_conv_desc* db, void* stream) {
+  return pair_launch(da, db, (hipStream_t)stream);
+}
+
+int fn2_conv2d_pair_kernel_name(const fn2_conv_desc* da, const fn2_conv_desc* db, char* name, int cap) {
+  FN2_REQUIRE(name && cap > 0, "conv2d_pair_kernel_name: no buffer");
+  name[0] = 0;
+  conv_name_sink() = ConvNameSink{name, cap};
+  const int rc = pair_launch(da, db, nullptr);
+  conv_name_sink() = ConvNameSink{nullptr, 0};
+  return rc;
 }
 
 int fn2_flow_head_gather(const float* t, int t_cs, const float* bias, float* out, int n, int h, int w, void* stream) {
diff --git a/flownet2-tf_amd/csrc/conv2.hip b/flownet2-tf_amd/csrc/conv2.hip
--- a/flownet2-tf_amd/csrc/conv2.hip
+++ b/flownet2-tf_amd/csrc/conv2.hip
@@ -163,8 +163,15 @@
   const int wc = wave / WP, wp = wave % WP;
 
   int pad_y = p.pad, pad_x = p.pad, oy_off = 0, ox_off = 0, osc = 1;
-  const T* wgt = reinterpret_cast<const T*>(p.wgt);
   const int phase = blockIdx.z / p.splitk, split = blockIdx.z - phase * p.splitk;
+  const void* in_p = p.in;
+  const void* wgt_p = p.wgt;
+  float* ws_p = p.ws;
+  int in_bytes_p = p.in_bytes;
+  if constexpr (WREG && SLAB) {
+    if (p.in2 != nullptr && phase != 0) { in_p = p.in2; wgt_p = p.wgt2; ws_p = p.ws2; in_bytes_p = p.in_bytes2; }
+  }
+  const T* wgt = reinterpret_cast<const T*>(wgt_p);
   const unsigned wrow_bytes = (unsigned)p.ksteps * 128u;
   if (p.deconv) {
     const int a = phase >> 1, b = phase & 1;
@@ -192,7 +199,7 @@
   const int c0 = by * BC;
 
   const v4i_t rsrc_w = make_rsrc(wgt, (int)(p.cout_pad * wrow_bytes));
-  const v4i_t rsrc_x = make_rsrc(p.in, p.in_bytes);
+  const v4i_t rsrc_x = make_rsrc(in_p, in_bytes_p);
 
   const int lrow = lane >> 3, lphys = lane & 7;
   unsigned woff[NWI];
@@ -675,7 +682,7 @@
   constexpr int CPR = WCOLS / 4, RPI = 64 / CPR;
   static_assert(!SLAB || WREG, "SLAB is a specialisation of the WREG instantiations");
   if ((SLAB || !WREG) && p.splitk > 1) {
-    float* slab = p.ws + (size_t)split * p.N * p.out_H * p.out_W * p.ws_cs;
+    float* slab = ws_p + (size_t)split * p.N * p.out_H * p.out_W * p.ws_cs;
     if constexpr (kLdsT) {
       if constexpr (STAGES >= 3) __syncthreads();
       if constexpr (FEED) { if (feeder) return; }
diff --git a/flownet2-tf_amd/csrc/conv_common.h b/flownet2-tf_amd/csrc/conv_common.h
--- a/flownet2-tf_amd/csrc/conv_common.h
+++ b/flownet2-tf_amd/csrc/conv_common.h
@@ -47,6 +47,7 @@
   int ws_cs;
   float out_scale;
   int in_bytes;
+  const void* in2; const void* wgt2; float* ws2; int in_bytes2;
   const void* mask_y;
   int mask_c0, mask_c1;
   int dbg;
diff --git a/flownet2-tf_amd/src/_hip.py b/flownet2-tf_amd/src/_hip.py
--- a/flownet2-tf_amd/src/_hip.py
+++ b/flownet2-tf_amd/src/_hip.py
@@ -66,6 +66,11 @@
     "fn2_conv2d": (_i, [C.POINTER(Fn2ConvDesc), _p]),
     "fn2_conv2d_kernel_name": (_i, [C.POINTER(Fn2ConvDesc), C.c_char_p, _i]),
     "fn2_conv2d_splits": (_i, [C.POINTER(Fn2ConvDesc)]),
+    "fn2_conv2d_pair_ok": (_i, [C.POINTER(Fn2ConvDesc), C.POINTER(Fn2ConvDesc)]),
+    "fn2_conv2d_pair_splits": (_i, [C.POINTER(Fn2ConvDesc), C.POINTER(Fn2ConvDesc)]),
+    "fn2_conv2d_pair_workspace_bytes": (C.c_int64, [C.POINTER(Fn2ConvDesc), C.POINTER(Fn2ConvDesc)]),
+    "fn2_conv2d_pair": (_i, [C.POINTER(Fn2ConvDesc), C.POINTER(Fn2ConvDesc), _p]),
+    "fn2_conv2d_pair_kernel_name": (_i, [C.POINTER(Fn2ConvDesc), C.POINTER(Fn2ConvDesc), C.c_char_p, _i]),
     "fn2_augment_f32": (_i, [_p, _p, _p, _p, _i, _i, _i, _i, _i, _i, _p]),
     "fn2_flow_augmentation_f32": (_i, [_p, _p, _p, _p, _i, _i, _i, _i, _i, _p]),
     "fn2_flow_head_gather": (_i, [_p, _i, _p, _p, _i, _i, _i, _p]),
diff --git a/flownet2-tf_amd/src/engine.py b/flownet2-tf_amd/src/engine.py
--- a/flownet2-tf_amd/src/engine.py
+++ b/flownet2-tf_amd/src/engine.py
@@ -32,6 +32,9 @@
         return f"2, 2, 2, 1, 3, 1, {m16}" if ring else f"2, 2, 2, 1, 2, 1, {m16}"
     return f"2, 2, 2, 2, 2, 1, {m16}"
 
+
+PAIR_TAILS_DEFAULT = "1"
+PAIR_FROM_DEFAULT = "conv4"
 
 _TNAME = {"f32": "float", "bf16": "__bf16", "f16": "_Float16", "f16x2": "fn2::x2_t"}
 
@@ -122,6 +125,8 @@
         self._defer_flow = False
         self._own_ws = set()
         self._pending_head = None
+        self._pair_hook = None
+        self._pairs = []
         self.outputs = self._build()
         assert self._pending_head is None
         self._check_variables(strict)
@@ -213,7 +218,7 @@
         self.ops.append((name, fn, args))
         self.branch_of.append(self._branch)
 
-    def _conv(self, scope, spec, src, dst, up=None, up_after=None, defer_head=False):
+    def _conv(self, scope, spec, src, dst, up=None, up_after=None, defer_head=False, emit=True):
         name, kind, k, stride, pad, cin, cout, act = spec
         sbuf, sc0, sc = src
         dbuf, dc0, dc = dst
@@ -301,17 +306,41 @@
             shape = {128: "4, 2, 2", 64: "4, 1, 4", 32: "2, 1, 4", 16: "1, 1, 4"}[tile]
             on = _TNAME[self.dtype_name] if self._code(dbuf) == self.act_code else "float"
             kern = f"conv_igemm_kernel<{tn}, {on}, {shape}>"
-        if defer_head and kern.startswith("flow_head_kernel"):
-            assert self._pending_head is None
-            self._pending_head = d
-        else:
-            self._op(f"{scope}/{name}", self.lib.fn2_conv2d, C.byref(d), kernel=kern)
         n, oh, ow = dbuf.shape[0], dbuf.shape[1], dbuf.shape[2]
         taps = k * k if kind == "conv" else 4
-        self.layer_flops.append((f"{scope}/{name}", 2.0 * n * oh * ow * taps * cin * cout))
         osz = 4 if dbuf.dtype == torch.float32 else 2
-        self.layer_io_bytes.append((f"{scope}/{name}", float(sbuf.shape[0] * sbuf.shape[1] * sbuf.shape[2] * cin * esz
-                                                            + n * oh * ow * cout * osz + k * k * cin * cout * esz)))
+        rec = dict(name=f"{scope}/{name}", desc=d, kern=kern, flops=2.0 * n * oh * ow * taps * cin * cout,
+                   io=float(sbuf.shape[0] * sbuf.shape[1] * sbuf.shape[2] * cin * esz + n * oh * ow * cout * osz
+                            + k * k * cin * cout * esz))
+        if not emit:
+            assert not defer_head
+            return rec
+        self._emit_conv(rec, launch=not (defer_head and kern.startswith("flow_head_kernel")))
+
+    def _emit_conv(self, rec, launch=True):
+        if launch:
+            self._op(rec["name"], self.lib.fn2_conv2d, C.byref(rec["desc"]), kernel=rec["kern"])
+        else:
+            assert self._pending_head is None
+            self._pending_head = rec["desc"]
+        self.layer_flops.append((rec["name"], rec["flops"]))
+        self.layer_io_bytes.append((rec["name"], rec["io"]))
+
+    def _pair_ok(self, da, db):
+        need = int(self.lib.fn2_conv2d_pair_workspace_bytes(C.byref(da), C.byref(db)))
+        if need <= 0:
+            return False
+        da.workspace, da.workspace_bytes = 1, need
+        ok = bool(self.lib.fn2_conv2d_pair_ok(C.byref(da), C.byref(db)))
+        da.workspace, da.workspace_bytes = None, 0
+        return ok
+
+    def _emit_pair(self, ra, rb):
+        name = ra["name"] + "+" + rb["name"]
+        self._op(name, self.lib.fn2_conv2d_pair, C.byref(ra["desc"]), C.byref(rb["desc"]), kernel=ra["kern"])
+        self._pairs.append((ra["desc"], rb["desc"], self._branch))
+        self.layer_flops.append((name, ra["flops"] + rb["flops"]))
+        self.layer_io_bytes.append((name, ra["io"] + rb["io"]))
 
     def _head_slabs(self, d, head_t, t_cs):
         need = int(self.lib.fn2_conv2d_workspace_bytes(C.byref(d)))
@@ -561,6 +590,9 @@
             if fn is self.lib.fn2_conv2d:
                 if self.lib.fn2_conv2d_kernel_name(args[0], buf, 256) == 0 and buf.value:
                     self.kernel_of[i] = buf.value.decode()
+            elif fn is self.lib.fn2_conv2d_pair:
+                _hip.check(self.lib.fn2_conv2d_pair_kernel_name(args[0], args[1], buf, 256))
+                self.kernel_of[i] = buf.value.decode()
 
     def _alloc_workspace(self):
         branches = self.desc_branch + [0] * (len(self.conv_descs) - len(self.desc_branch))
@@ -568,6 +600,8 @@
         for br in sorted(set(branches)):
             descs = [d for d, b in zip(self.conv_descs, branches) if b == br and C.addressof(d) not in self._own_ws]
             need = max([int(self.lib.fn2_conv2d_workspace_bytes(C.byref(d))) for d in descs] + [0])
+            need = max([int(self.lib.fn2_conv2d_pair_workspace_bytes(C.byref(da), C.byref(db)))
+                        for da, db, b in self._pairs if b == br] + [need])
             if need > 0:
                 self.workspace[br] = torch.empty((need + 3) // 4, dtype=torch.float32, device=self.device)
                 for d in descs:
@@ -646,19 +680,54 @@
                 3: self._buf(f"{tag}/concat3", N, H // 8, W_ // 8, 386),
                 2: self._buf(f"{tag}/concat2", N, H // 4, W_ // 4, 194)}
 
-    def _encoder_tail(self, scope, tag, L, cats):
+    def _tail_steps(self, tag, cats):
         N, H, W_ = self.N, self.H, self.W
         c4 = self._buf(f"{tag}/conv4", N, H // 16, W_ // 16, 512)
-        self._conv(scope, L["conv4"], (cats[3], 0, 256), (c4, 0, 512))
-        self._conv(scope, L["conv4_1"], (c4, 0, 512), (cats[4], 0, 512))
         c5 = self._buf(f"{tag}/conv5", N, H // 32, W_ // 32, 512)
-        self._conv(scope, L["conv5"], (cats[4], 0, 512), (c5, 0, 512))
-        self._conv(scope, L["conv5_1"], (c5, 0, 512), (cats[5], 0, 512))
         c6 = self._buf(f"{tag}/conv6", N, H // 64, W_ // 64, 1024)
-        self._conv(scope, L["conv6"], (cats[5], 0, 512), (c6, 0, 1024))
         c6_1 = self._buf(f"{tag}/conv6_1", N, H // 64, W_ // 64, 1024)
-        self._conv(scope, L["conv6_1"], (c6, 0, 1024), (c6_1, 0, 1024))
+        return [("conv4", (cats[3], 0, 256), (c4, 0, 512)), ("conv4_1", (c4, 0, 512), (cats[4], 0, 512)),
+                ("conv5", (cats[4], 0, 512), (c5, 0, 512)), ("conv5_1", (c5, 0, 512), (cats[5], 0, 512)),
+                ("conv6", (cats[5], 0, 512), (c6, 0, 1024)), ("conv6_1", (c6, 0, 1024), (c6_1, 0, 1024))], c6_1
+
+    def _encoder_tail(self, scope, tag, L, cats):
+        steps, c6_1 = self._tail_steps(tag, cats)
+        for name, src, dst in steps:
+            self._conv(scope, L[name], src, dst)
         return c6_1
+
+    def _encoder_tails_paired(self, net_a, net_b, lane_b):
+        (scope_a, tag_a, L_a, cats_a), (scope_b, tag_b, L_b, cats_b) = net_a, net_b
+        steps_a, out_a = self._tail_steps(tag_a, cats_a)
+        steps_b, out_b = self._tail_steps(tag_b, cats_b)
+        names = [s[0] for s in steps_a]
+        first = os.environ.get("FN2_PAIR_FROM", PAIR_FROM_DEFAULT)
+        if first not in names:
+            raise ValueError("FN2_PAIR_FROM must be one of %s, got %r" % (", ".join(names), first))
+        M = self._branch
+        b_ahead = True
+        a_ahead = False
+        for i, ((name, src_a, dst_a), (_, src_b, dst_b)) in enumerate(zip(steps_a, steps_b)):
+            ra = self._conv(scope_a, L_a[name], src_a, dst_a, emit=False)
+            with self._lane(lane_b):
+                rb = self._conv(scope_b, L_b[name], src_b, dst_b, emit=False)
+            if i >= names.index(first) and self._pair_ok(ra["desc"], rb["desc"]):
+                if b_ahead:
+                    self._sync(M, lane_b)
+                    b_ahead = False
+                self._emit_pair(ra, rb)
+                a_ahead = True
+            else:
+                with self._lane(lane_b):
+                    if a_ahead:
+                        self._sync(lane_b, M)
+                        a_ahead = False
+                    self._emit_conv(rb)
+                self._emit_conv(ra)
+                b_ahead = True
+        if a_ahead:
+            self._sync(lane_b, M)
+        return out_a, out_b
 
     def _net_s(self, scope, tag, x, cin):
         N, H, W_ = self.N, self.H, self.W
@@ -730,11 +799,23 @@
             self._conv(scope, L["conv_redir"], (c3a, 0, 256), (net, 0, 32))
         self._sync(M, T)
         self._conv(scope, L["conv3_1"], (net, 0, 473), (cats[3], 0, 256))
-        c6_1 = self._encoder_tail(scope, tag, L, cats)
+        if self._pair_hook is not None:
+            c6_1 = self._pair_hook(scope, tag, L, cats)
+        else:
+            c6_1 = self._encoder_tail(scope, tag, L, cats)
         preds = self._refine(scope, tag, L, c6_1, cats, False)
         return self._final_flow(tag, preds, 20.0)
 
     def _net_sd(self, scope, tag, x):
+        L, cats = self._net_sd_head(scope, tag, x)
+        c6_1 = self._encoder_tail(scope, tag, L, cats)
+        return self._net_sd_rest(scope, tag, L, c6_1, cats)
+
+    def _net_sd_rest(self, scope, tag, L, c6_1, cats):
+        preds = self._refine(scope, tag, L, c6_1, cats, True)
+        return self._final_flow(tag, preds, 0.05)
+
+    def _net_sd_head(self, scope, tag, x):
         N, H, W_ = self.N, self.H, self.W
         L = {s[0]: s for s in netdefs.flownet_sd_layers()}
         cats = self._alloc_cats(tag, N)
@@ -750,9 +831,7 @@
         c3 = self._buf(f"{tag}/conv3", N, H // 8, W_ // 8, 256)
         self._conv(scope, L["conv3"], (c2_1, 0, 128), (c3, 0, 256))
         self._conv(scope, L["conv3_1"], (c3, 0, 256), (cats[3], 0, 256))
-        c6_1 = self._encoder_tail(scope, tag, L, cats)
-        preds = self._refine(scope, tag, L, c6_1, cats, True)
-        return self._final_flow(tag, preds, 0.05)
+        return L, cats
 
     def _corr_kernel_name(self, tn, h):
         nl = 4 if self.dtype_name in ("bf16", "f16") else 8
@@ -802,14 +881,36 @@
     def _net_2(self, scope, tag):
         N, H, W_ = self.N, self.H, self.W
         fork = len(self.ops)
+        sd_scope, sd_tag = scope + "/FlowNetSD", tag + "/SD"
+
+        def fork_sd():
+            at = fork + min(int(os.environ.get("FN2_SD_FORK_OPS", "0")), len(self.ops) - fork)
+            self.syncs.append((at, 1, 0))
+            if self._lane_mask & 8 and int(os.environ.get("FN2_FORK3", "1")):
+                self.syncs.append((at, 3, 0))
+
+        paired = {}
+        if (self._lanes_on and self._lane_mask & 2 and self.dtype_name == "f16x2" and self.fragment_weights
+                and int(os.environ.get("FN2_PAIR_TAILS", PAIR_TAILS_DEFAULT))):
+            def hook(c_scope, c_tag, c_L, c_cats):
+                self._pair_hook = None
+                fork_sd()
+                with self._lane(1):
+                    sd_L, sd_cats = self._net_sd_head(sd_scope, sd_tag, self._pair_input(sd_tag, 1))
+                c6_1, sd_c6_1 = self._encoder_tails_paired((c_scope, c_tag, c_L, c_cats), (sd_scope, sd_tag, sd_L, sd_cats), 1)
+                paired.update(L=sd_L, cats=sd_cats, c6_1=sd_c6_1)
+                return c6_1
+            self._pair_hook = hook
         css = self._sub(self._net_css, scope + "/FlowNetCSS", tag + "/CSS")
-        if self._lanes_on and self._lane_mask & 2:
-            fork += min(int(os.environ.get("FN2_SD_FORK_OPS", "0")), len(self.ops) - fork)
-            self.syncs.append((fork, 1, 0))
-            if self._lane_mask & 8 and int(os.environ.get("FN2_FORK3", "1")):
-                self.syncs.append((fork, 3, 0))
-        with self._lane(1):
-            sd = self._sub(self._net_sd, scope + "/FlowNetSD", tag + "/SD", self._pair_input(tag + "/SD", 1))
+        assert self._pair_hook is None
+        if paired:
+            with self._lane(1):
+                sd = self._sub(self._net_sd_rest, sd_scope, sd_tag, paired["L"], paired["c6_1"], paired["cats"])
+        else:
+            if self._lanes_on and self._lane_mask & 2:
+                fork_sd()
+            with self._lane(1):
+                sd = self._sub(self._net_sd, sd_scope, sd_tag, self._pair_input(sd_tag, 1))
         if self._lanes_on and self._lane_mask & 2:
             self._sync(0, 1)
         L = {s[0]: s for s in netdefs.fusion_layers()}
diff --git a/include/flownet2_hip.h b/include/flownet2_hip.h
--- a/include/flownet2_hip.h
+++ b/include/flownet2_hip.h
@@ -102,6 +102,12 @@
 int fn2_conv2d_kernel_name(const fn2_conv_desc* desc, char* name, int cap);
 int fn2_conv2d_splits(const fn2_conv_desc* desc);
 
+int fn2_conv2d_pair_ok(const fn2_conv_desc* a, const fn2_conv_desc* b);
+int fn2_conv2d_pair_splits(const fn2_conv_desc* a, const fn2_conv_desc* b);
+int64_t fn2_conv2d_pair_workspace_bytes(const fn2_conv_desc* a, const fn2_conv_desc* b);
+int fn2_conv2d_pair(const fn2_conv_desc* a, const fn2_conv_desc* b, void* stream);
+int fn2_conv2d_pair_kernel_name(const fn2_conv_desc* a, const fn2_conv_desc* b, char* name, int cap);
+
 int fn2_flow_head_gather(const float* t, int t_cs, const float* bias, float* out, int n, int h, int w, void* stream);
 int fn2_flow_head_tail(const float* t, int t_cs, int taps, const float* bias, float* pf, int n, int h, int w, int ring,
                        const float* up_w, const float* up_bias, const fn2_tensor* up_out, void* stream);
```

Result: slower. 1063 pairs/s (-4.4%).
